# G1OJS/PyFT8

Hardware: AMD Instinct MI355X
Metric: FT8 15-s frames decoded/sec (higher is better)
Workload: dtype f32

## Files before the change

### pyft8_amd/csrc/ft8rx.hip

```cpp
#include <hip/hip_runtime.h>
#include <math.h>
#include <stdarg.h>
#include <stdio.h>
#include <stdlib.h>
#include <string.h>
#include <algorithm>
#include <new>
#include <string>
#include <vector>
#include "../../include/ft8rx.h"
#include "ft8_dev.h"

#define WL_MULT(i) ((i) == WL_BP0 ? 5 : (i) == WL_OSDNAN ? 10 : 1)
#define NF0MAX (FT8RX_MAX_F0 > 1024 ? 2048 : 1024)

#include "kernels/common.hpp"
#include "kernels/spectrogram.hpp"
#include "kernels/sync_search.hpp"
#include "kernels/llr.hpp"
#include "kernels/ap_patterns.hpp"
#include "kernels/bp.hpp"
#include "kernels/cycle_spectrum.hpp"
#include "kernels/fine_sync.hpp"
#include "kernels/osd.hpp"
#include "kernels/ap_calls.hpp"
#include "kernels/recall.hpp"
#include "kernels/report.hpp"
#include "kernels/ddc.hpp"
#include "kernels/synth.hpp"
#include "kernels/subtract.hpp"
#include "kernels/probes.hpp"
#include "host_messages.hpp"
#include "batch_plan.hpp"
#include "ddc_ring.hpp"
#include "optins.hpp"
#include "ilp_launch.hpp"

#define EV_EAGER_BYTES ((size_t)1 << 20)
#define HIPCHK(h, x) do { hipError_t _e = (x); if (_e != hipSuccess) { set_err(h, "%s failed: %s (%s:%d)", #x, hipGetErrorString(_e), __FILE__, __LINE__); return -2; } } while (0)

static std::vector<uint32_t> osd_trial_table(int S, int D, int T) {
    std::vector<uint32_t> t;
    const uint32_t N = OSD_NONE;
    t.push_back(N | (N << 8) | (N << 16));
    for (int i = 0; i < S; i++) t.push_back((uint32_t)i | (N << 8) | (N << 16));
    for (int i = 0; i < S; i++) for (int j = 0; j < D && j < i; j++) t.push_back((uint32_t)i | ((uint32_t)j << 8) | (N << 16));
    for (int i = 0; i < T; i++) for (int j = 0; j < i; j++) for (int k = 0; k < j; k++) t.push_back((uint32_t)i | ((uint32_t)j << 8) | ((uint32_t)k << 16));
    return t;
}
static int osd_nflip(int S, int T) { return S > T ? S : T; }

struct ft8rx_hashes { hostmsg::Hashes H; };

#define SYNC_WIN 352
static size_t sync_lds_bytes(const ft8rx_config& c) {
    const int nh0 = c.h0_hi - c.h0_lo;
    const size_t nrows = (size_t)((nh0 < SYNC_WIN ? nh0 : SYNC_WIN) + 24);
    return nrows * 16 * sizeof(double) + (nrows * 29 + 512) * sizeof(float);
}
static std::string g_create_err;

struct ResultSlot {
    ft8rx_record* rec = nullptr; int32_t* ncand = nullptr; ft8rx_event* ev = nullptr; int32_t* evcount = nullptr;
    ft8rx_record* h_rec = nullptr; int32_t* h_cnt = nullptr; ft8rx_event* h_ev = nullptr; int32_t* h_evc = nullptr;
    hipEvent_t ev_comp = nullptr, ev_done = nullptr;
    int B = 0;
    bool evpending = false;
    int32_t* d_evoffs = nullptr; ft8rx_event* h_evpacked = nullptr; ft8rx_event* d_evpacked = nullptr;
    bool packed = false;
    unsigned char* pk_buf = nullptr; hipEvent_t pk_fence = nullptr;
    ft8rx_packed_header* h_pkhdr = nullptr; ft8rx_packed_header* d_pkhdr = nullptr;
    bool recall = false;
    ft8rx_recall_entry* d_rc_ent = nullptr; int32_t* d_rc_cnt = nullptr; ft8rx_record* d_rc_rec = nullptr;
    ft8rx_record* h_rc_rec = nullptr; int32_t* h_rc_cnt = nullptr;
    bool reports = false;
    ft8rx_report* d_rp = nullptr; ft8rx_report* h_rp = nullptr;
};

static ApCalls ap_calls_off() { ApCalls a; memset(&a, 0, sizeof(a)); a.max_hd = FT8RX_AP_MAX_HD_DEFAULT; return a; }

#ifndef LADDER_GRID_CAP
#define LADDER_GRID_CAP (4 * 256 * 32)
#endif

struct ft8rx_handle {
    ft8rx_config cfg = {};
    int device = 0, max_frames = 0;
    hipStream_t stream = nullptr;
    int n_streams = 2;
    int ladder_mode = 0;
    int ladder_cap = LADDER_GRID_CAP;
    int msg_types = 0;
    bool weak = false; float weak_sync_min = FT8RX_WEAK_SYNC_MIN_DEFAULT; int32_t weak_osd_max_hd = FT8RX_WEAK_OSD_MAX_HD_DEFAULT;
    ApCalls ap = ap_calls_off();
    uint32_t ap_version = 0, ap_chunk_version[batchplan::MAX_CHUNKS] = {};
    ApCalls* d_apc = nullptr;
    int32_t* d_apcount = nullptr;
    bool rc_armed = false; int rc_frames = 0; bool rc_td = false; std::vector<int32_t> rc_off;
    int32_t rc_max_hd = FT8RX_RECALL_MAX_HD_DEFAULT, rc_min_gap = FT8RX_RECALL_MIN_GAP_DEFAULT;
    ft8rx_recall_entry* d_rc_src = nullptr; int32_t* d_rc_srccnt = nullptr; int32_t* d_rc_off = nullptr;
    int32_t* d_rc_trip = nullptr; int32_t* d_rc_tout = nullptr; float* d_rc_tsd = nullptr; float* d_rc_sgrid = nullptr; float* d_rc_llr = nullptr;
    bool reports = false;
    int32_t* d_rp_items = nullptr; int32_t* d_rp_count = nullptr;
    int sub_frames = FT8RX_SUBBATCH_DEFAULT;
    hipStream_t sub[batchplan::MAX_STREAMS] = {};
    hipEvent_t ev_fork = nullptr, ev_join[batchplan::MAX_STREAMS] = {};
    hipStream_t copy_s = nullptr;
    hipEvent_t ev_chunk[batchplan::MAX_CHUNKS] = {};
    Tables T = {};
    std::vector<void*> allocs, pinned;
    unsigned ready = 0;
    struct Chunk { void* p; size_t cap, used; };
    std::vector<Chunk> arena;
    int16_t* d_audio = nullptr;
    int16_t* d_audio2 = nullptr;
    hipStream_t h2d_s = nullptr;
    float* d_grid = nullptr;
    float* d_best_score = nullptr; int32_t* d_best_h0 = nullptr;
    ft8rx_record* d_rec = nullptr; int32_t* d_ncand = nullptr; ft8rx_event* d_ev = nullptr; int32_t* d_evcount = nullptr;
    float* d_llr0 = nullptr; float* d_saved = nullptr;
    Att *d_att0 = nullptr, *d_attG = nullptr, *d_attB = nullptr, *d_attO = nullptr;
    cpx *d_A = nullptr, *d_spec = nullptr;
    const uint32_t* d_trials = nullptr; int n_trials = 0;
    int32_t* d_work[WL_N] = {};
    int32_t* d_wcount = nullptr;
    uint8_t* d_colmask = nullptr; bool use_mask = false;
    ResultSlot slots[2];
    int slot_enq = 0, slot_fetch = 0, inflight = 0, last_slot = -1, fetched_slot = -1;
    hipEvent_t ev_cdone[2][batchplan::MAX_STREAMS] = {};
    bool free_running = false, need_barrier = true; int part_B = 0, part_n = 0;
    uint64_t pk_cap = 0; uint64_t* d_pkneed = nullptr; int32_t* d_pknrec = nullptr;
    hipEvent_t d2h_ev[32] = {}; uint32_t d2h_next = 0;
    float* d_wf = nullptr; double2* d_part = nullptr; double* d_pulse = nullptr; double* d_pc = nullptr;
    ft8rx_subsig* d_sigs = nullptr; int32_t* d_sigcnt = nullptr; int sig_cap = 0;
    float2 *d_zdec = nullptr, *d_model = nullptr, *d_adec = nullptr; SubdCtx* d_subctx = nullptr;
    double* d_ones = nullptr;
    DdcOut* d_ddc_outs = nullptr; DdcOut* h_ddc_outs = nullptr; hipEvent_t ddc_ev = nullptr; void* d_ddc_in = nullptr; size_t ddc_in_cap = 0;
    struct DdcStream {
        bool open = false; int kind = 0, D = 0, n_streams = 0, n_out = 0; int32_t rate = 0; float scale = 0.0f;
        int64_t n_origin = 0, pushed = 0, tiles = 0, cap = 0;
        void* d_in = nullptr; int16_t* d_out = nullptr; float* d_f32 = nullptr; DdcOut* d_outs = nullptr; char* h_stage = nullptr;
        hipEvent_t ev = nullptr;
    } ds;
    std::string err;
    bool profiling = false;
    std::vector<hipEvent_t> pev;
    std::vector<const char*> pnames;
    int n_stage = 0;
    float stage_ms[24] = {};
};
static_assert(sizeof(ft8rx_handle::ev_chunk) / sizeof(hipEvent_t) == batchplan::MAX_CHUNKS &&
              sizeof(ft8rx_handle::ap_chunk_version) / sizeof(uint32_t) == batchplan::MAX_CHUNKS &&
              sizeof(batchplan::BatchPlan::cb) / sizeof(int) == batchplan::MAX_CHUNKS + 1 &&
              batchplan::MAX_CHUNKS == 16 && batchplan::MAX_STREAMS == 8, "per-chunk arrays and the plan's boundaries");

static_assert(ddcring::TILE == DDC_TO && ddcring::OUT_RING == 2 * FT8RX_NSAMP, "ddc_ring.hpp: tile and output ring");
template <int D> constexpr bool ddc_ring_geom_ok() {
    using G = DdcGeom<D>;
    return ddcring::geom(D).R1 == G::R1 && ddcring::geom(D).C1 == G::C1 && ddcring::geom(D).R2 == G::R2 && ddcring::geom(D).C2 == G::C2 &&
           ddcring::last(D) == (int64_t)(G::NV - 1 - G::C2) * G::R1 + G::C1 && ddcring::in_capacity(D) >= 12000 * D + ddcring::span(D);
}
static_assert(ddc_ring_geom_ok<1>() && ddc_ring_geom_ok<2>() && ddc_ring_geom_ok<4>() && ddc_ring_geom_ok<8>() && ddc_ring_geom_ok<16>(),
              "ddc_ring.hpp: the filter geometry is the kernels'");

static void set_err(ft8rx_handle* h, const char* fmt, ...) {
    char buf[512];
    va_list ap; va_start(ap, fmt); vsnprintf(buf, sizeof(buf), fmt, ap); va_end(ap);
    if (h) h->err = buf; else g_create_err = buf;
}

#include <mutex>
struct StreamPool { hipStream_t main = nullptr, copy = nullptr, h2d = nullptr, sub[8] = {}; };
static std::mutex g_pool_mu;
static StreamPool g_pool[64];
static hipStream_t pool_stream(int device, hipStream_t StreamPool::* which, bool blocking) {
    std::lock_guard<std::mutex> lk(g_pool_mu);
    StreamPool& P = g_pool[device & 63];
    if (!(P.*which)) {
        hipStream_t s = nullptr;
        if ((blocking ? hipStreamCreate(&s) : hipStreamCreateWithFlags(&s, hipStreamNonBlocking)) != hipSuccess) return nullptr;
        P.*which = s;
    }
    return P.*which;
}
static hipStream_t pool_sub(int device, int i) {
    std::lock_guard<std::mutex> lk(g_pool_mu);
    StreamPool& P = g_pool[device & 63];
    if (!P.sub[i] && hipStreamCreateWithFlags(&P.sub[i], hipStreamNonBlocking) != hipSuccess) P.sub[i] = nullptr;
    return P.sub[i];
}

template <typename T> static int dalloc(ft8rx_handle* h, T** p, size_t n) {
    void* q = nullptr;
    hipError_t e = hipMalloc(&q, n * sizeof(T));
    if (e != hipSuccess) { set_err(h, "hipMalloc(%zu bytes) failed: %s", n * sizeof(T), hipGetErrorString(e)); return -2; }
    h->allocs.push_back(q); *p = (T*)q; return 0;
}
template <typename T> static int halloc(ft8rx_handle* h, T** p, size_t n, T** dev = nullptr) {
    void *q = nullptr, *d = nullptr;
    hipError_t e = hipHostMalloc(&q, n * sizeof(T), hipHostMallocDefault);
    if (e == hipSuccess && dev && (e = hipHostGetDevicePointer(&d, q, 0)) != hipSuccess) hipHostFree(q);
    if (e != hipSuccess) { set_err(h, "hipHostMalloc(%zu bytes) failed: %s", n * sizeof(T), hipGetErrorString(e)); return -2; }
    h->pinned.push_back(q); *p = (T*)q; if (dev) *dev = (T*)d; return 0;
}

enum WsGroup { WS_STAGING, WS_STAGING2, WS_MASK, WS_RECALL, WS_REPORTS, WS_PACKED, WS_SUB, WS_SUBD, WS_ONES, WS_DDC };
struct FirstUse {
    ft8rx_handle* h; WsGroup g; size_t nd, nh; int rc = 0;
    std::vector<void**> members;
    FirstUse(ft8rx_handle* h_, WsGroup g_) : h(h_), g(g_), nd(h_->allocs.size()), nh(h_->pinned.size()) {}
    template <typename T> void dev(T** p, size_t n) { if (!rc && !(rc = dalloc(h, p, n))) members.push_back((void**)p); }
    template <typename T> void host(T** p, size_t n, T** d = nullptr) {
        if (rc || (rc = halloc(h, p, n, d))) return;
        members.push_back((void**)p); if (d) members.push_back((void**)d);
    }
    int done() {
        if (!rc) { h->ready |= 1u << g; return 0; }
        while (h->allocs.size() > nd) { hipFree(h->allocs.back()); h->allocs.pop_back(); }
        while (h->pinned.size() > nh) { hipHostFree(h->pinned.back()); h->pinned.pop_back(); }
        for (void** m : members) *m = nullptr;
        return -2;
    }
};
static bool ws_ready(const ft8rx_handle* h, WsGroup g) { return (h->ready >> g) & 1u; }
#define FIRST_HIP(F, x) do { if (!(F).rc) { hipError_t _e = (x); if (_e != hipSuccess) { set_err((F).h, "%s failed: %s (%s:%d)", #x, hipGetErrorString(_e), __FILE__, __LINE__); (F).rc = -2; } } } while (0)

static int need_staging(ft8rx_handle* h, bool second = false) {
    const WsGroup g = second ? WS_STAGING2 : WS_STAGING;
    if (ws_ready(h, g)) return 0;
    FirstUse F(h, g);
    F.dev(second ? &h->d_audio2 : &h->d_audio, (size_t)h->max_frames * FT8RX_NSAMP);
    return F.done();
}

static void host_twiddle(int n, int count, std::vector<cpx>& w) {
    w.resize(count);
    for (int t = 0; t < count; t++) {
        double ang = (2.0 * M_PI * (double)t) / (double)n;
        w[t] = make_float2((float)cos(ang), (float)(-sin(ang)));
    }
}
template <typename T> static int upload(ft8rx_handle* h, const T** dst, const std::vector<T>& v) {
    T* p; if (dalloc(h, &p, v.size())) return -2;
    if (hipMemcpy(p, v.data(), v.size() * sizeof(T), hipMemcpyHostToDevice) != hipSuccess) { set_err(h, "table upload failed"); return -2; }
    *dst = p; return 0;
}

struct Scratch {
    ft8rx_handle* h;
    ~Scratch() { for (auto& c : h->arena) c.used = 0; }
    void* raw(size_t bytes) {
        bytes = (bytes + 255) & ~(size_t)255;
        if (!bytes) bytes = 256;
        for (auto& c : h->arena) if (c.cap - c.used >= bytes) { void* q = (char*)c.p + c.used; c.used += bytes; return q; }
        size_t largest = 0;
        for (auto& c : h->arena) if (c.cap > largest) largest = c.cap;
        size_t cap = bytes > 2 * largest ? bytes : 2 * largest;
        if (cap < ((size_t)1 << 20)) cap = (size_t)1 << 20;
        for (size_t i = 0; i < h->arena.size();) {
            if (h->arena[i].used == 0) { hipFree(h->arena[i].p); h->arena.erase(h->arena.begin() + i); } else i++;
        }
        void* q = nullptr;
        if (hipMalloc(&q, cap) != hipSuccess) { if (cap == bytes || hipMalloc(&q, bytes) != hipSuccess) return nullptr; cap = bytes; }
        h->arena.push_back({q, cap, bytes});
        return q;
    }
    template <typename T> T* get(size_t n) { return (T*)raw(n * sizeof(T)); }
    template <typename T> T* put(const T* src, size_t n) { T* q = get<T>(n); if (q && hipMemcpy(q, src, n * sizeof(T), hipMemcpyHostToDevice) != hipSuccess) return nullptr; return q; }
};

static int quiesce(ft8rx_handle* h, bool next_is_batch = false) {
    if (h->free_running || (h->last_slot >= 0 && !next_is_batch)) HIPCHK(h, hipStreamSynchronize(h->copy_s));
    h->free_running = false;
    h->need_barrier = true;
    return 0;
}
#define ENTER(h) do { HIPCHK(h, hipSetDevice((h)->device)); { const int _q = quiesce(h); if (_q) return _q; } } while (0)

template <class K, class KX, class... A>
static void launch_mt(K k, KX kx, unsigned mt, int grid, hipStream_t s, A... a) {
    if (!mt) k<<<grid, 64, 0, s>>>(a...);
    else kx<<<grid, 64, 0, s>>>(a..., mt);
}

static unsigned active_optins(const ft8rx_handle* h) {
    using namespace optins;
    return (h->slots[0].pk_buf ? bit(PACKED) : 0) | (h->msg_types != 0 ? bit(MSG_TYPES) : 0) | (h->ap.np != 0 ? bit(AP_CALLS) : 0) |
           (h->rc_armed ? bit(RECALL) : 0) | (h->weak ? bit(WEAK) : 0) | (h->reports ? bit(REPORTS) : 0);
}
static int refuse_conflict(ft8rx_handle* h, const char* who, optins::Id which, const char* hint = "") {
    const int c = optins::conflict(active_optins(h), which);
    if (c < 0) return 0;
    set_err(h, "%s: not supported together with %s%s", who, optins::TABLE[c].name, hint);
    return -1;
}

extern "C" {

int ft8rx_default_config(ft8rx_config* c) {
    if (!c) return -1;
    c->sync_score_min = 85.0f; c->max_cands = 200; c->f0_lo = 32; c->f0_hi = 960; c->h0_lo = -37; c->h0_hi = 87;
    c->bp_nc0_a = 35; c->bp_iters_a = 5; c->bp_nc0_b = 90; c->bp_iters_b = 20; c->osd_single = 30; c->osd_double = 2;
    c->llr_sd_min = 5.0f;
    c->osd_triple = 0; c->osd_max_hd = 0;
    return 0;
}

int ft8rx_device_count(void) { int n = 0; if (hipGetDeviceCount(&n) != hipSuccess) return 0; return n; }
int ft8rx_device_pci_bus_id(int device, char* buf, int len) {
    if (!buf || len < 16) return -1;
    return hipDeviceGetPCIBusId(buf, len, device) == hipSuccess ? 0 : -2;
}
int ft8rx_build_info(int32_t* grid_cols, int32_t* spec_bins, int32_t* max_f0) {
    static_assert(NF0MAX >= FT8RX_GRID_COLS && NF0MAX >= FT8RX_MAX_F0, "per-f0 scratch stride");
    if (grid_cols) *grid_cols = FT8RX_GRID_COLS;
    if (spec_bins) *spec_bins = FT8RX_SPEC_BINS;
    if (max_f0) *max_f0 = FT8RX_MAX_F0;
    return 0;
}
int ft8rx_build_limits(int32_t* max_cands, int32_t* event_cap) {
    static_assert(FT8RX_MAX_CANDS <= NF0MAX && (1 << cand_shift(FT8RX_MAX_CANDS)) == FT8RX_MAX_CANDS,
                  "max_cands: never more than k_topk has keys, and the largest candidate stride is the limit itself");
    if (max_cands) *max_cands = FT8RX_MAX_CANDS;
    if (event_cap) *event_cap = FT8RX_EVENT_CAP;
    return 0;
}

int ft8rx_get_fft_plans(int32_t* p1920, int32_t* p3200, int32_t* p300, int32_t* p320) {
    const int32_t a[8] = {8, 4, 4, 5, 3, 0, 0, 0}, b[8] = {8, 4, 4, 5, 5, 0, 0, 0}, c[8] = {5, 5, 4, 3, 0, 0, 0, 0}, d[8] = {8, 8, 5, 0, 0, 0, 0, 0};
    if (p1920) memcpy(p1920, a, sizeof(a));
    if (p3200) memcpy(p3200, b, sizeof(b));
    if (p300) memcpy(p300, c, sizeof(c));
    if (p320) memcpy(p320, d, sizeof(d));
    return 0;
}

const char* ft8rx_last_error(ft8rx_handle* h) { return h ? h->err.c_str() : g_create_err.c_str(); }

void ft8rx_destroy(ft8rx_handle* h) {
    if (!h) return;
    hipSetDevice(h->device);
    if (h->stream) hipStreamSynchronize(h->stream);
    if (h->copy_s) hipStreamSynchronize(h->copy_s);
    if (h->h2d_s) hipStreamSynchronize(h->h2d_s);
    for (int i = 0; i < 8; i++) { if (h->sub[i]) hipStreamSynchronize(h->sub[i]); if (h->ev_join[i]) hipEventDestroy(h->ev_join[i]); }
    for (void* p : h->allocs) hipFree(p);
    for (auto& c : h->arena) hipFree(c.p);
    for (auto e : h->pev) hipEventDestroy(e);
    for (int k = 0; k < 2; k++) for (int i = 0; i < 8; i++) if (h->ev_cdone[k][i]) hipEventDestroy(h->ev_cdone[k][i]);
    for (int i = 0; i < 32; i++) if (h->d2h_ev[i]) hipEventDestroy(h->d2h_ev[i]);
    for (hipEvent_t e : h->ev_chunk) if (e) hipEventDestroy(e);
    if (h->ev_fork) hipEventDestroy(h->ev_fork);
    if (h->ddc_ev) hipEventDestroy(h->ddc_ev);
    if (h->ds.ev) hipEventDestroy(h->ds.ev);
    for (ResultSlot& sl : h->slots) {
        if (sl.ev_comp) hipEventDestroy(sl.ev_comp);
        if (sl.ev_done) hipEventDestroy(sl.ev_done);
    }
    for (void* p : h->pinned) hipHostFree(p);
    delete h;
}

int ft8rx_create(const ft8rx_config* cfg, int device, int max_frames, ft8rx_handle** out) {
    if (!cfg || !out || max_frames < 1) { set_err(nullptr, "ft8rx_create: bad arguments"); return -1; }
    if (cfg->max_cands < 1 || cfg->max_cands > FT8RX_MAX_CANDS || cfg->f0_lo < 4 || cfg->f0_hi > FT8RX_MAX_F0 || cfg->f0_lo >= cfg->f0_hi ||
        cfg->h0_hi <= cfg->h0_lo || cfg->h0_lo < FT8RX_MIN_H0 || cfg->h0_hi > FT8RX_MAX_H0 || cfg->bp_nc0_a > cfg->bp_nc0_b || cfg->bp_iters_a > cfg->bp_iters_b ||
        cfg->osd_single < 0 || cfg->osd_single > OSD_MAXFLIP || cfg->osd_double < 0 || cfg->osd_double > OSD_MAXFLIP ||
        cfg->osd_triple < 0 || cfg->osd_triple > 40 || cfg->osd_max_hd < 0 || cfg->osd_max_hd > 174 ||
        osd_trial_table(cfg->osd_single, cfg->osd_double, cfg->osd_triple).size() > OSD_MAXTRIALS) {
        set_err(nullptr, "ft8rx_create: configuration out of the supported range"); return -1; }
    int ndev = 0;
    if (hipGetDeviceCount(&ndev) != hipSuccess || ndev < 1) { set_err(nullptr, "ft8rx_create: no HIP device available (this library has no CPU fallback)"); return -3; }
    if (device < 0 || device >= ndev) { set_err(nullptr, "ft8rx_create: device %d out of range (%d devices)", device, ndev); return -1; }
    ft8rx_handle* h = new ft8rx_handle();
    h->cfg = *cfg; h->device = device; h->max_frames = max_frames;
    if (hipSetDevice(device) != hipSuccess || !(h->stream = pool_stream(device, &StreamPool::main, true))) { set_err(nullptr, "ft8rx_create: cannot open device %d", device); delete h; return -2; }
    const size_t B = (size_t)max_frames, S = (size_t)1 << cand_shift(*cfg);
    int rc = 0;
    rc |= dalloc(h, &h->d_grid, B * FT8RX_GRID_ROWS * FT8RX_GRID_COLS);
    rc |= dalloc(h, &h->d_best_score, B * NF0MAX);
    rc |= dalloc(h, &h->d_best_h0, B * NF0MAX);
    rc |= dalloc(h, &h->d_rec, B * S);
    rc |= dalloc(h, &h->d_ncand, B);
    rc |= dalloc(h, &h->d_llr0, B * S * 174);
    rc |= dalloc(h, &h->d_saved, B * S * 5 * 174);
    rc |= dalloc(h, &h->d_att0, B * S * 5);
    rc |= dalloc(h, &h->d_attG, B * S * 2);
    rc |= dalloc(h, &h->d_attB, B * S * 5);
    rc |= dalloc(h, &h->d_attO, B * S * 10);
    static_assert((size_t)(96000 + FT8RX_SPEC_BINS) * sizeof(cpx) <= (size_t)FT8RX_GRID_ROWS * FT8RX_GRID_COLS * sizeof(float), "scratch A + cycle spectrum fit a frame's grid");
    if (!rc) { h->d_A = reinterpret_cast<cpx*>(h->d_grid); h->d_spec = h->d_A + B * 96000; }
    for (int i = 0; i < WL_N; i++) rc |= dalloc(h, &h->d_work[i], B * S * WL_MULT(i));
    rc |= dalloc(h, &h->d_wcount, (size_t)batchplan::MAX_CHUNKS * WL_N);
    rc |= dalloc(h, &h->d_apc, batchplan::MAX_CHUNKS);
    rc |= dalloc(h, &h->d_apcount, (size_t)batchplan::MAX_CHUNKS * 2);
    rc |= dalloc(h, &h->d_ev, B * FT8RX_EVENT_CAP);
    rc |= dalloc(h, &h->d_evcount, B);
    ResultSlot* const sl = h->slots;
    sl[0].rec = h->d_rec; sl[0].ncand = h->d_ncand; sl[0].ev = h->d_ev; sl[0].evcount = h->d_evcount;
    rc |= dalloc(h, &sl[1].rec, B * S);
    rc |= dalloc(h, &sl[1].ncand, B);
    rc |= dalloc(h, &sl[1].ev, B * FT8RX_EVENT_CAP);
    rc |= dalloc(h, &sl[1].evcount, B);
    const bool ev_compact = B * FT8RX_EVENT_CAP * sizeof(ft8rx_event) > EV_EAGER_BYTES;
    for (int k = 0; k < 2 && ev_compact; k++) rc |= dalloc(h, &sl[k].d_evoffs, B + 1);
    for (int k = 0; k < 2 && !rc; k++) {
        rc = halloc(h, &sl[k].h_rec, B * cfg->max_cands);
        if (!rc) rc = halloc(h, &sl[k].h_cnt, B);
        if (!rc) rc = halloc(h, &sl[k].h_ev, B * FT8RX_EVENT_CAP);
        if (!rc) rc = halloc(h, &sl[k].h_evc, B);
        if (!rc && ev_compact) rc = halloc(h, &sl[k].h_evpacked, B * FT8RX_EVENT_CAP, &sl[k].d_evpacked);
    }
    if (rc) { g_create_err = h->err; ft8rx_destroy(h); return -2; }
    std::vector<float> win(3840);
    for (int i = 0; i < 3840; i++) win[i] = (float)(0.5 + 0.5 * cos(M_PI * (double)(2 * i + 1 - 3840) / 3839.0));
    std::vector<double> taper(100);
    { double step = (0.0 - M_PI) / 99.0; for (int i = 0; i < 100; i++) { double y = (i == 99) ? 0.0 : (double)i * step + M_PI; taper[i] = 0.5 * (1.0 + cos(y)); } }
    std::vector<cpx> w;
    rc |= upload(h, &h->T.win, win);
    rc |= upload(h, &h->T.taper, taper);
    host_twiddle(1920, 1920, w);   rc |= upload(h, &h->T.W1920, w);
    host_twiddle(3840, FT8RX_GRID_COLS, w);    rc |= upload(h, &h->T.WR3840, w);
    host_twiddle(3200, 3200, w);   rc |= upload(h, &h->T.W3200, w);
    host_twiddle(96000, 96000, w); rc |= upload(h, &h->T.W96000, w);
    host_twiddle(300, 300, w);     rc |= upload(h, &h->T.W300, w);
    host_twiddle(320, 320, w);     rc |= upload(h, &h->T.W320, w);
    host_twiddle(192000, FT8RX_SPEC_BINS, w); rc |= upload(h, &h->T.WR192k, w);
    host_twiddle(32, 32, w);       rc |= upload(h, &h->T.W32, w);
    {
        std::vector<float> k32(1800);
        std::vector<cpx> cs(156), g1000(1000);
        for (int m = -900; m < 900; m++) {
            const int r = ((m % 100) + 100) % 100;
            k32[m + 900] = (r == 0) ? (m == 0 ? 32.0f : 0.0f) : (float)(sin(M_PI * (double)r / 100.0) / sin(M_PI * (double)m / 3200.0));
        }
        for (int sidx = 1; sidx < 7; sidx++) for (int q = 0; q <= 25; q++) {
            const double a = 2.0 * M_PI * (double)((q * sidx) % 100) / 100.0;
            cpx v = make_float2((float)cos(a), (float)sin(a));
            if (q == 0) v = make_float2(1.0f, 0.0f);
            cs[(sidx - 1) * 26 + q] = v;
        }
        for (int k = -150; k < 850; k++) {
            const int r = ((k % 100) + 100) % 100, j = (k - r) / 100;
            const double a = M_PI * (31.0 * (double)r - 100.0 * (double)j) / 3200.0;
            g1000[k + 150] = make_float2((float)cos(a), (float)sin(a));
        }
        std::vector<cpx> tw100(100);
        for (int m = 0; m < 100; m++) { const double a = -2.0 * M_PI * (double)m / 100.0; tw100[m] = make_float2((float)cos(a), (float)sin(a)); }
        rc |= upload(h, &h->T.K32, k32); rc |= upload(h, &h->T.CS100, cs); rc |= upload(h, &h->T.G1000, g1000); rc |= upload(h, &h->T.TW100, tw100);
    }
    if (rc) { g_create_err = h->err; ft8rx_destroy(h); return -2; }
    bool ok = true;
    ok &= hipMemcpyToSymbol(HIP_SYMBOL(d_CHK_N), FT8_CHK_N, sizeof(FT8_CHK_N)) == hipSuccess;
    ok &= hipMemcpyToSymbol(HIP_SYMBOL(d_CHK_V), FT8_CHK_V, sizeof(FT8_CHK_V)) == hipSuccess;
    {
        static uint8_t ev[522], ec[522]; static uint16_t ve[174][3];
        auto slot = [](int e) { const int c = FT8_EDGE_C[e], j = e - FT8_CHK_E0[c]; return j < 6 ? 83 * j + c : 498 + (c - 59); };
        for (int e = 0; e < 522; e++) { ev[slot(e)] = FT8_EDGE_V[e]; ec[slot(e)] = FT8_EDGE_C[e]; }
        for (int v = 0; v < 174; v++) for (int k = 0; k < 3; k++) ve[v][k] = (uint16_t)slot(FT8_VAR_E[v][k]);
        ok &= hipMemcpyToSymbol(HIP_SYMBOL(d_EDGE_V), ev, sizeof(ev)) == hipSuccess;
        ok &= hipMemcpyToSymbol(HIP_SYMBOL(d_EDGE_C), ec, sizeof(ec)) == hipSuccess;
        ok &= hipMemcpyToSymbol(HIP_SYMBOL(d_VAR_E), ve, sizeof(ve)) == hipSuccess;
    }
    ok &= hipMemcpyToSymbol(HIP_SYMBOL(d_G0), FT8_G0, sizeof(FT8_G0)) == hipSuccess;
    {
        static uint64_t rcg[83][2];
        memset(rcg, 0, sizeof(rcg));
        for (int r = 0; r < 91; r++) for (int j = 0; j < 83; j++) {
            const int v = 91 + j;
            if ((FT8_G0[r][v >> 6] >> (v & 63)) & 1ull) rcg[j][r >> 6] |= 1ull << (r & 63);
        }
        ok &= hipMemcpyToSymbol(HIP_SYMBOL(d_RCG), rcg, sizeof(rcg)) == hipSuccess;
    }
    {
        static uint64_t cm[128][3];
        memset(cm, 0, sizeof(cm));
        for (int c = 0; c < 83; c++) for (int j = 0; j < FT8_CHK_N[c]; j++) { int v = FT8_CHK_V[c][j]; cm[c][v >> 6] |= 1ull << (v & 63); }
        ok &= hipMemcpyToSymbol(HIP_SYMBOL(d_CHK_MASK), cm, sizeof(cm)) == hipSuccess;
    }
    {
        uint16_t syn[77];
        for (int pos = 0; pos < 77; pos++) syn[pos] = (uint16_t)hostmsg::crc14_serial(pos < 64 ? (1ull << pos) : 0ull, pos >= 64 ? (1ull << (pos - 64)) : 0ull);
        ok &= hipMemcpyToSymbol(HIP_SYMBOL(d_CRC_SYN), syn, sizeof(syn)) == hipSuccess;
    }
    {
        static uint32_t g0t[192][3];
        memset(g0t, 0, sizeof(g0t));
        for (int r = 0; r < 91; r++) for (int v = 0; v < 174; v++) if ((FT8_G0[r][v >> 6] >> (v & 63)) & 1ull) g0t[v][r >> 5] |= 1u << (r & 31);
        ok &= hipMemcpyToSymbol(HIP_SYMBOL(d_G0T), g0t, sizeof(g0t)) == hipSuccess;
        uint16_t syn91[96]; memset(syn91, 0, sizeof(syn91));
        for (int v = 0; v < 91; v++) {
            if (v < 77) { const int pos = 76 - v; syn91[v] = (uint16_t)hostmsg::crc14_serial(pos < 64 ? (1ull << pos) : 0ull, pos >= 64 ? (1ull << (pos - 64)) : 0ull); }
            else syn91[v] = (uint16_t)(1u << (13 - (v - 77)));
        }
        uint32_t synm[14][3]; memset(synm, 0, sizeof(synm));
        for (int v = 0; v < 91; v++) for (int k = 0; k < 14; k++) if ((syn91[v] >> k) & 1) synm[k][v >> 5] |= 1u << (v & 31);
        ok &= hipMemcpyToSymbol(HIP_SYMBOL(d_SYNM), synm, sizeof(synm)) == hipSuccess;
        static uint16_t ct[12][256];
        for (int b = 0; b < 12; b++) for (int x = 0; x < 256; x++) { uint16_t a = 0; for (int t = 0; t < 8; t++) if ((x >> t) & 1) a ^= syn91[8 * b + t]; ct[b][x] = a; }
        ok &= hipMemcpyToSymbol(HIP_SYMBOL(d_CRC_T), ct, sizeof(ct)) == hipSuccess;
        {
            float xn[174]; int perm[176], stk[64]; uint8_t p8[192];
            for (int i = 0; i < 174; i++) xn[i] = NAN;
            osd_std_sort_withnan(xn, perm, stk);
            memset(p8, 0, sizeof(p8));
            for (int i = 0; i < 174; i++) p8[i] = (uint8_t)perm[i];
            ok &= hipMemcpyToSymbol(HIP_SYMBOL(d_NANPERM), p8, sizeof(p8)) == hipSuccess;
        }
        const std::vector<uint32_t> tr = osd_trial_table(cfg->osd_single, cfg->osd_double, cfg->osd_triple);
        h->n_trials = (int)tr.size();
        if (upload(h, &h->d_trials, tr)) ok = false;
    }
    if (!ok) { set_err(nullptr, "ft8rx_create: device table upload failed"); ft8rx_destroy(h); return -2; }
    if (sync_lds_bytes(*cfg) > 65536) {
        ok &= hipFuncSetAttribute((const void*)k_sync, hipFuncAttributeMaxDynamicSharedMemorySize, (int)sync_lds_bytes(*cfg)) == hipSuccess;
        ok &= hipFuncSetAttribute((const void*)k_sync_acc, hipFuncAttributeMaxDynamicSharedMemorySize, (int)sync_lds_bytes(*cfg)) == hipSuccess;
    }
    if (!ok) { set_err(nullptr, "ft8rx_create: cannot reserve LDS for k_sync"); ft8rx_destroy(h); return -2; }
    int nfill = (int)B * FT8RX_GRID_COLS;
    k_fill_row0<<<(nfill + 255) / 256, 256, 0, h->stream>>>(h->d_grid, (int)B);
    if (hipStreamSynchronize(h->stream) != hipSuccess) { set_err(nullptr, "ft8rx_create: init kernel failed"); ft8rx_destroy(h); return -2; }
    bool okc = true;
    for (int i = 0; i < 24; i++) { hipEvent_t e = nullptr; okc = okc && hipEventCreate(&e) == hipSuccess; if (e) h->pev.push_back(e); }
    if (const char* e = getenv("FT8RX_SUBS_FIRST")) for (int i = 0; i < atoi(e) && i < 8; i++) pool_sub(device, i);
    okc = okc && (h->copy_s = pool_stream(device, &StreamPool::copy, false)) != nullptr;
    okc = okc && (h->h2d_s = pool_stream(device, &StreamPool::h2d, false)) != nullptr;
    for (hipEvent_t& e : h->ev_chunk) okc = okc && hipEventCreateWithFlags(&e, hipEventDisableTiming) == hipSuccess;
    okc = okc && hipEventCreateWithFlags(&h->ev_fork, hipEventDisableTiming) == hipSuccess;
    for (ResultSlot& s : h->slots) {
        okc = okc && hipEventCreateWithFlags(&s.ev_comp, hipEventDisableTiming) == hipSuccess;
        okc = okc && hipEventCreateWithFlags(&s.ev_done, hipEventDisableTiming) == hipSuccess;
    }
    if (!okc) { set_err(nullptr, "ft8rx_create: cannot create HIP streams/events"); ft8rx_destroy(h); return -2; }
    *out = h;
    return 0;
}

int ft8rx_set_profiling(ft8rx_handle* h, int on) { if (!h) return -1; h->profiling = on != 0; return 0; }

int ft8rx_get_stage_times(ft8rx_handle* h, int* n, const char** names, float* ms) {
    if (!h || !n) return -1;
    *n = h->n_stage;
    for (int i = 0; i < h->n_stage; i++) { if (names) names[i] = h->pnames[i]; if (ms) ms[i] = h->stage_ms[i]; }
    return 0;
}


static int ladder_grid(const ft8rx_handle* h, int max_items) { return max_items < h->ladder_cap ? max_items : h->ladder_cap; }

static void launch_sync(const float* grid, float* bs, int32_t* bh, const ft8rx_config& c, int B, hipStream_t s, bool weak) {
    const auto first = weak ? k_sync3 : k_sync, acc = weak ? k_sync3_acc : k_sync_acc;
    const int win = weak ? SYNC3_WIN : SYNC_WIN;
    const size_t lds = weak ? 0 : sync_lds_bytes(c);
    const int ntile = (c.f0_hi - c.f0_lo + 15) / 16;
    for (int lo = c.h0_lo; lo < c.h0_hi; lo += win) {
        ft8rx_config w = c;
        w.h0_lo = lo; w.h0_hi = lo + win < c.h0_hi ? lo + win : c.h0_hi;
        (lo == c.h0_lo ? first : acc)<<<dim3(ntile, B), 256, lds, s>>>(grid, bs, bh, w);
    }
}
static ft8rx_config weak_config(const ft8rx_handle* h) {
    ft8rx_config w = h->cfg;
    w.sync_score_min = h->weak_sync_min;
    w.llr_sd_min = -INFINITY;
    if (!w.osd_max_hd) w.osd_max_hd = h->weak_osd_max_hd;
    return w;
}
static void launch_fine(ft8rx_handle* h, const ft8rx_config& cfg, bool weak, int n_blocks, hipStream_t s, const cpx* spec, ft8rx_record* rec,
                        const int32_t* ncand, float* llr, const int32_t* trip, int32_t* t_out, float* t_sd, float* t_sgrid, WorkList work,
                        bool need_td) {
    if (weak) { k_fine_weak<<<n_blocks, FINE_NT, 0, s>>>(spec, rec, ncand, llr, h->T, cfg, trip, t_out, t_sd, t_sgrid, work); return; }
    ft8rx_ilp_fine(n_blocks, s, spec, rec, ncand, llr, h->T, cfg, trip, t_out, t_sd, t_sgrid, work);
    if (need_td) k_fine_td<<<n_blocks, FINE_NT, 0, s>>>(spec, rec, ncand, llr, h->T, cfg, trip, t_out, t_sd, t_sgrid, work);
}

static bool osd_wide(int nflip) { return nflip > OSD_FLIPS_A; }
static void launch_osd(const ft8rx_handle* h, unsigned mt, int grid, hipStream_t s, int mode, const float* llr, const float* saved, const Att* attB, ft8rx_record* rec,
                       const int32_t* ncand, Att* attO, ft8rx_event* ev, int32_t* evc, const uint32_t* trials, int ntr, int nflip, int max_hd,
                       int sh, WorkList work, WorkList nanl) {
    const bool wide = osd_wide(nflip);
    launch_mt(wide ? k_osd_wide : k_osd, wide ? k_osd_wide_ext : k_osd_ext, mt, grid, s,
              mode, llr, saved, attB, rec, ncand, attO, ev, evc, trials, ntr, nflip, max_hd, sh, work, nanl);
    launch_mt(wide ? k_osd_nan_wide : k_osd_nan, wide ? k_osd_nan_wide_ext : k_osd_nan_ext, mt, ladder_grid(h, OSD_NAN_GRID), s,
              mode, llr, saved, attB, rec, ncand, attO, ev, evc, trials, ntr, nflip, max_hd, sh, nanl);
}

static void launch_ap_calls(ft8rx_handle* h, int B, const float* llr0, ft8rx_record* rec, const int32_t* ncand, Att* attO, ft8rx_event* ev,
                            int32_t* evc, int32_t* cand_items, int32_t* osd_items, int32_t* ac, const ApCalls* apc, hipStream_t s) {
    const ft8rx_config& c = h->cfg;
    const int sh = cand_shift(c); const size_t S = (size_t)1 << sh;
    const int nflip = osd_nflip(c.osd_single, c.osd_triple);
    hipMemsetAsync(ac, 0, 2 * sizeof(int32_t), s);
    const WorkList cl = {cand_items, ac}, ol = {osd_items, ac + 1};
    k_ap_worklist<<<(B * S + 255) / 256, 256, 0, s>>>(rec, ncand, B, sh, cl);
    k_bp_ap<<<ladder_grid(h, B * c.max_cands * h->ap.np), 64, 0, s>>>(llr0, rec, ncand, attO, ev, evc, c, apc, cl, ol);
    (osd_wide(nflip) ? k_osd_ap_wide : k_osd_ap)<<<ladder_grid(h, B * c.max_cands * 3), 64, 0, s>>>(
        llr0, rec, ncand, attO, ev, evc, h->d_trials, h->n_trials, nflip, sh, apc, ol);
    k_select_ap<<<(B * S + 255) / 256, 256, 0, s>>>(rec, attO, apc, cl);
}

static void launch_reports(ft8rx_handle* h, int B, const cpx* spec, const ft8rx_record* rec, const int32_t* ncand, int32_t* items,
                           int32_t* count, ft8rx_report* rep, hipStream_t s) {
    const ft8rx_config& c = h->cfg;
    const int sh = cand_shift(c); const size_t S = (size_t)1 << sh;
    hipMemsetAsync(count, 0, sizeof(int32_t), s);
    const WorkList wl = {items, count};
    k_report_worklist<<<(B * S + 255) / 256, 256, 0, s>>>(rec, ncand, B, sh, wl, rep);
    k_report<<<ladder_grid(h, B * c.max_cands), FINE_NT, 0, s>>>(spec, rec, rep, h->T, sh, wl);
}

static void enqueue_chain(ft8rx_handle* h, const int16_t* d_audio, int f0, int B, hipStream_t s, bool prof, int slot, int chunk) {
    const ResultSlot& sl = h->slots[slot];
    const bool weak = h->weak;
    const ft8rx_config cw = weak ? weak_config(h) : h->cfg;
    const ft8rx_config& c = weak ? cw : h->cfg;
    const size_t F = (size_t)f0;
    const int sh = cand_shift(c); const size_t S = (size_t)1 << sh, FS = F * S;
    const int16_t* audio = d_audio + F * FT8RX_NSAMP;
    float* grid = h->d_grid + F * FT8RX_GRID_ROWS * FT8RX_GRID_COLS;
    float* bs = h->d_best_score + F * NF0MAX; int32_t* bh = h->d_best_h0 + F * NF0MAX;
    ft8rx_record* rec = sl.rec + FS; int32_t* ncand = sl.ncand + F;
    float* llr0 = h->d_llr0 + FS * 174; float* saved = h->d_saved + FS * 5 * 174;
    Att* att0 = h->d_att0 + FS * 5; Att* attG = h->d_attG + FS * 2; Att* attB = h->d_attB + FS * 5; Att* attO = h->d_attO + FS * 10;
    cpx* A = reinterpret_cast<cpx*>(grid); cpx* spec = A + (size_t)B * 96000;
    ft8rx_event* ev = sl.ev + F * FT8RX_EVENT_CAP; int32_t* evc = sl.evcount + F;
#define STAGE(name) do { if (prof) { hipEventRecord(h->pev[h->pnames.size()], s); h->pnames.push_back(name); } } while (0)
    int32_t* wc = h->d_wcount + WL_N * chunk;
    WorkList wl[WL_N];
    for (int i = 0; i < WL_N; i++) { wl[i].items = h->d_work[i] + FS * WL_MULT(i); wl[i].count = wc + i; }
    STAGE("spectrogram");
    ft8rx_ilp_spectrogram(B, s, audio, grid, h->T);
    STAGE("sync");
    launch_sync(grid, bs, bh, c, B, s, weak);
    STAGE("topk");
    k_topk<<<B, 1024, 0, s>>>(bs, bh, rec, ncand, c, evc, wc, h->use_mask ? h->d_colmask + F * NF0MAX : nullptr);
    STAGE("grid_llr");
    const unsigned mt = (unsigned)h->msg_types;
    launch_mt(k_grid_llr, k_grid_llr_ext, mt, XCD_GRID(B, c.max_cands), s, grid, rec, ncand, llr0, c, nullptr, nullptr, nullptr, att0, ev, evc, B);
    k_worklist_att<<<(B * S * 5 + 255) / 256, 256, 0, s>>>(rec, ncand, att0, B, sh, wl[WL_BP0]);
    STAGE("bp_grid");
    launch_mt(k_bp, k_bp_ext, mt, ladder_grid(h, B * c.max_cands * 5), s, 0, llr0, rec, ncand, nullptr, att0, nullptr, ev, evc, c, c.bp_nc0_a, c.bp_iters_a, wl[WL_BP0], 0, 5);
    STAGE("select0");
    k_select0<<<(B * S + 255) / 256, 256, 0, s>>>(rec, ncand, att0, B, sh, wl[WL_FINE]);
    STAGE("cycle_fft");
    k_cyc_a<<<dim3(40, B), 256, 0, s>>>(audio, A, h->T);
    k_cyc_bc<<<dim3(CYC_BC_GRID, B), 256, 0, s>>>(A, spec, h->T);
    STAGE("fine");
    launch_fine(h, c, weak, ladder_grid(h, B * c.max_cands), s, spec, rec, ncand, llr0, nullptr, nullptr, nullptr, nullptr, wl[WL_FINE],
                c.h0_lo < FT8RX_MIN_H0_FD || c.h0_hi > FT8RX_MAX_H0_FD + 1);
    k_worklist<<<(B * S + 255) / 256, 256, 0, s>>>(rec, ncand, B, sh, wl[WL_BP1]);
    STAGE("bp_fine");
    const auto bp_fine = [&](int n_variants, const WorkList& work, int v0) {
        launch_mt(k_bp, k_bp_ext, mt, B * c.max_cands * n_variants, s, 1, llr0, rec, ncand, attG, attB, saved, ev, evc, c, c.bp_nc0_b, c.bp_iters_b,
                  work, v0, n_variants);
    };
    if (h->ladder_mode == 0) {
        bp_fine(1, wl[WL_BP1], 0);
        k_select1<<<(B * S + 255) / 256, 256, 0, s>>>(0, rec, ncand, attG, attB, B, c, wl[WL_BP1B]);
        bp_fine(1, wl[WL_BP1B], 1);
        k_select1<<<(B * S + 255) / 256, 256, 0, s>>>(1, rec, ncand, attG, attB, B, c, wl[WL_BP1C]);
        bp_fine(3, wl[WL_BP1C], 2);
        STAGE("select1");
        k_select1<<<(B * S + 255) / 256, 256, 0, s>>>(2, rec, ncand, attG, attB, B, c, wl[WL_OSD]);
    } else {
        bp_fine(5, wl[WL_BP1], 0);
        STAGE("select1");
        k_select1<<<(B * S + 255) / 256, 256, 0, s>>>(3, rec, ncand, attG, attB, B, c, wl[WL_OSD]);
    }
    STAGE("osd");
    launch_osd(h, mt, ladder_grid(h, B * c.max_cands * 10), s, 0, llr0, saved, attB, rec, ncand, attO, ev, evc, h->d_trials, h->n_trials,
               osd_nflip(c.osd_single, c.osd_triple), c.osd_max_hd, sh, wl[WL_OSD], wl[WL_OSDNAN]);
    STAGE("select2");
    k_select2<<<(B * S + 255) / 256, 256, 0, s>>>(rec, ncand, attO, B, sh);
    if (h->ap.np) {
        STAGE("ap_calls");
        ApCalls* apc = h->d_apc + chunk;
        if (h->ap_chunk_version[chunk] != h->ap_version) {
            k_ap_stage<<<1, 64, 0, s>>>(apc, h->ap);
            h->ap_chunk_version[chunk] = h->ap_version;
        }
        launch_ap_calls(h, B, llr0, rec, ncand, attO, ev, evc, wl[WL_BP0].items, wl[WL_OSDNAN].items, h->d_apcount + 2 * chunk, apc, s);
    }
    if (sl.recall) {
        STAGE("recall");
        ft8rx_recall_entry* ent = sl.d_rc_ent + F * FT8RX_RECALL_MAX;
        int32_t* rcnt = sl.d_rc_cnt + F;
        k_recall_stage<<<B, FT8RX_RECALL_MAX, 0, s>>>(h->d_rc_src + F * FT8RX_RECALL_MAX, h->d_rc_srccnt + F, ent, rcnt, sl.d_rc_rec + F * FT8RX_RECALL_MAX);
        const int base = h->rc_off[F], n = h->rc_off[F + B] - base;
        if (n > 0) {
            k_recall_trip<<<B, FT8RX_RECALL_MAX, 0, s>>>(ent, rcnt, h->d_rc_off + F, h->d_rc_trip);
            const size_t b = (size_t)base;
            launch_fine(h, c, false, n, s, spec, nullptr, nullptr, h->d_rc_llr + b * 174, h->d_rc_trip + 3 * b, h->d_rc_tout + 5 * b,
                        h->d_rc_tsd + b, h->d_rc_sgrid + b * 632, WorkList{nullptr, nullptr}, h->rc_td);
            k_recall_score<<<n, 64, 0, s>>>(h->d_rc_sgrid, h->d_rc_tout, h->d_rc_trip, h->d_rc_off + F, base, ent, rec, ncand, sh,
                                            h->rc_max_hd, h->rc_min_gap, sl.d_rc_rec + F * FT8RX_RECALL_MAX);
        }
    }
    if (sl.reports) {
        STAGE("report");
        launch_reports(h, B, spec, rec, ncand, h->d_rp_items + FS, h->d_rp_count + chunk, sl.d_rp + FS, s);
    }
    if (prof) hipEventRecord(h->pev[h->pnames.size()], s);
#undef STAGE
}

static void enqueue_chunk(ft8rx_handle* h, const int16_t* d_audio, int f0, int n, hipStream_t s, int slot, int chunk) {
    const int sub = (h->sub_frames > 0 && h->sub_frames < n) ? h->sub_frames : n;
    for (int o = 0; o < n; o += sub) enqueue_chain(h, d_audio, f0 + o, (o + sub <= n) ? sub : n - o, s, false, slot, chunk);
}

using batchplan::BatchPlan;
using batchplan::Entry;

static int batch_begin(ft8rx_handle* h, Entry e, int B, int slot, bool chunked, int16_t** stage) {
    ResultSlot& sl = h->slots[slot];
    h->pnames.clear();
    if (e != batchplan::DEVICE && need_staging(h)) return -2;
    if (e == batchplan::HOST_PIPELINED && slot == 1 && need_staging(h, true)) return -2;
    if (h->inflight == 2) { h->slot_fetch ^= 1; h->inflight = 1; }
    if (h->rc_armed && B != h->rc_frames) { set_err(h, "recall entries were set for %d frames, the batch has %d", h->rc_frames, B); return -1; }
    sl.recall = h->rc_armed;
    h->rc_armed = false;
    sl.reports = h->reports;
    *stage = h->d_audio;
    if (e == batchplan::HOST_PIPELINED) {
        *stage = slot ? h->d_audio2 : h->d_audio;
        HIPCHK(h, hipStreamWaitEvent(h->h2d_s, sl.ev_comp, 0));
    }
    for (int i = 1; i < h->n_streams && chunked; i++) if (!h->sub[i - 1]) {
        if (!(h->sub[i - 1] = pool_sub(h->device, i - 1))) { set_err(h, "cannot create a chunk stream"); return -2; }
        HIPCHK(h, hipEventCreateWithFlags(&h->ev_join[i - 1], hipEventDisableTiming));
    }
    return 0;
}

static int batch_submit(ft8rx_handle* h, const BatchPlan& plan, Entry e, int slot, const int16_t* audio, int16_t* stage) {
    ResultSlot& sl = h->slots[slot];
    const bool host = e != batchplan::DEVICE;
    const int16_t* d_audio = host ? stage : audio; const int16_t* host_audio = host ? audio : nullptr;
    const int ns = h->n_streams, nc = plan.nc, B = plan.cb[nc];
    const bool free_run = plan.mode == batchplan::FREE_RUN, pipelined = e == batchplan::HOST_PIPELINED, sync_host = e == batchplan::HOST_SYNC;
    hipStream_t cs = pipelined ? h->h2d_s : h->copy_s;
    const size_t frame_bytes = sizeof(int16_t) * (size_t)FT8RX_NSAMP;
    auto chunk_stream = [&](int k) { const int i = k % ns; return i == 0 ? h->stream : h->sub[i - 1]; };
    if (free_run) {
        for (int i = 0; i < ns; i++) for (int k = 0; k < 2; k++)
            if (!h->ev_cdone[k][i]) HIPCHK(h, hipEventCreateWithFlags(&h->ev_cdone[k][i], hipEventDisableTiming));
        if (h->need_barrier || h->part_B != B || h->part_n != nc) {
            if (h->free_running) HIPCHK(h, hipStreamWaitEvent(h->stream, h->slots[h->last_slot].ev_comp, 0));
            HIPCHK(h, hipEventRecord(h->ev_fork, h->stream));
            for (int i = 1; i < ns; i++) HIPCHK(h, hipStreamWaitEvent(h->sub[i - 1], h->ev_fork, 0));
            h->need_barrier = false; h->part_B = B; h->part_n = nc;
        }
    } else {
        { const int q = quiesce(h, true); if (q) return q; }
        HIPCHK(h, hipStreamWaitEvent(h->stream, sl.ev_done, 0));
        if (plan.mode == batchplan::SINGLE) {
            if (host_audio) HIPCHK(h, hipMemcpyAsync(stage, host_audio, frame_bytes * B, hipMemcpyHostToDevice, h->stream));
            if (h->profiling) enqueue_chain(h, d_audio, 0, B, h->stream, true, slot, 0);
            else enqueue_chunk(h, d_audio, 0, B, h->stream, slot, 0);
            return 0;
        }
        HIPCHK(h, hipEventRecord(h->ev_fork, h->stream));
        if (sync_host) HIPCHK(h, hipStreamWaitEvent(cs, h->ev_fork, 0));
        for (int i = 1; i < ns; i++) HIPCHK(h, hipStreamWaitEvent(h->sub[i - 1], h->ev_fork, 0));
    }
    if (pipelined) {
        HIPCHK(h, hipMemcpyAsync(stage, host_audio, frame_bytes * B, hipMemcpyHostToDevice, cs));
        HIPCHK(h, hipEventRecord(h->ev_chunk[0], cs));
        if (!free_run) for (int i = 0; i < ns; i++) HIPCHK(h, hipStreamWaitEvent(chunk_stream(i), h->ev_chunk[0], 0));
    }
    for (int k = 0; k < nc; k++) {
        const int f0 = plan.cb[k], n = plan.cb[k + 1] - f0;
        if (n <= 0 && !free_run) continue;
        hipStream_t s = chunk_stream(k);
        if (free_run) {
            HIPCHK(h, hipStreamWaitEvent(s, sl.ev_done, 0));
            if (pipelined) HIPCHK(h, hipStreamWaitEvent(s, h->ev_chunk[0], 0));
        } else if (sync_host) {
            HIPCHK(h, hipMemcpyAsync(stage + (size_t)f0 * FT8RX_NSAMP, host_audio + (size_t)f0 * FT8RX_NSAMP, frame_bytes * n, hipMemcpyHostToDevice, cs));
            HIPCHK(h, hipEventRecord(h->ev_chunk[k], cs));
            HIPCHK(h, hipStreamWaitEvent(s, h->ev_chunk[k], 0));
        }
        if (n > 0) enqueue_chunk(h, d_audio, f0, n, s, slot, k);
        if (free_run) {
            HIPCHK(h, hipEventRecord(h->ev_cdone[slot][k], s));
            HIPCHK(h, hipStreamWaitEvent(h->copy_s, h->ev_cdone[slot][k], 0));
        }
    }
    if (free_run) h->free_running = true;
    else for (int i = 1; i < ns; i++) {
        HIPCHK(h, hipEventRecord(h->ev_join[i - 1], h->sub[i - 1]));
        HIPCHK(h, hipStreamWaitEvent(h->stream, h->ev_join[i - 1], 0));
    }
    return 0;
}

static int batch_finish(ft8rx_handle* h, int slot, int B, hipStream_t fin) {
    ResultSlot& sl = h->slots[slot];
    const int mc = h->cfg.max_cands, sh = cand_shift(h->cfg);
    const bool pack_events = sl.d_evpacked && (size_t)B * FT8RX_EVENT_CAP * sizeof(ft8rx_event) > EV_EAGER_BYTES;
    if (pack_events) {
        k_ev_scan<<<1, 1024, 0, fin>>>(sl.evcount, B, sl.d_evoffs);
        k_ev_compact<<<B, 64, 0, fin>>>(sl.ev, sl.evcount, sl.d_evoffs, sl.d_evpacked);
    }
    sl.packed = sl.pk_buf != nullptr;
    if (sl.packed) {
        if (sl.pk_fence) { HIPCHK(h, hipStreamWaitEvent(fin, sl.pk_fence, 0)); sl.pk_fence = nullptr; }
        k_pack_count<<<B, 256, 0, fin>>>(sl.rec, sl.ncand, sl.ev, sl.evcount, h->d_pkneed, h->d_pknrec, sh);
        k_pack_scan<<<1, 1024, 0, fin>>>(h->d_pknrec, sl.ncand, sl.evcount, B, mc, (unsigned long long)h->pk_cap, sl.pk_buf, sl.d_pkhdr);
        k_pack_write<<<B, 256, 0, fin>>>(sl.rec, sl.ev, h->d_pkneed, B, sl.pk_buf, sh);
    }
    HIPCHK(h, hipEventRecord(sl.ev_comp, fin));
    if (fin != h->copy_s) HIPCHK(h, hipStreamWaitEvent(h->copy_s, sl.ev_comp, 0));
    HIPCHK(h, hipMemcpyAsync(sl.h_cnt, sl.ncand, sizeof(int32_t) * B, hipMemcpyDeviceToHost, h->copy_s));
    HIPCHK(h, hipMemcpy2DAsync(sl.h_rec, sizeof(ft8rx_record) * mc, sl.rec, sizeof(ft8rx_record) << sh, sizeof(ft8rx_record) * mc, B, hipMemcpyDeviceToHost, h->copy_s));
    HIPCHK(h, hipMemcpyAsync(sl.h_evc, sl.evcount, sizeof(int32_t) * B, hipMemcpyDeviceToHost, h->copy_s));
    sl.evpending = pack_events;
    if (!pack_events) HIPCHK(h, hipMemcpyAsync(sl.h_ev, sl.ev, sizeof(ft8rx_event) * (size_t)B * FT8RX_EVENT_CAP, hipMemcpyDeviceToHost, h->copy_s));
    if (sl.recall) {
        HIPCHK(h, hipMemcpyAsync(sl.h_rc_cnt, sl.d_rc_cnt, sizeof(int32_t) * B, hipMemcpyDeviceToHost, h->copy_s));
        HIPCHK(h, hipMemcpyAsync(sl.h_rc_rec, sl.d_rc_rec, sizeof(ft8rx_record) * FT8RX_RECALL_MAX * (size_t)B, hipMemcpyDeviceToHost, h->copy_s));
    }
    if (sl.reports)
        HIPCHK(h, hipMemcpy2DAsync(sl.h_rp, sizeof(ft8rx_report) * mc, sl.d_rp, sizeof(ft8rx_report) << sh, sizeof(ft8rx_report) * mc, B, hipMemcpyDeviceToHost, h->copy_s));
    HIPCHK(h, hipEventRecord(sl.ev_done, h->copy_s));
    sl.B = B; h->last_slot = slot; h->slot_enq ^= 1; h->inflight++;
    return 0;
}

static int launch_batch(ft8rx_handle* h, Entry e, const int16_t* audio, int B) {
    HIPCHK(h, hipSetDevice(h->device));
    const BatchPlan plan = batchplan::plan_batch(B, h->n_streams, h->profiling, e);
    const int slot = h->slot_enq;
    int16_t* stage = nullptr;
    if (const int rc = batch_begin(h, e, B, slot, plan.mode != batchplan::SINGLE, &stage)) return rc;
    if (const int rc = batch_submit(h, plan, e, slot, audio, stage)) return rc;
    HIPCHK(h, hipGetLastError());
    return batch_finish(h, slot, B, plan.mode == batchplan::FREE_RUN ? h->copy_s : h->stream);
}

static void fetch_events(ResultSlot& sl) {
    if (!sl.evpending) return;
    size_t off = 0;
    for (int f = 0; f < sl.B; f++) {
        int c = sl.h_evc[f]; c = c > FT8RX_EVENT_CAP ? FT8RX_EVENT_CAP : (c < 0 ? 0 : c);
// ... 2 lines not shown
    }
    sl.evpending = false;
}

int ft8rx_enqueue_batch(ft8rx_handle* h, const int16_t* d_audio, int B) {
    if (!h || !d_audio) return -1;
    if (B < 1 || B > h->max_frames) { set_err(h, "ft8rx_enqueue_batch: n_frames %d outside [1, %d]", B, h->max_frames); return -1; }
    return launch_batch(h, batchplan::DEVICE, d_audio, B);
}

int ft8rx_enqueue_batch_host(ft8rx_handle* h, const int16_t* audio, int B) {
    if (!h || !audio) return -1;
    if (B < 1 || B > h->max_frames) { set_err(h, "ft8rx_enqueue_batch_host: n_frames %d outside [1, %d]", B, h->max_frames); return -1; }
    return launch_batch(h, batchplan::HOST_PIPELINED, audio, B);
}

int ft8rx_set_streams(ft8rx_handle* h, int n) { if (!h || n < 1 || n > batchplan::MAX_STREAMS) return -1; h->n_streams = n; return 0; }
int ft8rx_set_subbatch(ft8rx_handle* h, int frames) { if (!h || frames < 0) return -1; h->sub_frames = frames; return 0; }
int ft8rx_set_ladder_mode(ft8rx_handle* h, int mode) { if (!h || mode < 0 || mode > 1) return -1; h->ladder_mode = mode; return 0; }

int ft8rx_set_ladder_grid(ft8rx_handle* h, int cap) {
    if (!h) return -1;
    if (cap < 0 || cap > LADDER_GRID_CAP) { set_err(h, "ft8rx_set_ladder_grid: cap %d outside [0, %d] (0 = the default, %d)", cap, LADDER_GRID_CAP, LADDER_GRID_CAP); return -1; }
    ENTER(h);
    h->ladder_cap = cap ? cap : LADDER_GRID_CAP;
    return 0;
}

int ft8rx_set_weak(ft8rx_handle* h, int32_t on, float sync_min, int32_t osd_max_hd) {
    if (!h) return -1;
    if (on) {
        if (!(sync_min > 0.0f) || !(sync_min < INFINITY)) { set_err(h, "ft8rx_set_weak: sync_min %g must be a positive score", (double)sync_min); return -1; }
        if (osd_max_hd < 1 || osd_max_hd > 174) { set_err(h, "ft8rx_set_weak: osd_max_hd %d outside [1, 174]", osd_max_hd); return -1; }
        if (refuse_conflict(h, "ft8rx_set_weak", optins::WEAK)) return -1;
        h->weak_sync_min = sync_min; h->weak_osd_max_hd = osd_max_hd;
    }
    h->weak = on != 0;
    return 0;
}

int ft8rx_set_msg_types(ft8rx_handle* h, int32_t mask) {
    if (!h) return -1;
    if (mask < 0 || mask > FT8RX_MT_ALL) { set_err(h, "ft8rx_set_msg_types: mask %d outside [0, %d]", mask, FT8RX_MT_ALL); return -1; }
    if (mask && refuse_conflict(h, "ft8rx_set_msg_types", optins::MSG_TYPES)) return -1;
    h->msg_types = mask;
    return 0;
}

static int build_ap_patterns(const char* my, const char* dx, ApCalls* a, std::string* err) {
    const bool hm = my && *my, hd = dx && *dx;
    const long cm = hm ? hostmsg::pack_c28_std(my) : 0, cd = hd ? hostmsg::pack_c28_std(dx) : 0;
    if (cm < 0) { *err = std::string("my_call '") + my + "' is not a standard callsign"; return -1; }
    if (cd < 0) { *err = std::string("dx_call '") + dx + "' is not a standard callsign"; return -1; }
    const int32_t max_hd = a->max_hd;
    memset(a, 0, sizeof(*a)); a->max_hd = max_hd;
    auto word = [](long c1, long c2, unsigned g15) { return ((unsigned __int128)c1 << 49) | ((unsigned __int128)c2 << 20) | ((unsigned __int128)g15 << 3) | 1u; };
    const unsigned G_RRR = 32402, G_73 = 32404, G_RR73 = 32403;
    for (int p = 5; p <= 10; p++) {
        const bool on = p == 5 ? hm : p == 7 ? hd : (hm && hd);
        if (!on) continue;
        const int k = p - FT8RX_AP_FIRST;
        const unsigned __int128 w = word(p == 7 ? 2 : cm, p == 5 ? 0 : cd, p == 8 ? G_RRR : p == 9 ? G_73 : G_RR73);
        const uint64_t lo = (uint64_t)w, hi = (uint64_t)(w >> 64);
        if (p >= 8) {
            hostmsg::encode_cw174(lo, hi, a->val[k]);
            a->msk[k][0] = a->msk[k][1] = ~0ull; a->msk[k][2] = (1ull << 46) - 1;
            a->lo[k] = lo; a->hi[k] = hi;
            hostmsg::Hashes H; std::string f[3];
            if (!hostmsg::unpack_ext(lo, hi, 0, H, f)) { *err = "the words of my_call / dx_call do not unpack as a standard message"; return -1; }
        } else {
            const int nk = p == 5 ? 29 : 58;
            for (int i = 0; i < 77; i++) {
                if (!(i < nk || i >= 74)) continue;
                const unsigned b = (unsigned)((w >> (76 - i)) & 1u);
                a->msk[k][i >> 6] |= 1ull << (i & 63);
                if (b) a->val[k][i >> 6] |= 1ull << (i & 63);
            }
        }
        a->pat[a->np++] = p;
    }
    return 0;
}

int ft8rx_set_ap_calls(ft8rx_handle* h, const char* my_call, const char* dx_call) {
    if (!h) return -1;
    ApCalls a = h->ap;
    std::string err;
    if (build_ap_patterns(my_call, dx_call, &a, &err)) { set_err(h, "ft8rx_set_ap_calls: %s", err.c_str()); return -1; }
    if (a.np && refuse_conflict(h, "ft8rx_set_ap_calls", optins::AP_CALLS)) return -1;
    h->ap = a; h->ap_version++;
    return 0;
}

int ft8rx_set_ap_max_hd(ft8rx_handle* h, int32_t max_hd) {
    if (!h) return -1;
    if (max_hd < 1 || max_hd > 174) { set_err(h, "ft8rx_set_ap_max_hd: %d outside [1, 174]", max_hd); return -1; }
    h->ap.max_hd = max_hd; h->ap_version++;
    return 0;
}

int ft8rx_ap_patterns(const char* my_call, const char* dx_call, uint8_t* bits_out, uint8_t* mask_out) {
    ApCalls a = ap_calls_off();
    std::string err;
    if (build_ap_patterns(my_call, dx_call, &a, &err)) { g_create_err = "ft8rx_ap_patterns: " + err; return -1; }
    for (int k = 0; k < FT8RX_AP_N; k++) for (int i = 0; i < 174; i++) {
        if (bits_out) bits_out[k * 174 + i] = (uint8_t)((a.val[k][i >> 6] >> (i & 63)) & 1ull);
        if (mask_out) mask_out[k * 174 + i] = (uint8_t)((a.msk[k][i >> 6] >> (i & 63)) & 1ull);
    }
    return 0;
}

static int recall_kind(uint64_t lo, uint64_t hi) {
    const unsigned i3 = (unsigned)(lo & 7u);
    if (i3 != 1 && i3 != 2) return RC_SKIP;
    const uint64_t ca = ((lo >> 49) | (hi << 15)) & 0xFFFFFFFull, cb = (lo >> 20) & 0xFFFFFFFull;
    const uint64_t STD = 2063592ull + 4194304ull;
    if (cb < STD || !(ca < 3 || ca >= STD)) return RC_SKIP;
    hostmsg::Hashes H; std::string f[3];
    if (!hostmsg::unpack_ext(lo, hi & 0x1FFFull, 0, H, f)) return RC_SKIP;
    for (int k = 0; k < 3; k++) if (f[k].find('<') != std::string::npos) return RC_SKIP;
    return ca < 3 ? RC_TOKEN : RC_CALL;
}

int ft8rx_recall_hypotheses(const ft8rx_recall_entry* entry, uint64_t* words_lo, uint64_t* words_hi) {
    if (!entry) return -1;
    const uint64_t lo = entry->msg_lo, hi = entry->msg_hi & 0x1FFFull;
    const int kind = recall_kind(lo, hi);
    if (kind == RC_SKIP) return 0;
    int n = 0;
    for (int k = 0; k < 126; k++) {
        uint64_t w; unsigned g15 = 0, r = 0;
        if (k == 0) w = lo;
        else if (kind != RC_CALL) break;
        else {
            if (k <= 3) g15 = 32401u + (unsigned)k;
            else if (k < 65) g15 = (unsigned)(32435 + (k - 4) - 30);
            else { g15 = (unsigned)(32435 + (k - 65) - 30); r = 1; }
            w = (lo & ~(0xFFFFull << 3)) | ((uint64_t)g15 << 3) | ((uint64_t)r << 18);
            if (w == lo) continue;
        }
        if (words_lo) words_lo[n] = w;
        if (words_hi) words_hi[n] = hi;
        n++;
    }
    return n;
}

static int recall_alloc(ft8rx_handle* h) {
    if (ws_ready(h, WS_RECALL)) return 0;
    const size_t B = (size_t)h->max_frames, N = B * FT8RX_RECALL_MAX;
    FirstUse F(h, WS_RECALL);
    F.dev(&h->d_rc_src, N); F.dev(&h->d_rc_srccnt, B); F.dev(&h->d_rc_off, B + 1);
    F.dev(&h->d_rc_trip, N * 3); F.dev(&h->d_rc_tout, N * 5); F.dev(&h->d_rc_tsd, N);
    F.dev(&h->d_rc_sgrid, N * 632); F.dev(&h->d_rc_llr, N * 174);
    for (ResultSlot& sl : h->slots) {
        F.dev(&sl.d_rc_ent, N); F.dev(&sl.d_rc_cnt, B); F.dev(&sl.d_rc_rec, N);
        F.host(&sl.h_rc_rec, N); F.host(&sl.h_rc_cnt, B);
    }
    return F.done();
}

int ft8rx_set_recall(ft8rx_handle* h, const ft8rx_recall_entry* entries, const int32_t* counts, int n_frames) {
    if (!h) return -1;
    ENTER(h);
    if (!entries || n_frames == 0) { h->rc_armed = false; return 0; }
    if (!counts || n_frames < 1 || n_frames > h->max_frames) { set_err(h, "ft8rx_set_recall: n_frames %d outside [1, %d]", n_frames, h->max_frames); return -1; }
    if (refuse_conflict(h, "ft8rx_set_recall", optins::RECALL)) return -1;
    const ft8rx_config& c = h->cfg;
    std::vector<ft8rx_recall_entry> st((size_t)n_frames * FT8RX_RECALL_MAX);
    std::vector<int32_t> cnt(n_frames), off(n_frames + 1, 0);
    bool td = false;
    for (int f = 0; f < n_frames; f++) {
        if (counts[f] < 0 || counts[f] > FT8RX_RECALL_MAX) { set_err(h, "ft8rx_set_recall: counts[%d] = %d outside [0, %d]", f, counts[f], FT8RX_RECALL_MAX); return -1; }
        cnt[f] = counts[f]; off[f + 1] = off[f] + counts[f];
        for (int e = 0; e < counts[f]; e++) {
            ft8rx_recall_entry E = entries[(size_t)f * FT8RX_RECALL_MAX + e];
            if (E.f0_idx < c.f0_lo || E.f0_idx >= c.f0_hi || E.h0_idx < c.h0_lo || E.h0_idx >= c.h0_hi) {
                set_err(h, "ft8rx_set_recall: entry %d of frame %d at (f0_idx %d, h0_idx %d) lies outside the search range", e, f, E.f0_idx, E.h0_idx); return -1; }
            E.pad = (uint16_t)recall_kind(E.msg_lo, E.msg_hi);
            td |= E.h0_idx < FT8RX_MIN_H0_FD || E.h0_idx > FT8RX_MAX_H0_FD;
            st[(size_t)f * FT8RX_RECALL_MAX + e] = E;
        }
    }
    if (recall_alloc(h)) return -2;
    HIPCHK(h, hipMemcpy(h->d_rc_src, st.data(), sizeof(ft8rx_recall_entry) * st.size(), hipMemcpyHostToDevice));
    HIPCHK(h, hipMemcpy(h->d_rc_srccnt, cnt.data(), sizeof(int32_t) * cnt.size(), hipMemcpyHostToDevice));
    HIPCHK(h, hipMemcpy(h->d_rc_off, off.data(), sizeof(int32_t) * off.size(), hipMemcpyHostToDevice));
    h->rc_off = off; h->rc_frames = n_frames; h->rc_td = td; h->rc_armed = true;
    return 0;
}

int ft8rx_fetch_recall(ft8rx_handle* h, int n_frames, ft8rx_record* records, int32_t* counts) {
    if (!h) return -1;
    const int slot = h->fetched_slot;
    if (slot < 0) { set_err(h, "ft8rx_fetch_recall: no batch has been fetched"); return -1; }
    const ResultSlot& sl = h->slots[slot];
    if (n_frames < 1 || n_frames > sl.B) { set_err(h, "ft8rx_fetch_recall: %d frames requested, the batch had %d", n_frames, sl.B); return -1; }
    HIPCHK(h, hipEventSynchronize(sl.ev_done));
    if (!sl.recall) {
        if (counts) memset(counts, 0, sizeof(int32_t) * n_frames);
        if (records) memset(records, 0, sizeof(ft8rx_record) * FT8RX_RECALL_MAX * (size_t)n_frames);
        return 0;
    }
    if (counts) memcpy(counts, sl.h_rc_cnt, sizeof(int32_t) * n_frames);
    if (records) memcpy(records, sl.h_rc_rec, sizeof(ft8rx_record) * FT8RX_RECALL_MAX * (size_t)n_frames);
    return 0;
}

int ft8rx_set_reports(ft8rx_handle* h, int32_t on) {
    if (!h) return -1;
    ENTER(h);
    if (!on) { h->reports = false; return 0; }
    if (refuse_conflict(h, "ft8rx_set_reports", optins::REPORTS)) return -1;
    if (!ws_ready(h, WS_REPORTS)) {
        const size_t B = (size_t)h->max_frames, N = B << cand_shift(h->cfg);
        FirstUse F(h, WS_REPORTS);
        F.dev(&h->d_rp_items, N); F.dev(&h->d_rp_count, (size_t)batchplan::MAX_CHUNKS);
        for (ResultSlot& sl : h->slots) { F.dev(&sl.d_rp, N); F.host(&sl.h_rp, B * h->cfg.max_cands); }
        if (F.done()) return -2;
    }
    h->reports = true;
    return 0;
}

int ft8rx_fetch_reports(ft8rx_handle* h, int n_frames, ft8rx_report* reports) {
    if (!h || !reports) return -1;
    const int slot = h->fetched_slot;
    if (slot < 0) { set_err(h, "ft8rx_fetch_reports: no batch has been fetched"); return -1; }
    const ResultSlot& sl = h->slots[slot];
    if (n_frames < 1 || n_frames > sl.B) { set_err(h, "ft8rx_fetch_reports: %d frames requested, the batch had %d", n_frames, sl.B); return -1; }
    HIPCHK(h, hipEventSynchronize(sl.ev_done));
    const size_t bytes = sizeof(ft8rx_report) * (size_t)n_frames * h->cfg.max_cands;
    if (!sl.reports) memset(reports, 0, bytes);
    else memcpy(reports, sl.h_rp, bytes);
    return 0;
}

int ft8rx_set_recall_gates(ft8rx_handle* h, int32_t max_hd, int32_t min_gap) {
    if (!h) return -1;
    if (max_hd < 1 || max_hd > 174 || min_gap < 0 || min_gap > 174) { set_err(h, "ft8rx_set_recall_gates: max_hd %d / min_gap %d outside [1, 174] / [0, 174]", max_hd, min_gap); return -1; }
    h->rc_max_hd = max_hd; h->rc_min_gap = min_gap;
    return 0;
}

static double ddc_bessel_i0(double x) {
    double sum = 1.0, term = 1.0;
    for (int k = 1; k < 200; k++) { term *= (x / (2.0 * k)) * (x / (2.0 * k)); sum += term; if (term < 1e-20 * sum) break; }
    return sum;
}
static std::vector<float> ddc_design(double f_pass, double f_stop, double A, double fs) {
    int N = (int)ceil((A - 7.95) / (2.285 * 2.0 * M_PI * (f_stop - f_pass) / fs)) + 1;
    if (N % 2 == 0) N++;
    const double beta = 0.1102 * (A - 8.7), fc = (f_pass + f_stop) / (2.0 * fs), c = (N - 1) / 2.0;
    std::vector<double> h(N);
    double sum = 0.0;
    for (int n = 0; n < N; n++) {
        const double x = n - c, r = x / c;
        const double sinc = x == 0.0 ? 2.0 * fc : sin(2.0 * M_PI * fc * x) / (M_PI * x);
        h[n] = sinc * ddc_bessel_i0(beta * sqrt(1.0 - r * r)) / ddc_bessel_i0(beta);
        sum += h[n];
    }
    std::vector<float> out(N);
    for (int n = 0; n < N; n++) out[n] = (float)(h[n] / sum);
    return out;
}
struct DdcTaps { std::vector<float> h1[3], h2[2]; };
static const DdcTaps& ddc_taps() {
    static const DdcTaps T = [] {
        DdcTaps t;
        for (int i = 0; i < 3; i++) t.h1[i] = ddc_design(3200.0, 20800.0, 85.0, 48000.0 * (1 << i));
        t.h2[0] = ddc_design(2800.0, 3200.0, 75.0, 24000.0);
        t.h2[1] = ddc_design(2800.0, 3200.0, 75.0, 12000.0);
        return t;
    }();
    return T;
}
static int ddc_decimation(int32_t rate_hz) {
    for (int D = 1; D <= 16; D *= 2) if (rate_hz == 12000 * D) return D;
    return 0;
}
static const std::vector<float>* ddc_stage_taps(int D, int stage) {
    const DdcTaps& T = ddc_taps();
    if (stage == 2) return &T.h2[D == 1];
    return D >= 4 ? &T.h1[D == 4 ? 0 : D == 8 ? 1 : 2] : nullptr;
}

int ft8rx_ddc_taps(int32_t rate_hz, int stage, float* taps, int cap) {
    const int D = ddc_decimation(rate_hz);
    if (!D || (stage != 1 && stage != 2)) return -1;
    const std::vector<float>* t = ddc_stage_taps(D, stage);
    if (!t) return 0;
    for (int i = 0; taps && i < cap && i < (int)t->size(); i++) taps[i] = (*t)[i];
    return (int)t->size();
}

static int ddc_workspaces(ft8rx_handle* h) {
    if (ws_ready(h, WS_DDC)) return 0;
    const DdcTaps& T = ddc_taps();
    static_assert(sizeof(c_ddc_h1) == sizeof(float) * 3 * 64 && sizeof(c_ddc_h2) == sizeof(float) * 2 * 288, "tap tables");
    std::vector<float> a(3 * 64, 0.0f), b(2 * 288, 0.0f);
    for (int i = 0; i < 3; i++) { if (T.h1[i].size() > 64) return -2; memcpy(&a[i * 64], T.h1[i].data(), sizeof(float) * T.h1[i].size()); }
    for (int i = 0; i < 2; i++) { if (T.h2[i].size() > 288) return -2; memcpy(&b[i * 288], T.h2[i].data(), sizeof(float) * T.h2[i].size()); }
    if (T.h1[0].size() != 17 || T.h1[1].size() != 31 || T.h1[2].size() != 61 || T.h2[0].size() != 283 || T.h2[1].size() != 143) {
        set_err(h, "ft8rx_ddc: the designed filters do not have the lengths the kernels were compiled for"); return -2;
    }
    FirstUse F(h, WS_DDC);
    F.dev(&h->d_ddc_outs, (size_t)h->max_frames);
// ... 394 lines not shown

static int launch_batch_sync(ft8rx_handle* h, const int16_t* audio, int B) {
    h->inflight = 0; h->slot_fetch = h->slot_enq;
    if (need_staging(h)) return -2;
    return launch_batch(h, batchplan::HOST_SYNC, audio, B);
}

int ft8rx_decode_batch(ft8rx_handle* h, const int16_t* audio, int B, ft8rx_record* records, int32_t* counts,
                       ft8rx_event* events, int32_t* event_counts) {
    if (!h || !audio) return -1;
    if (B < 1 || B > h->max_frames) { set_err(h, "ft8rx_decode_batch: n_frames %d outside [1, %d]", B, h->max_frames); return -1; }
    if (const int rc = launch_batch_sync(h, audio, B)) return rc;
    return ft8rx_fetch_results(h, B, records, counts, events, event_counts);
}

int ft8rx_decode_messages(ft8rx_handle* h, const int16_t* audio, int B, ft8rx_message* out, int max_msgs, int32_t* out_counts,
                          int n_threads, ft8rx_hashes* table, int32_t* flags) {
    if (!h || !audio || !out || !out_counts) return -1;
    if (B < 1 || B > h->max_frames || max_msgs < 1) { set_err(h, "ft8rx_decode_messages: bad n_frames / max_msgs"); return -1; }
    if (refuse_conflict(h, "ft8rx_decode_messages", optins::DECODE_MESSAGES,
                        " (ft8rx_message rows cannot carry it); use ft8rx_decode_batch with ft8rx_package_batch_ext / ft8rx_fetch_recall")) return -1;
    int rc = launch_batch_sync(h, audio, B);
    if (rc) return rc;
    const ft8rx_record* rec; const int32_t* cnt; const ft8rx_event* ev; const int32_t* evc;
    rc = ft8rx_fetch_results_view(h, B, &rec, &cnt, &ev, &evc);
    if (rc) return rc;
    return hostmsg::package_batch(rec, cnt, ev, evc, B, h->cfg.max_cands, out, max_msgs, out_counts, n_threads, table ? &table->H : nullptr, flags);
}

#define NEED(p) do { if (!(p)) { set_err(h, "scratch allocation/copy failed (%s:%d)", __FILE__, __LINE__); return -2; } } while (0)

int ft8rx_spectrogram(ft8rx_handle* h, const int16_t* audio, int B, float* grid) {
    if (!h || !audio || !grid || B < 1 || B > h->max_frames) return -1;
    ENTER(h);
    if (need_staging(h)) return -2;
    HIPCHK(h, hipMemcpy(h->d_audio, audio, sizeof(int16_t) * (size_t)B * FT8RX_NSAMP, hipMemcpyHostToDevice));
    ft8rx_ilp_spectrogram(B, h->stream, h->d_audio, h->d_grid, h->T);
    HIPCHK(h, hipStreamSynchronize(h->stream));
    HIPCHK(h, hipMemcpy(grid, h->d_grid, sizeof(float) * (size_t)B * FT8RX_GRID_ROWS * FT8RX_GRID_COLS, hipMemcpyDeviceToHost));
    return 0;
}

int ft8rx_hop_spectrum(ft8rx_handle* h, const int16_t* window3840, float* row) {
    if (!h || !window3840 || !row) return -1;
    ENTER(h);
    if (need_staging(h)) return -2;
    float* d_row = h->d_best_score;
    HIPCHK(h, hipMemcpyAsync(h->d_audio, window3840, sizeof(int16_t) * 3840, hipMemcpyHostToDevice, h->stream));
    ft8rx_ilp_hop_spectrum(h->stream, h->d_audio, d_row, h->T);
    HIPCHK(h, hipMemcpyAsync(row, d_row, sizeof(float) * FT8RX_GRID_COLS, hipMemcpyDeviceToHost, h->stream));
    HIPCHK(h, hipStreamSynchronize(h->stream));
    return 0;
}

int ft8rx_sync_search(ft8rx_handle* h, const float* grid, int B, int32_t* f0_idx, int32_t* h0_idx, float* score, int32_t* counts) {
    if (!h || !grid || B < 1 || B > h->max_frames) return -1;
    ENTER(h);
    const ft8rx_config& c = h->cfg;
    HIPCHK(h, hipMemcpy(h->d_grid, grid, sizeof(float) * (size_t)B * FT8RX_GRID_ROWS * FT8RX_GRID_COLS, hipMemcpyHostToDevice));
    launch_sync(h->d_grid, h->d_best_score, h->d_best_h0, c, B, h->stream, false);
    k_topk<<<B, 1024, 0, h->stream>>>(h->d_best_score, h->d_best_h0, h->d_rec, h->d_ncand, c, nullptr, nullptr, nullptr);
    HIPCHK(h, hipStreamSynchronize(h->stream));
    const size_t S = (size_t)1 << cand_shift(c);
    std::vector<ft8rx_record> rec((size_t)B * S);
    HIPCHK(h, hipMemcpy(rec.data(), h->d_rec, sizeof(ft8rx_record) * rec.size(), hipMemcpyDeviceToHost));
    HIPCHK(h, hipMemcpy(counts, h->d_ncand, sizeof(int32_t) * B, hipMemcpyDeviceToHost));
    for (int f = 0; f < B; f++) for (int i = 0; i < c.max_cands; i++) {
        const ft8rx_record& r = rec[(size_t)f * S + i];
        size_t o = (size_t)f * c.max_cands + i;
        f0_idx[o] = r.f0_idx; h0_idx[o] = r.h0_idx; score[o] = r.score;
    }
    return 0;
}

static int sync_scores(ft8rx_handle* h, const float* grid, int B, int f0_lo, int f0_hi, float* score, int32_t* h0_idx, bool weak) {
    const char* who = weak ? "ft8rx_sync_scores_weak" : "ft8rx_sync_scores";
    if (!h || !grid || !score || !h0_idx || B < 1 || B > h->max_frames) return -1;
    if (f0_lo < 4 || f0_hi <= f0_lo || f0_hi > FT8RX_GRID_COLS - 15 || f0_hi - f0_lo > NF0MAX) {
        set_err(h, "%s: f0 range [%d, %d) outside [4, %d]", who, f0_lo, f0_hi, FT8RX_GRID_COLS - 15); return -1; }
    ENTER(h);
    ft8rx_config c = h->cfg;
    c.f0_lo = f0_lo; c.f0_hi = f0_hi;
    HIPCHK(h, hipMemcpy(h->d_grid, grid, sizeof(float) * (size_t)B * FT8RX_GRID_ROWS * FT8RX_GRID_COLS, hipMemcpyHostToDevice));
    const int nf0 = f0_hi - f0_lo;
    launch_sync(h->d_grid, h->d_best_score, h->d_best_h0, c, B, h->stream, weak);
    HIPCHK(h, hipGetLastError());
    HIPCHK(h, hipMemcpy2DAsync(score, sizeof(float) * nf0, h->d_best_score, sizeof(float) * NF0MAX, sizeof(float) * nf0, B, hipMemcpyDeviceToHost, h->stream));
    HIPCHK(h, hipMemcpy2DAsync(h0_idx, sizeof(int32_t) * nf0, h->d_best_h0, sizeof(int32_t) * NF0MAX, sizeof(int32_t) * nf0, B, hipMemcpyDeviceToHost, h->stream));
    HIPCHK(h, hipStreamSynchronize(h->stream));
    return 0;
}

int ft8rx_sync_scores(ft8rx_handle* h, const float* grid, int B, int f0_lo, int f0_hi, float* score, int32_t* h0_idx) {
    return sync_scores(h, grid, B, f0_lo, f0_hi, score, h0_idx, false);
}
int ft8rx_sync_scores_weak(ft8rx_handle* h, const float* grid, int B, int f0_lo, int f0_hi, float* score, int32_t* h0_idx) {
    return sync_scores(h, grid, B, f0_lo, f0_hi, score, h0_idx, true);
}

static std::vector<int32_t> pack_triples(int n, const int32_t* frame, const int32_t* f0_idx, const int32_t* h0_idx) {
    std::vector<int32_t> trip(3 * (size_t)n);
    for (int i = 0; i < n; i++) { trip[3 * i] = frame[i]; trip[3 * i + 1] = f0_idx[i]; trip[3 * i + 2] = h0_idx[i]; }
    return trip;
}

int ft8rx_llr_grid(ft8rx_handle* h, const float* grid, int B, int n, const int32_t* frame, const int32_t* f0_idx,
                   const int32_t* h0_idx, float* llr, float* sd, int32_t* snr) {
    if (!h || !grid || B < 1 || B > h->max_frames || n < 1) return -1;
    ENTER(h);
    HIPCHK(h, hipMemcpy(h->d_grid, grid, sizeof(float) * (size_t)B * FT8RX_GRID_ROWS * FT8RX_GRID_COLS, hipMemcpyHostToDevice));
    const std::vector<int32_t> trip = pack_triples(n, frame, f0_idx, h0_idx);
    Scratch S{h};
    int32_t* d_trip = S.put(trip.data(), trip.size()); NEED(d_trip);
    float* d_llr = S.get<float>((size_t)n * 174); NEED(d_llr);
    float* d_sd = S.get<float>(n); NEED(d_sd);
    int32_t* d_snr = S.get<int32_t>(n); NEED(d_snr);
    k_grid_llr<<<n, 64, 0, h->stream>>>(h->d_grid, nullptr, nullptr, d_llr, h->cfg, d_trip, d_sd, d_snr, nullptr, nullptr, nullptr, n);
    HIPCHK(h, hipStreamSynchronize(h->stream));
    HIPCHK(h, hipMemcpy(llr, d_llr, sizeof(float) * (size_t)n * 174, hipMemcpyDeviceToHost));
    HIPCHK(h, hipMemcpy(sd, d_sd, sizeof(float) * n, hipMemcpyDeviceToHost));
    HIPCHK(h, hipMemcpy(snr, d_snr, sizeof(int32_t) * n, hipMemcpyDeviceToHost));
    return 0;
}

int ft8rx_cycle_spectrum(ft8rx_handle* h, const int16_t* audio, int B, float* spec) {
    if (!h || !audio || !spec || B < 1 || B > h->max_frames) return -1;
    ENTER(h);
    if (need_staging(h)) return -2;
    HIPCHK(h, hipMemcpy(h->d_audio, audio, sizeof(int16_t) * (size_t)B * FT8RX_NSAMP, hipMemcpyHostToDevice));
    k_cyc_a<<<dim3(40, B), 256, 0, h->stream>>>(h->d_audio, h->d_A, h->T);
    k_cyc_bc<<<dim3(CYC_BC_GRID, B), 256, 0, h->stream>>>(h->d_A, h->d_spec, h->T);
    HIPCHK(h, hipStreamSynchronize(h->stream));
    HIPCHK(h, hipMemcpy(spec, h->d_spec, sizeof(cpx) * (size_t)B * FT8RX_SPEC_BINS, hipMemcpyDeviceToHost));
    return 0;
}

static int fine_probe(ft8rx_handle* h, const float* spec, int B, int n, const int32_t* frame, const int32_t* f0_idx, const int32_t* h0_idx,
                      int32_t* ret, int32_t* ttweak, int32_t* ftweak, int32_t* nsync, float* llr, float* sd, int32_t* snr, float* sgrid, bool weak) {
    if (!h || !spec || B < 1 || B > h->max_frames || n < 1) return -1;
    if (weak) for (int i = 0; i < n; i++)
        if (frame[i] < 0 || frame[i] >= B || f0_idx[i] < 4 || f0_idx[i] >= FT8RX_MAX_F0 || h0_idx[i] < FT8RX_MIN_H0 || h0_idx[i] >= FT8RX_MAX_H0) {
            set_err(h, "ft8rx_fine_weak: triple %d (frame %d, f0 %d, h0 %d) outside [0, %d) x [4, %d) x [%d, %d)", i,
                    frame[i], f0_idx[i], h0_idx[i], B, FT8RX_MAX_F0, FT8RX_MIN_H0, FT8RX_MAX_H0); return -1; }
    ENTER(h);
    HIPCHK(h, hipMemcpy(h->d_spec, spec, sizeof(cpx) * (size_t)B * FT8RX_SPEC_BINS, hipMemcpyHostToDevice));
    const std::vector<int32_t> trip = pack_triples(n, frame, f0_idx, h0_idx);
    Scratch S{h};
    int32_t* d_trip = S.put(trip.data(), trip.size()); NEED(d_trip);
    float* d_llr = S.get<float>((size_t)n * 174); NEED(d_llr);
    HIPCHK(h, hipMemset(d_llr, 0, sizeof(float) * (size_t)n * 174));
    float* d_sd = S.get<float>(n); NEED(d_sd);
    int32_t* d_out = S.get<int32_t>((size_t)n * 5); NEED(d_out);
    float* d_sg = sgrid ? S.get<float>((size_t)n * 632) : nullptr; if (sgrid) NEED(d_sg);
    launch_fine(h, weak ? weak_config(h) : h->cfg, weak, n, h->stream, h->d_spec, nullptr, nullptr, d_llr, d_trip, d_out, d_sd, d_sg,
                WorkList{nullptr, nullptr}, true);
    HIPCHK(h, hipStreamSynchronize(h->stream));
    std::vector<int32_t> o((size_t)n * 5);
    HIPCHK(h, hipMemcpy(o.data(), d_out, sizeof(int32_t) * o.size(), hipMemcpyDeviceToHost));
    for (int i = 0; i < n; i++) { ret[i] = o[5 * i]; ttweak[i] = o[5 * i + 1]; ftweak[i] = o[5 * i + 2]; nsync[i] = o[5 * i + 3]; snr[i] = o[5 * i + 4]; }
    HIPCHK(h, hipMemcpy(llr, d_llr, sizeof(float) * (size_t)n * 174, hipMemcpyDeviceToHost));
    HIPCHK(h, hipMemcpy(sd, d_sd, sizeof(float) * n, hipMemcpyDeviceToHost));
    if (sgrid) HIPCHK(h, hipMemcpy(sgrid, d_sg, sizeof(float) * (size_t)n * 632, hipMemcpyDeviceToHost));
    return 0;
}

int ft8rx_fine(ft8rx_handle* h, const float* spec, int B, int n, const int32_t* frame, const int32_t* f0_idx, const int32_t* h0_idx,
               int32_t* ret, int32_t* ttweak, int32_t* ftweak, int32_t* nsync, float* llr, float* sd, int32_t* snr, float* sgrid) {
    return fine_probe(h, spec, B, n, frame, f0_idx, h0_idx, ret, ttweak, ftweak, nsync, llr, sd, snr, sgrid, false);
}
int ft8rx_fine_weak(ft8rx_handle* h, const float* spec, int B, int n, const int32_t* frame, const int32_t* f0_idx, const int32_t* h0_idx,
                    int32_t* ret, int32_t* ttweak, int32_t* ftweak, int32_t* nsync, float* llr, float* sd, int32_t* snr, float* sgrid) {
    return fine_probe(h, spec, B, n, frame, f0_idx, h0_idx, ret, ttweak, ftweak, nsync, llr, sd, snr, sgrid, true);
}

int ft8rx_ldpc(ft8rx_handle* h, const float* llr, int n, int max_ncheck0, int max_iters, int32_t* ok, uint64_t* msg_lo,
               uint64_t* msg_hi, int32_t* n_its, int32_t* has_out, float* llr_out) {
    if (!h || !llr || n < 1) return -1;
    ENTER(h);
    Scratch S{h};
    float* d_in = S.put(llr, (size_t)n * 174); NEED(d_in);
    float* d_out = S.get<float>((size_t)n * 174); NEED(d_out);
    HIPCHK(h, hipMemset(d_out, 0, sizeof(float) * (size_t)n * 174));
    Att* d_att = S.get<Att>(n); NEED(d_att);
    k_bp<<<n, 64, 0, h->stream>>>(2, d_in, nullptr, nullptr, nullptr, d_att, d_out, nullptr, nullptr, h->cfg, max_ncheck0, max_iters, WorkList{nullptr, nullptr}, 0, 1);
    HIPCHK(h, hipStreamSynchronize(h->stream));
    std::vector<Att> a(n);
    HIPCHK(h, hipMemcpy(a.data(), d_att, sizeof(Att) * n, hipMemcpyDeviceToHost));
    for (int i = 0; i < n; i++) { ok[i] = a[i].ok; msg_lo[i] = a[i].lo; msg_hi[i] = a[i].hi; n_its[i] = a[i].ok ? a[i].n_its : -1; has_out[i] = a[i].has_out; }
    if (llr_out) HIPCHK(h, hipMemcpy(llr_out, d_out, sizeof(float) * (size_t)n * 174, hipMemcpyDeviceToHost));
    return 0;
}

int ft8rx_ap_calls_probe(ft8rx_handle* h, const float* llr, int n, ft8rx_record* records, ft8rx_event* events, int32_t* event_count) {
    if (!h || !llr || !records || n < 1 || n > h->cfg.max_cands) { if (h) set_err(h, "ft8rx_ap_calls_probe: 1 <= n <= max_cands"); return -1; }
    if (!h->ap.np) { set_err(h, "ft8rx_ap_calls_probe: no call set (ft8rx_set_ap_calls)"); return -1; }
    ENTER(h);
    Scratch S{h};
    const size_t st = (size_t)1 << cand_shift(h->cfg);
    std::vector<ft8rx_record> r0(st);
    memset(r0.data(), 0, sizeof(ft8rx_record) * st);
    for (int i = 0; i < n; i++) r0[i].status = FT8RX_ST_EXHAUSTED;
    std::vector<float> l0(st * 174, 0.0f);
    memcpy(l0.data(), llr, sizeof(float) * (size_t)n * 174);
    const int32_t nc = n, zero = 0;
    float* d_llr = S.put(l0.data(), l0.size()); NEED(d_llr);
    ft8rx_record* d_rec = S.put(r0.data(), st); NEED(d_rec);
    int32_t* d_nc = S.put(&nc, 1); NEED(d_nc);
    int32_t* d_evc = S.put(&zero, 1); NEED(d_evc);
    Att* d_att = S.get<Att>(st * 10); NEED(d_att);
    ft8rx_event* d_ev = S.get<ft8rx_event>(FT8RX_EVENT_CAP); NEED(d_ev);
    int32_t* d_cl = S.get<int32_t>(st); NEED(d_cl);
    int32_t* d_ol = S.get<int32_t>(st * 3); NEED(d_ol);
    int32_t* d_ac = S.get<int32_t>(2); NEED(d_ac);
    ApCalls* d_apc = S.get<ApCalls>(1); NEED(d_apc);
    k_ap_stage<<<1, 64, 0, h->stream>>>(d_apc, h->ap);
    launch_ap_calls(h, 1, d_llr, d_rec, d_nc, d_att, d_ev, d_evc, d_cl, d_ol, d_ac, d_apc, h->stream);
    HIPCHK(h, hipStreamSynchronize(h->stream));
    HIPCHK(h, hipMemcpy(records, d_rec, sizeof(ft8rx_record) * (size_t)n, hipMemcpyDeviceToHost));
    int32_t ne = 0;
    HIPCHK(h, hipMemcpy(&ne, d_evc, sizeof(int32_t), hipMemcpyDeviceToHost));
    if (event_count) *event_count = ne;
    if (events) HIPCHK(h, hipMemcpy(events, d_ev, sizeof(ft8rx_event) * (size_t)(ne < FT8RX_EVENT_CAP ? ne : FT8RX_EVENT_CAP), hipMemcpyDeviceToHost));
    return 0;
}

int ft8rx_recall_probe(ft8rx_handle* h, const float* sgrid, const ft8rx_recall_entry* entries, int n, ft8rx_record* records) {
    if (!h || !sgrid || !entries || !records || n < 1) { if (h) set_err(h, "ft8rx_recall_probe: bad arguments"); return -1; }
    ENTER(h);
    Scratch S{h};
    std::vector<ft8rx_recall_entry> st((size_t)n * FT8RX_RECALL_MAX);
    std::vector<int32_t> trip(3 * (size_t)n), off(n + 1), tout(5 * (size_t)n, 0);
    for (int i = 0; i < n; i++) {
        ft8rx_recall_entry E = entries[i];
        E.pad = (uint16_t)recall_kind(E.msg_lo, E.msg_hi);
        st[(size_t)i * FT8RX_RECALL_MAX] = E;
        trip[3 * i] = i; trip[3 * i + 1] = E.f0_idx; trip[3 * i + 2] = E.h0_idx; off[i] = i;
    }
    off[n] = n;
    float* d_sg = S.put(sgrid, (size_t)n * 632); NEED(d_sg);
    ft8rx_recall_entry* d_ent = S.put(st.data(), st.size()); NEED(d_ent);
    int32_t* d_trip = S.put(trip.data(), trip.size()); NEED(d_trip);
    int32_t* d_off = S.put(off.data(), off.size()); NEED(d_off);
    int32_t* d_tout = S.put(tout.data(), tout.size()); NEED(d_tout);
    ft8rx_record* d_rec = S.get<ft8rx_record>((size_t)n * FT8RX_RECALL_MAX); NEED(d_rec);
    HIPCHK(h, hipMemset(d_rec, 0, sizeof(ft8rx_record) * (size_t)n * FT8RX_RECALL_MAX));
    k_recall_score<<<n, 64, 0, h->stream>>>(d_sg, d_tout, d_trip, d_off, 0, d_ent, nullptr, nullptr, 0, h->rc_max_hd, h->rc_min_gap, d_rec);
    HIPCHK(h, hipStreamSynchronize(h->stream));
    HIPCHK(h, hipMemcpy2D(records, sizeof(ft8rx_record), d_rec, sizeof(ft8rx_record) * FT8RX_RECALL_MAX, sizeof(ft8rx_record), n, hipMemcpyDeviceToHost));
    return 0;
}

int ft8rx_report_probe(ft8rx_handle* h, const float* spec, int B, int n, const int32_t* frame, const int32_t* f0_idx, const int32_t* h0_idx,
                       const int32_t* ttweak, const int32_t* ftweak, const uint64_t* msg_lo, const uint64_t* msg_hi, ft8rx_report* reports) {
    if (!h || !spec || !frame || !f0_idx || !h0_idx || !ttweak || !ftweak || !msg_lo || !msg_hi || !reports || B < 1 || B > h->max_frames || n < 1) {
        if (h) set_err(h, "ft8rx_report_probe: bad arguments (1 <= n_frames <= max_frames, n >= 1)"); return -1; }
    const int sh = cand_shift(h->cfg); const size_t S = (size_t)1 << sh;
    std::vector<ft8rx_record> r0((size_t)B * S);
    memset(r0.data(), 0, sizeof(ft8rx_record) * r0.size());
    std::vector<int32_t> nc(B, 0), where(n);
    for (int i = 0; i < n; i++) {
        if (frame[i] < 0 || frame[i] >= B || f0_idx[i] < -32768 || f0_idx[i] > 32767 || h0_idx[i] < -32768 || h0_idx[i] > 32767 ||
            ttweak[i] < -128 || ttweak[i] > 127 || ftweak[i] < -128 || ftweak[i] > 127) {
            set_err(h, "ft8rx_report_probe: candidate %d (frame %d, f0 %d, h0 %d, tweaks %d / %d) is out of range", i, frame[i], f0_idx[i], h0_idx[i], ttweak[i], ftweak[i]); return -1; }
        if (nc[frame[i]] >= (int)S) { set_err(h, "ft8rx_report_probe: more than %zu candidates in frame %d", S, frame[i]); return -1; }
        where[i] = (int32_t)((size_t)frame[i] * S + nc[frame[i]]++);
        ft8rx_record& r = r0[where[i]];
        r.msg_lo = msg_lo[i]; r.msg_hi = msg_hi[i]; r.f0_idx = (int16_t)f0_idx[i]; r.h0_idx = (int16_t)h0_idx[i];
        r.ttweak = (int8_t)ttweak[i]; r.ftweak = (int8_t)ftweak[i]; r.status = FT8RX_ST_DECODED;
    }
    ENTER(h);
    HIPCHK(h, hipMemcpy(h->d_spec, spec, sizeof(cpx) * (size_t)B * FT8RX_SPEC_BINS, hipMemcpyHostToDevice));
    Scratch Sc{h};
    ft8rx_record* d_rec = Sc.put(r0.data(), r0.size()); NEED(d_rec);
    int32_t* d_nc = Sc.put(nc.data(), nc.size()); NEED(d_nc);
    int32_t* d_items = Sc.get<int32_t>((size_t)B * S); NEED(d_items);
    int32_t* d_count = Sc.get<int32_t>(1); NEED(d_count);
    ft8rx_report* d_rep = Sc.get<ft8rx_report>((size_t)B * S); NEED(d_rep);
    launch_reports(h, B, h->d_spec, d_rec, d_nc, d_items, d_count, d_rep, h->stream);
    HIPCHK(h, hipGetLastError());
    HIPCHK(h, hipStreamSynchronize(h->stream));
    std::vector<ft8rx_report> out((size_t)B * S);
    HIPCHK(h, hipMemcpy(out.data(), d_rep, sizeof(ft8rx_report) * out.size(), hipMemcpyDeviceToHost));
    for (int i = 0; i < n; i++) reports[i] = out[where[i]];
    return 0;
}

int ft8rx_osd_ext(ft8rx_handle* h, const float* llr, int n, int singleflips, int doubleflips, int tripleflips, int max_hd,
                  int32_t* ok, uint64_t* msg_lo, uint64_t* msg_hi, int32_t* trial, int32_t* hd) {
    if (!h || !llr || n < 1) return -1;
    if (singleflips < 0 || singleflips > OSD_MAXFLIP || doubleflips < 0 || doubleflips > OSD_MAXFLIP || tripleflips < 0 || tripleflips > 40 ||
        max_hd < 0 || max_hd > 174) { set_err(h, "ft8rx_osd: flip counts out of range"); return -1; }
    const std::vector<uint32_t> tr = osd_trial_table(singleflips, doubleflips, tripleflips);
    if (tr.size() > OSD_MAXTRIALS) { set_err(h, "ft8rx_osd: %zu trials exceed %d", tr.size(), OSD_MAXTRIALS); return -1; }
    ENTER(h);
    Scratch S{h};
    float* d_in = S.put(llr, (size_t)n * 174); NEED(d_in);
    uint32_t* d_tr = S.put(tr.data(), tr.size()); NEED(d_tr);
    Att* d_att = S.get<Att>(n); NEED(d_att);
    int32_t* d_nan = S.get<int32_t>((size_t)n + 1); NEED(d_nan);
    HIPCHK(h, hipMemsetAsync(d_nan, 0, sizeof(int32_t), h->stream));
    const WorkList nanl{d_nan + 1, d_nan};
    launch_osd(h, 0, n, h->stream, 2, d_in, nullptr, nullptr, nullptr, nullptr, d_att, nullptr, nullptr, d_tr, (int)tr.size(),
               osd_nflip(singleflips, tripleflips), max_hd, cand_shift(h->cfg), WorkList{nullptr, nullptr}, nanl);
    HIPCHK(h, hipStreamSynchronize(h->stream));
    std::vector<Att> a(n);
    HIPCHK(h, hipMemcpy(a.data(), d_att, sizeof(Att) * n, hipMemcpyDeviceToHost));
    for (int i = 0; i < n; i++) {
        ok[i] = a[i].ok; msg_lo[i] = a[i].lo; msg_hi[i] = a[i].hi; trial[i] = a[i].ok ? a[i].n_its : -1;
// ... 157 lines not shown
                                             decimated ? SUBD_D * SUBD_CH : SUB_CH);
    }
}
static void sub_apply_fullrate(ft8rx_handle* h, int B, const SubSel& sel, const SubTables& T) {
    k_sub_accum<<<dim3(SUB_GRIDX, B), 256, 0, h->stream>>>(h->d_wf, sel, T, h->d_part);
    k_sub_apply<<<dim3(SUB_GRIDX, B), 256, 0, h->stream>>>(h->d_wf, sel, T, h->d_part);
}

int ft8rx_subtract(ft8rx_handle* h, int16_t* d_audio, int B, ft8rx_subsig* sigs, const int32_t* counts, int max_sigs,
                   int refine, float* audio_f32_out) {
    if (!h || !d_audio || !sigs || !counts) return -1;
    if (B < 1 || B > h->max_frames || max_sigs < 1 || max_sigs > 256 || refine < 0 || refine > 3) { set_err(h, "ft8rx_subtract: bad n_frames / max_sigs / refine"); return -1; }
    ENTER(h);
    HIPCHK(h, hipStreamSynchronize(h->stream));
    if (subtract_workspaces(h, 0)) return -2;
    if (h->sig_cap < max_sigs) {
        ft8rx_subsig* p = nullptr;
        if (dalloc(h, &p, (size_t)h->max_frames * max_sigs)) return -2;
        h->d_sigs = p; h->sig_cap = max_sigs;
    }
    int nmax = 0;
    for (int f = 0; f < B; f++) {
        if (counts[f] < 0 || counts[f] > max_sigs) { set_err(h, "ft8rx_subtract: counts[%d] = %d outside [0, %d]", f, counts[f], max_sigs); return -1; }
        if (counts[f] > nmax) nmax = counts[f];
    }
    HIPCHK(h, hipMemcpyAsync(h->d_sigs, sigs, sizeof(ft8rx_subsig) * (size_t)B * max_sigs, hipMemcpyHostToDevice, h->stream));
    HIPCHK(h, hipMemcpyAsync(h->d_sigcnt, counts, sizeof(int32_t) * B, hipMemcpyHostToDevice, h->stream));
    const size_t n = (size_t)B * FT8RX_NSAMP;
    k_sub_to_f32<<<(unsigned)((n + 255) / 256), 256, 0, h->stream>>>(d_audio, h->d_wf, n);
    if (subtract_workspaces(h, refine)) return -2;
    const SubTables T{h->d_pulse, h->d_pc};
    Tables Tones = h->T;
    if (refine == 3) Tones.taper = h->d_ones;
    for (int s = 0; s < nmax; s++) {
        const SubSel sel{h->d_sigs, h->d_sigcnt, max_sigs, s};
        if (refine == 2) {
            k_subd_mix<<<dim3(SUBD_NZ / 256, B), 256, 0, h->stream>>>(h->d_wf, sel, h->d_zdec, h->d_subctx);
            sub_refine(h, B, sel, T, true);
            k_subd_model<<<dim3((SUBD_N + 255) / 256, B), 256, 0, h->stream>>>(sel, T, h->d_subctx, h->d_model);
            k_subd_accum<<<B, 256, 0, h->stream>>>(h->d_zdec, h->d_model, sel, h->d_subctx, h->d_adec);
            k_subd_apply<<<dim3(SUB_GRIDX, B), 256, 0, h->stream>>>(h->d_wf, sel, T, h->d_adec);
            continue;
        }
        if (refine == 1) sub_refine(h, B, sel, T, false);
        if (refine == 3) {
            k_cyc_a_f32<<<dim3(40, B), 256, 0, h->stream>>>(h->d_wf, h->d_A, h->T);
            k_cyc_bc<<<dim3(CYC_BC_GRID, B), 256, 0, h->stream>>>(h->d_A, h->d_spec, h->T);
            k_refine3<<<B, FINE_NT, 0, h->stream>>>(h->d_spec, sel, Tones);
        }
        sub_apply_fullrate(h, B, sel, T);
    }
    k_sub_to_i16<<<(unsigned)((n + 255) / 256), 256, 0, h->stream>>>(h->d_wf, d_audio, n);
    HIPCHK(h, hipGetLastError());
    if (audio_f32_out) HIPCHK(h, hipMemcpyAsync(audio_f32_out, h->d_wf, sizeof(float) * n, hipMemcpyDeviceToHost, h->stream));
    if (refine) HIPCHK(h, hipMemcpyAsync(sigs, h->d_sigs, sizeof(ft8rx_subsig) * (size_t)B * max_sigs, hipMemcpyDeviceToHost, h->stream));
    HIPCHK(h, hipStreamSynchronize(h->stream));
    return 0;
}

int ft8rx_encode_tones(const uint64_t* msg_lo, const uint64_t* msg_hi, int n, uint8_t* tones) {
    if (!msg_lo || !msg_hi || !tones || n < 0) return -1;
    for (int i = 0; i < n; i++) hostmsg::encode_tones(msg_lo[i], msg_hi[i], tones + (size_t)i * 79);
    return 0;
}

void* ft8rx_alloc_host(ft8rx_handle* h, uint64_t bytes) {
    if (!h || bytes == 0) return nullptr;
    void* p = nullptr;
    if (hipSetDevice(h->device) != hipSuccess || hipHostMalloc(&p, (size_t)bytes, hipHostMallocDefault) != hipSuccess) {
        set_err(h, "ft8rx_alloc_host: hipHostMalloc(%llu) failed", (unsigned long long)bytes);
        return nullptr;
    }
    return p;
}

int ft8rx_free_host(ft8rx_handle* h, void* p) {
    if (!p) return -1;
    const hipError_t e = hipHostFree(p);
    if (e != hipSuccess) { if (h) set_err(h, "hipHostFree failed: %s", hipGetErrorString(e)); return -2; }
    return 0;
}

int ft8rx_synth_frames_ex(ft8rx_handle* h, uint64_t seed, int first_index, int n_frames, int n_signals,
                          const void* signal_table, int signal_bytes, const double* pulse_cumsum, int16_t* d_audio, int no_noise) {
    if (!h || !signal_table || !pulse_cumsum || !d_audio || n_frames < 1 || n_signals < 0 || n_signals > 64) return -1;
    if (signal_bytes != (int)sizeof(SynthSig)) { set_err(h, "ft8rx_synth_frames: signal record is %d bytes, expected %d", signal_bytes, (int)sizeof(SynthSig)); return -1; }
    ENTER(h);
    Scratch S{h};
    SynthSig* d_s = S.put((const SynthSig*)signal_table, (size_t)n_frames * (n_signals ? n_signals : 1)); NEED(d_s);
    double* d_q = S.put(pulse_cumsum, 5761); NEED(d_q);
    k_synth<<<dim3((FT8RX_NSAMP / 4 + 255) / 256, n_frames), 256, 0, h->stream>>>(d_audio, d_s, n_signals, d_q, (uint32_t)seed, (uint32_t)(seed >> 32), first_index, no_noise);
    HIPCHK(h, hipStreamSynchronize(h->stream));
    return 0;
}

int ft8rx_synth_frames(ft8rx_handle* h, uint64_t seed, int first_index, int n_frames, int n_signals,
                       const void* signal_table, int signal_bytes, const double* pulse_cumsum, int16_t* d_audio) {
    return ft8rx_synth_frames_ex(h, seed, first_index, n_frames, n_signals, signal_table, signal_bytes, pulse_cumsum, d_audio, 0);
}

int ft8rx_package_batch(const ft8rx_record* records, const int32_t* counts, const ft8rx_event* events, const int32_t* event_counts,
                        int n_frames, int max_cands, ft8rx_message* out, int max_msgs, int32_t* out_counts, int n_threads,
                        ft8rx_hashes* table, int32_t* flags) {
    return hostmsg::package_batch(records, counts, events, event_counts, n_frames, max_cands, out, max_msgs, out_counts, n_threads,
                                  table ? &table->H : nullptr, flags);
}

int ft8rx_package_batch_ext(const ft8rx_record* records, const int32_t* counts, const ft8rx_event* events, const int32_t* event_counts,
                            int n_frames, int max_cands, ft8rx_message_ext* out, int max_msgs, int32_t* out_counts, int n_threads,
                            ft8rx_hashes* table, int32_t* flags, int32_t mask) {
    if (mask < 0 || mask > FT8RX_MT_ALL) return -1;
    return hostmsg::package_batch(records, counts, events, event_counts, n_frames, max_cands, out, max_msgs, out_counts, n_threads,
                                  table ? &table->H : nullptr, flags, (unsigned)mask);
}

int ft8rx_package_batch_recall(const ft8rx_record* records, const int32_t* counts, const ft8rx_event* events, const int32_t* event_counts,
                               const ft8rx_record* recall, const int32_t* recall_counts, int n_frames, int max_cands, ft8rx_message* out,
                               int max_msgs, int32_t* out_counts, int n_threads, ft8rx_hashes* table, int32_t* flags) {
    if (!recall || !recall_counts) return -1;
    return hostmsg::package_batch(records, counts, events, event_counts, n_frames, max_cands, out, max_msgs, out_counts, n_threads,
                                  table ? &table->H : nullptr, flags, 0u, recall, recall_counts);
}

int ft8rx_package_packed(const void* packed, uint64_t bytes, int frame_lo, int n_frames, ft8rx_message* out, int max_msgs,
                         int32_t* out_counts, int n_threads, ft8rx_hashes* table, int32_t* flags) {
    return hostmsg::package_packed(packed, bytes, frame_lo, n_frames, out, max_msgs, out_counts, n_threads, table ? &table->H : nullptr, flags);
}

int ft8rx_merge_messages(ft8rx_message* out, int32_t* out_counts, int max_out, const ft8rx_message* add, const int32_t* add_counts,
                         int max_add, int n_frames, int pass_tag, int drop_osd, ft8rx_message* fresh, int32_t* fresh_counts) {
    if (!out || !out_counts || !add || !add_counts || n_frames < 0 || max_out < 1 || max_add < 1) return -1;
    hostmsg::merge_messages(out, out_counts, max_out, add, add_counts, max_add, n_frames, pass_tag, drop_osd, fresh, fresh_counts);
    return 0;
}

int ft8rx_subtraction_list(const ft8rx_message* msgs, const int32_t* counts, int max_msgs, const ft8rx_record* records, int max_cands,
                           int n_frames, int min_snr, ft8rx_subsig* sigs, int max_sigs, int32_t* sig_counts) {
    if (!msgs || !counts || !records || !sigs || !sig_counts || n_frames < 0 || max_msgs < 1 || max_cands < 1 || max_sigs < 1) return -1;
    return hostmsg::subtraction_list(msgs, counts, max_msgs, records, max_cands, n_frames, min_snr, sigs, max_sigs, sig_counts);
}

ft8rx_hashes* ft8rx_hashes_create(void) { return new (std::nothrow) ft8rx_hashes(); }
void ft8rx_hashes_destroy(ft8rx_hashes* t) { delete t; }
int ft8rx_hashes_clear(ft8rx_hashes* t) { if (!t) return -1; t->H.clear(); return 0; }
int ft8rx_hashes_add(ft8rx_hashes* t, const char* call) { if (!t || !call) return -1; t->H.add(call); return 0; }
int ft8rx_hashes_size(const ft8rx_hashes* t) { return t ? (int)t->H.size() : -1; }

int ft8rx_set_reject_log(const char* path) { hostmsg::set_reject_log(path); return 0; }

#ifdef FINE_TIMING
int ft8rx_debug_fine_times(ft8rx_handle* h, unsigned long long* out32, int reset) {
    if (!h) return -1;
    ENTER(h);
    return ft8rx_ilp_fine_times(out32, reset);
}
#endif

#ifdef BP_TIMING
int ft8rx_debug_bp_times(ft8rx_handle* h, unsigned long long* out8, int reset) {
    if (!h) return -1;
    ENTER(h);
    if (hipDeviceSynchronize() != hipSuccess) return -2;
    std::vector<unsigned long long> all((size_t)65536 * 8);
    if (out8) {
        if (hipMemcpyFromSymbol(all.data(), HIP_SYMBOL(g_bp_t), sizeof(unsigned long long) * all.size()) != hipSuccess) return -2;
        for (int i = 0; i < 8; i++) out8[i] = 0;
        for (size_t b = 0; b < 65536; b++) for (int i = 0; i < 8; i++) out8[i] += all[b * 8 + i];
    }
    if (reset) { std::fill(all.begin(), all.end(), 0ull); if (hipMemcpyToSymbol(HIP_SYMBOL(g_bp_t), all.data(), sizeof(unsigned long long) * all.size()) != hipSuccess) return -2; }
    return 0;
}
#endif
#ifdef OSD_TIMING
int ft8rx_debug_osd_times(ft8rx_handle* h, unsigned long long* out16, int reset) {
    if (!h) return -1;
    ENTER(h);
    if (hipDeviceSynchronize() != hipSuccess) return -2;
    std::vector<unsigned long long> all((size_t)32768 * 10);
    if (out16) {
        if (hipMemcpyFromSymbol(all.data(), HIP_SYMBOL(g_osd_t), sizeof(unsigned long long) * all.size()) != hipSuccess) return -2;
        for (int i = 0; i < 16; i++) out16[i] = 0;
        for (size_t b = 0; b < 32768; b++) for (int i = 0; i < 10; i++) out16[i == 9 ? 15 : i] += all[b * 10 + i];
    }
    if (reset) { std::fill(all.begin(), all.end(), 0ull); if (hipMemcpyToSymbol(HIP_SYMBOL(g_osd_t), all.data(), sizeof(unsigned long long) * all.size()) != hipSuccess) return -2; }
    return 0;
}
#endif

int ft8rx_math_probe(ft8rx_handle* h, int which, const float* x, int n, float* y) {
    if (!h || !x || !y || n < 1) return -1;
    ENTER(h);
    Scratch S{h};
    if (which == 0 || which == 1) {
        float* d_x = S.put(x, n); NEED(d_x);
        float* d_y = S.get<float>(n); NEED(d_y);
        k_math_probe<<<(n + 255) / 256, 256, 0, h->stream>>>(which, d_x, d_y, n);
        HIPCHK(h, hipStreamSynchronize(h->stream));
        HIPCHK(h, hipMemcpy(y, d_y, sizeof(float) * n, hipMemcpyDeviceToHost));
        return 0;
    }
    if (which == 2) {
        cpx* d_x = S.put((const cpx*)x, n); NEED(d_x);
        cpx* d_y = S.get<cpx>(n); NEED(d_y);
        const size_t lds = 2 * (size_t)n * sizeof(cpx);
        if (n == 1920) k_fft_probe<1920, 8, 4, 4, 5, 3><<<1, 256, lds, h->stream>>>(d_x, d_y, h->T.W1920);
        else if (n == 3200) k_fft_probe<3200, 8, 4, 4, 5, 5><<<1, 256, lds, h->stream>>>(d_x, d_y, h->T.W3200);
        else if (n == 300) k_fft_probe<300, 5, 5, 4, 3><<<1, 256, lds, h->stream>>>(d_x, d_y, h->T.W300);
        else if (n == 320) k_fft_probe<320, 8, 8, 5><<<1, 256, lds, h->stream>>>(d_x, d_y, h->T.W320);
        else { set_err(h, "ft8rx_math_probe: no FFT plan of length %d", n); return -1; }
        HIPCHK(h, hipStreamSynchronize(h->stream));
        HIPCHK(h, hipMemcpy(y, d_y, sizeof(cpx) * n, hipMemcpyDeviceToHost));
        return 0;
    }
    return -1;
}

}
```

### pyft8_amd/csrc/ft8rx_ilp.hip

```cpp
#define FT8RX_ILP_UNIT 1
#include <hip/hip_runtime.h>
#include <math.h>
#include <stdint.h>
#include <string.h>
#include "../../include/ft8rx.h"
#include "ft8_dev.h"

#define NF0MAX (FT8RX_MAX_F0 > 1024 ? 2048 : 1024)

#include "kernels/common.hpp"
#include "kernels/spectrogram.hpp"
#include "kernels/llr.hpp"
#include "kernels/fine_sync.hpp"
#include "ilp_launch.hpp"

void ft8rx_ilp_spectrogram(int n_frames, hipStream_t s, const int16_t* audio, float* grid, const Tables& T) {
    k_spectrogram<<<dim3(376, n_frames), SPEC_NT, 0, s>>>(audio, grid, T);
}
void ft8rx_ilp_hop_spectrum(hipStream_t s, const int16_t* win3840, float* row, const Tables& T) {
    k_hop_spectrum<<<1, SPEC_NT, 0, s>>>(win3840, row, T);
}
void ft8rx_ilp_fine(int n_blocks, hipStream_t s, const cpx* spec, ft8rx_record* rec, const int32_t* ncand, float* llr0, const Tables& T,
                    const ft8rx_config& cfg, const int32_t* trip, int32_t* t_out, float* t_sd, float* t_sgrid, WorkList work) {
    k_fine<<<n_blocks, FINE_NT, 0, s>>>(spec, rec, ncand, llr0, T, cfg, trip, t_out, t_sd, t_sgrid, work);
}
#ifdef FINE_TIMING
int ft8rx_ilp_fine_times(unsigned long long* out32, int reset) {
    if (hipDeviceSynchronize() != hipSuccess) return -2;
    if (out32 && hipMemcpyFromSymbol(out32, HIP_SYMBOL(g_fine_t), sizeof(unsigned long long) * 32) != hipSuccess) return -2;
    if (reset) { unsigned long long z[32] = {0}; if (hipMemcpyToSymbol(HIP_SYMBOL(g_fine_t), z, sizeof(z)) != hipSuccess) return -2; }
    return 0;
}
#endif
```

### pyft8_amd/csrc/ilp_launch.hpp

```cpp
#ifndef FT8RX_ILP_LAUNCH_HPP
#define FT8RX_ILP_LAUNCH_HPP
void ft8rx_ilp_spectrogram(int n_frames, hipStream_t s, const int16_t* audio, float* grid, const Tables& T);
void ft8rx_ilp_hop_spectrum(hipStream_t s, const int16_t* win3840, float* row, const Tables& T);
void ft8rx_ilp_fine(int n_blocks, hipStream_t s, const cpx* spec, ft8rx_record* rec, const int32_t* ncand, float* llr0, const Tables& T,
                    const ft8rx_config& cfg, const int32_t* trip, int32_t* t_out, float* t_sd, float* t_sgrid, WorkList work);
#ifdef FINE_TIMING
int ft8rx_ilp_fine_times(unsigned long long* out32, int reset);
#endif
#endif
```

### pyft8_amd/csrc/kernels/fine_sync.hpp

```cpp
#ifndef FT8RX_FINE_SYNC_HPP
#define FT8RX_FINE_SYNC_HPP

#ifndef FINE_NT
#define FINE_NT 128
#endif
#ifndef FINE_WV
#define FINE_WV 3
#endif
#define FINE_INV 0.0003125f

#ifdef FINE_TIMING
__device__ unsigned long long g_fine_t[32];
#define FT_DECL __shared__ unsigned long long ft_l[32]; if (tid < 32) ft_l[tid] = 0; __syncthreads(); unsigned long long ft_prev = __builtin_readcyclecounter();
#define FT_ARG , unsigned long long& ft_prev, unsigned long long* ft_l
#define FT_PASS , ft_prev, ft_l
#define FT(i) do { if (tid == 0) { unsigned long long ft_now = __builtin_readcyclecounter(); ft_l[i] += ft_now - ft_prev; ft_prev = __builtin_readcyclecounter(); } } while (0)
#define FT_FLUSH do { __syncthreads(); if (tid < 32) atomicAdd(&g_fine_t[tid], ft_l[tid]); } while (0)
#else
#define FT_DECL
#define FT_ARG
#define FT_PASS
#define FT(i) do { } while (0)
#define FT_FLUSH do { } while (0)
#endif

#define FINE_SLICE 1064
FT8_DEV cpx fine_taper(cpx v, double t) { return make_float2((float)((double)v.x * t), (float)((double)v.y * t)); }
FT8_DEV cpx fine_conj(cpx v) { return make_float2(v.x, -v.y); }

FT8_DEV void dft8_in012(cpx* a) {
    const float h = 0.70710678f;
    const cpx a0 = a[0], a1 = a[1], a2 = a[2];
    const cpx e0 = cadd(a0, a2), e2 = csub(a0, a2);
    const cpx e1 = make_float2(a0.x + a2.y, a0.y - a2.x), e3 = make_float2(a0.x - a2.y, a0.y + a2.x);
    const cpx o1 = make_float2(h * (a1.x + a1.y), h * (a1.y - a1.x));
    const cpx o2 = make_float2(a1.y, -a1.x);
    const cpx o3 = make_float2(o1.y, -o1.x);
    a[0] = cadd(e0, a1); a[4] = csub(e0, a1);
    a[1] = cadd(e1, o1); a[5] = csub(e1, o1);
    a[2] = cadd(e2, o2); a[6] = csub(e2, o2);
    a[3] = cadd(e3, o3); a[7] = csub(e3, o3);
}
FT8_DEV void dft8_in017(cpx* a) {
    const float h = 0.70710678f;
    const cpx a0 = a[0], a1 = a[1], a7 = a[7];
    const cpx q0 = cadd(a1, a7), q2 = csub(a1, a7);
    const cpx q1 = make_float2(a1.x - a7.y, a1.y + a7.x), q3 = make_float2(a1.x + a7.y, a1.y - a7.x);
    const cpx o1 = make_float2(h * (q1.x + q1.y), h * (q1.y - q1.x));
    const cpx o2 = make_float2(q2.y, -q2.x);
    const cpx o3 = make_float2(h * (q3.y - q3.x), -(h * (q3.x + q3.y)));
    a[0] = cadd(a0, q0); a[4] = csub(a0, q0);
    a[1] = cadd(a0, o1); a[5] = csub(a0, o1);
    a[2] = cadd(a0, o2); a[6] = csub(a0, o2);
    a[3] = cadd(a0, o3); a[7] = csub(a0, o3);
}
static_assert(FINE_NT == 128, "fine_stage1 is written for 128 threads");
FT8_DEV void fine_stage1(const cpx* S, int fb, cpx* z, const cpx* __restrict__ W,
                         const double* __restrict__ taper, int tid FT_ARG) {
    const cpx zero = make_float2(0.0f, 0.0f);
    const cpx* s0 = S + fb + tid;
    const cpx* s7 = S + fb - 150 - 250 + tid;
    const cpx a00 = s0[0], a01 = s0[400];
    const cpx a10 = s0[128], a11 = s0[528];
    const cpx a20 = s0[256], a21 = s0[656];
    const bool r3 = tid < 16;
    const int t3 = r3 ? tid : 0;
    const cpx a30 = s0[384 + t3 - tid], a31 = s0[784 + t3 - tid];
    const bool has02 = tid < 50;
    const cpx a02r = s0[has02 ? 800 : 0];
    const double t02 = taper[has02 ? tid + 50 : 0];
    const bool has17 = tid >= 122;
    const cpx a17r = s7[has17 ? 128 : 250];
    const double t17 = taper[has17 ? tid - 122 : 0];
    const uint32_t m02 = has02 ? 0xFFFFFFFFu : 0u, m17 = has17 ? 0xFFFFFFFFu : 0u;
    const cpx a27r = s7[256];
    const bool tap21 = tid >= 94;
    const double t2 = taper[tap21 ? tid - 94 : tid + 6];
    const cpx a37r = s7[384 + t3 - tid];
    const double t31 = taper[34 + t3];
    const cpx t02v = fine_taper(a02r, t02), t17v = fine_taper(a17r, t17);
    const cpx a02 = make_float2(__uint_as_float(__float_as_uint(t02v.x) & m02), __uint_as_float(__float_as_uint(t02v.y) & m02));
    const cpx a17 = make_float2(__uint_as_float(__float_as_uint(t17v.x) & m17), __uint_as_float(__float_as_uint(t17v.y) & m17));
    const cpx sel2 = fine_taper(tap21 ? a21 : a27r, t2);
    const cpx b21 = tap21 ? sel2 : a21, a27 = tap21 ? a27r : sel2;
    const cpx b31 = fine_taper(a31, t31);
    cpx a[4][8];
#pragma unroll
    for (int i = 0; i < 4; i++)
#pragma unroll
        for (int j = 2; j < 7; j++) a[i][j] = zero;
    a[0][0] = fine_conj(a00); a[0][1] = fine_conj(a01); a[0][2] = fine_conj(a02); a[0][7] = zero;
    a[1][0] = fine_conj(a10); a[1][1] = fine_conj(a11); a[1][7] = fine_conj(a17);
    a[2][0] = fine_conj(a20); a[2][1] = fine_conj(b21); a[2][7] = fine_conj(a27);
    a[3][0] = fine_conj(a30); a[3][1] = fine_conj(b31); a[3][7] = fine_conj(a37r);
#pragma unroll
    for (int i = 0; i < 4; i++) {
        const int p = tid + 128 * i;
        const int pw = (i < 3) ? p : 384 + t3;
        cpx w[8];
#pragma unroll
        for (int j = 1; j < 8; j++) w[j] = W[j * pw];
        if (i == 0) dft8_in012(a[i]); else dft8_in017(a[i]);
#pragma unroll
        for (int j = 1; j < 8; j++) a[i][j] = cmul(a[i][j], w[j]);
        if (i < 3 || r3) {
#pragma unroll
            for (int j = 0; j < 8; j++) z[8 * p + j] = a[i][j];
        }
    }
    FT(1);
    __syncthreads();
    FT(2);
}
FT8_DEV void fine_stage2(cpx* z, const cpx* w400, int tid FT_ARG) {
    typedef Fused2<3200, 400, 8, 4, 4> F;
    constexpr int R = (F::groups + FINE_NT - 1) / FINE_NT;
    cpx a[R][4][4];
#pragma unroll
    for (int r = 0; r < R; r++) { const int g = tid + FINE_NT * r; if (g < F::groups) F::load_affine<200, 800>(z, g, a[r]); }
    FT(3);
    __syncthreads();
    FT(4);
#pragma unroll
    for (int r = 0; r < R; r++) {
        const int g = tid + FINE_NT * r;
        if (g < F::groups) {
            const int pp = g >> 3;
#pragma unroll
            for (int jp = 0; jp < 4; jp++) {
                dft<4>(a[r][jp]);
                const int pq = pp + 25 * jp;
#pragma unroll
                for (int j = 1; j < 4; j++) a[r][jp][j] = cmul(a[r][jp][j], w400[j * pq]);
            }
#pragma unroll
            for (int j = 0; j < 4; j++) {
                cpx b[4];
#pragma unroll
                for (int jp = 0; jp < 4; jp++) b[jp] = a[r][jp][j];
                dft<4>(b);
#pragma unroll
                for (int jp = 1; jp < 4; jp++) b[jp] = cmul(b[jp], w400[4 * jp * pp]);
#pragma unroll
                for (int jp = 0; jp < 4; jp++) a[r][jp][j] = b[jp];
            }
            F::store_affine<32, 8>(z, (g & 7) + 128 * (g >> 3), a[r]);
        }
    }
    FT(5);
    __syncthreads();
    FT(6);
}
FT8_DEV void fine_stage3(cpx* z, const cpx* __restrict__ W, int tid, int lo, int hi FT_ARG) {
    typedef Fused2<3200, 25, 128, 5, 5> F;
    constexpr int R = F::groups / FINE_NT;
    cpx a[R][5][5];
#pragma unroll
    for (int r = 0; r < R; r++) F::load_affine<128, 640>(z, tid + FINE_NT * r, a[r]);
    FT(7);
    __syncthreads();
    FT(8);
#pragma unroll
    for (int r = 0; r < R; r++) {
        const int q = tid + FINE_NT * r;
        F::compute_passA(0, a[r], W);
#pragma unroll
        for (int j = 0; j < 5; j++) {
            const int rr = q + 128 * j;
            const int first = rr + 640 * (lo / 640 + (rr < lo % 640 ? 1 : 0));
            if (first < hi && first < 3200) {
                cpx b[5];
#pragma unroll
                for (int jp = 0; jp < 5; jp++) b[jp] = a[r][jp][j];
                dft<5>(b);
#pragma unroll
                for (int jp = 0; jp < 5; jp++) z[rr + 640 * jp] = b[jp];
            }
        }
    }
    FT(9);
    __syncthreads();
    FT(10);
}
FT8_DEV void fine_fft(const cpx* S, int fb, cpx* z, const cpx* w400, const Tables& T, int tid, int lo, int hi FT_ARG) {
    FT(0);
    fine_stage1(S, fb, z, T.W3200, T.taper, tid FT_PASS);
    fine_stage2(z, w400, tid FT_PASS);
    fine_stage3(z, T.W3200, tid, lo, hi FT_PASS);
}

template <int NT>
FT8_DEV void fine_sym_quad(const cpx* z, int i0, int n2, const cpx* wq, float* mag) {
    if (i0 < 0) i0 = 0;
    if (i0 > 3168) i0 = 3168;
    cpx x[8];
#pragma unroll
    for (int n1 = 0; n1 < 8; n1++) { cpx v = z[i0 + 4 * n1 + n2]; x[n1] = make_float2(v.x * FINE_INV, -(v.y * FINE_INV)); }
    sym32_quad<NT>(x, n2, wq, mag);
}

#ifdef FT8RX_ILP_UNIT
#define FS_CS 0
#define FS_H 156
#define FS_MAG 1556
struct FsLane {
    float k[17];
    cpx g0[10];
    cpx g[10];
    double tap;
    cpx cs[2];
    int r, jlo;
};
FT8_DEV void fscore_fetch(FsLane& L, const Tables& T, int tid) {
    const int lane = tid & 63;
    const int ln = lane < 50 ? lane : 0;
    L.r = tid < 64 ? 50 + ln : ln;
    L.jlo = tid < 64 ? -2 : -1;
#pragma unroll
    for (int u = 0; u < 17; u++) L.k[u] = T.K32[900 + L.r + 100 * (L.jlo - 7 + u)];
#pragma unroll
    for (int q = 0; q < 10; q++) L.g0[q] = T.G1000[L.r + 100 * (L.jlo + q) + 150];
    L.tap = T.taper[tid < 64 ? ln : 50 + ln];
#pragma unroll
    for (int u = 0; u < 2; u++) { const int i = tid + FINE_NT * u; L.cs[u] = T.CS100[i < 156 ? i : 0]; }
}
FT8_DEV void fscore_phases(FsLane& L, const Tables& T, int nb0) {
    cpx w[10];
    {
        const int step = (((100 * nb0) % 3200) + 3200) % 3200;
        int idx = ((((L.r + 100 * L.jlo) * nb0) % 3200) + 3200) % 3200;
#pragma unroll
        for (int q = 0; q < 10; q++) { w[q] = T.W3200[idx]; idx += step; idx -= (idx >= 3200) ? 3200 : 0; }
    }
#pragma unroll
    for (int q = 0; q < 10; q++) L.g[q] = cmul(make_float2(w[q].x, -w[q].y), L.g0[q]);
}
FT8_DEV void fscore_prepare(FsLane& L, cpx* zi, const Tables& T, int nb0, int tid) {
    fscore_phases(L, T, nb0);
#pragma unroll
    for (int u = 0; u < 2; u++) { const int i = tid + FINE_NT * u; if (i < 156) zi[FS_CS + i] = L.cs[u]; }
    __syncthreads();
}
template <int NTONE>
FT8_DEV void fscore_p1(const cpx* S, int off, const FsLane& L, cpx* H, int tid FT_ARG) {
    cpx b[10];
#pragma unroll
    for (int q = 0; q < 10; q++) {
        cpx x = S[off + L.r + 100 * (L.jlo + q)];
        if (q == 0 || q == 9) x = fine_taper(x, L.tap);
        b[q] = cmul(x, L.g[q]);
    }
    FT(16);
    float hx[NTONE], hy[NTONE];
#pragma unroll
    for (int t = 0; t < NTONE; t++) { hx[t] = 0.0f; hy[t] = 0.0f; }
#pragma unroll
    for (int u = 0; u < 17; u++) {
#pragma unroll
        for (int t = 0; t < NTONE; t++) {
            const int q = u + t - 7;
            if (q >= 0 && q < 10) {
                hx[t] = __builtin_fmaf(b[q].x, L.k[u], hx[t]);
                hy[t] = __builtin_fmaf(b[q].y, L.k[u], hy[t]);
            }
        }
    }
    FT(17);
#pragma unroll
    for (int t = 0; t < NTONE; t++) H[t * 100 + L.r] = make_float2(hx[t], hy[t]);
}
FT8_DEV void dft10_fwd(const cpx* x, cpx* y) {
    cpx a0[5], a1[5];
#pragma unroll
    for (int n = 0; n < 5; n++) { const cpx u = x[(2 * n) % 10], v = x[(5 + 2 * n) % 10]; a0[n] = cadd(u, v); a1[n] = csub(u, v); }
    dft<5>(a0); dft<5>(a1);
#pragma unroll
    for (int k = 0; k < 5; k++) { y[(6 * k) % 10] = a0[k]; y[(5 + 6 * k) % 10] = a1[k]; }
}
FT8_DEV float row16_sum(float v) {
    v += __int_as_float(__builtin_amdgcn_update_dpp(0, __float_as_int(v), 0xB1, 0xf, 0xf, false));
    v += __int_as_float(__builtin_amdgcn_update_dpp(0, __float_as_int(v), 0x4E, 0xf, 0xf, false));
    v += __int_as_float(__builtin_amdgcn_update_dpp(0, __float_as_int(v), 0x141, 0xf, 0xf, false));
    v += __int_as_float(__builtin_amdgcn_update_dpp(0, __float_as_int(v), 0x140, 0xf, 0xf, false));
    return v;
}
FT8_DEV void fine_fscore(const cpx* S, int off, const FsLane& L, cpx* zi, int n, int tid FT_ARG) {
    cpx* H = zi + FS_H + (n & 1) * 700;
    float* mags = reinterpret_cast<float*>(zi + FS_MAG) + n * 56;
    const int lane = tid & 63;
    if (lane < 50) fscore_p1<7>(S, off, L, H, tid FT_PASS);
    FT(11);
    __syncthreads();
    FT(12);
    {
        const int c = tid & 15, t = tid >> 4;
        cpx acc[7];
#pragma unroll
        for (int s = 0; s < 7; s++) acc[s] = make_float2(0.0f, 0.0f);
        const cpx* Ht = H + (t < 7 ? t : 0) * 100;
#pragma unroll
        for (int i = 0; i < 2; i++) {
            const int p = c + 16 * i;
            if (i < 1 || c < 10) {
                const bool first = (i == 0 && c == 0), last = (i == 1 && c == 9);
                const cpx zero = make_float2(0.0f, 0.0f);
                const cpx h1 = Ht[p];
                cpx h2 = Ht[first ? 99 : 100 - p], h3 = Ht[50 - p], h4 = Ht[50 + p];
                if (first) { h2 = zero; h4 = zero; }
                if (last) { h3 = zero; h4 = zero; }
                const cpx P = make_float2(h1.x + h2.x, h1.y + h2.y), M = make_float2(h1.x - h2.x, h1.y - h2.y);
                const cpx P2 = make_float2(h3.x + h4.x, h3.y + h4.y), M2 = make_float2(h3.x - h4.x, h3.y - h4.y);
                const cpx A = make_float2(P.x + P2.x, P.y + P2.y), B = make_float2(P.x - P2.x, P.y - P2.y);
                const cpx C = make_float2(M.x - M2.x, M.y - M2.y), D = make_float2(M.x + M2.x, M.y + M2.y);
                acc[0] = cadd(acc[0], A);
#pragma unroll
                for (int s = 1; s < 7; s++) {
                    const cpx e = zi[FS_CS + (s - 1) * 26 + p];
                    const cpx X = (s & 1) ? B : A, Y = (s & 1) ? D : C;
                    acc[s].x = __builtin_fmaf(X.x, e.x, __builtin_fmaf(-Y.y, e.y, acc[s].x));
                    acc[s].y = __builtin_fmaf(X.y, e.x, __builtin_fmaf(Y.x, e.y, acc[s].y));
                }
            }
        }
        FT(19);
#pragma unroll
        for (int s = 0; s < 7; s++) { acc[s].x = row16_sum(acc[s].x); acc[s].y = row16_sum(acc[s].y); }
        {
            cpx v = acc[0];
#pragma unroll
            for (int s = 1; s < 7; s++) v = (c == s) ? acc[s] : v;
            const float re = v.x * FINE_INV, im = v.y * FINE_INV;
            mags[c < 7 ? c * 8 + t : 7] = sqrtf(re * re + im * im);
        }
    }
    FT(14);
}

FT8_DEV void fine_candidate(int tid, int bid, const cpx* __restrict__ spec, ft8rx_record* __restrict__ rec,
                            const int32_t* __restrict__ ncand, float* __restrict__ llr0, const Tables& T, const ft8rx_config& cfg,
                            const int32_t* __restrict__ trip, int32_t* __restrict__ t_out ,
                            float* __restrict__ t_sd, float* __restrict__ t_sgrid) {
    __shared__ cpx z[3200];
    __shared__ cpx w400[400];
    float* mg = reinterpret_cast<float*>(w400);
    static_assert(sizeof(cpx) * 400 >= sizeof(float) * 640, "mg overlays w400");
    __shared__ cpx w32[32];
    __shared__ float sc[16];
    __shared__ int ish[4];
    const int lane = tid & 63;
    int frame, ci = 0, f0, h0;
    if (trip) { frame = trip[3 * bid]; f0 = trip[3 * bid + 1]; h0 = trip[3 * bid + 2]; }
    else {
        frame = bid >> cand_shift(cfg); ci = bid & ((1 << cand_shift(cfg)) - 1);
        if (ci >= ncand[frame]) return;
        const ft8rx_record& r = rec[bid];
        if (r.status != FT8RX_ST_ACTIVE) return;
        f0 = r.f0_idx; h0 = r.h0_idx;
    }
    if (h0 < FT8RX_MIN_H0_FD || h0 > FT8RX_MAX_H0_FD) return;
    const cpx w32v = T.W32[tid & 31];
    const int fb0 = 50 * f0;
    {
        constexpr int NW = (400 + FINE_NT - 1) / FINE_NT;
        cpx wv[NW];
#pragma unroll
        for (int q = 0; q < NW; q++) { const int i = tid + FINE_NT * q; wv[q] = T.W3200[8 * (i < 400 ? i : 0)]; }
#pragma unroll
        for (int q = 0; q < NW; q++) { const int i = tid + FINE_NT * q; if (i < 400) w400[i] = wv[q]; }
        if (tid < 32) w32[tid] = w32v;
        __syncthreads();
    }
    const cpx* __restrict__ Sg = spec + (size_t)frame * FT8RX_SPEC_BINS + (fb0 - 182);
    FT_DECL
    cpx wq[8];
    sym32_twiddles(w32, tid & 3, wq);
    const int tb0 = 8 * h0 + (h0 < 0 ? 1 : 0);
    double* dsum = reinterpret_cast<double*>(mg);
    fine_fft(Sg, 182, z, w400, T, tid, tb0 - 8 + 32 * 36, tb0 + 6 + 32 * 43 FT_PASS);
    FsLane L;
    fscore_fetch(L, T, tid);
    const bool lowslice = tb0 >= 667;
    cpx* slice = z + (lowslice ? 0 : 2048);
    cpx* zi = z + (lowslice ? 1152 : 0);
    static_assert(9 * 128 <= 1152 && 2048 + 9 * 128 <= 3200 && 1152 + 1780 <= 3200 && 1780 <= 2048, "slice copy and scan tables share the image");
    {
        const int wv = tid >> 6, ln = tid & 63;
#pragma unroll
        for (int c = 0; c < 5; c++) {
            const int ch = wv + 2 * c;
            if (ch < 9)
                __builtin_amdgcn_global_load_lds((const __attribute__((address_space(1))) void*)(Sg + 128 * ch + 2 * ln),
                                                 (__attribute__((address_space(3))) void*)(slice + 128 * ch), 16, 0, 0);
        }
    }
    const cpx* S = slice;
    float* p = reinterpret_cast<float*>(slice);
    float* llr = p + 464;
    float* sq = llr + 176;
#pragma unroll 1
    for (int r = 0; r < (224 + FINE_NT - 1) / FINE_NT; r++) {
        const int task = tid + FINE_NT * r, qd = task >> 2, n2 = task & 3;
        const bool valid = qd < 56;
        const int ti = valid ? qd / 7 : 0, a = valid ? qd - 7 * ti : 0;
        float mag[8];
        fine_sym_quad<7>(z, tb0 - 8 + 2 * ti + 32 * (36 + a), n2, wq, mag);
#pragma unroll
        for (int b = 0; b < 7; b++) asm volatile("" :: "v"(mag[b]));
        if (valid && n2 == 0) {
            const int c = d_COSTAS[a];
            double off = 0.0, on = 0.0;
#pragma unroll
            for (int b = 0; b < 7; b++) { const double m = (double)mag[b]; on = (b == c) ? m : on; off += (b == c) ? 0.0 : m; }
            dsum[(ti * 7 + a) * 2] = on; dsum[(ti * 7 + a) * 2 + 1] = off;
        }
    }
    FT(25);
    __syncthreads();
    int tt = -8; float score_f0 = 0.0f;
    {
        const int ti = tid & 7;
        double s1 = 0.0, s2 = 0.0;
#pragma unroll
        for (int a = 0; a < 7; a++) { s1 += dsum[(ti * 7 + a) * 2]; s2 += dsum[(ti * 7 + a) * 2 + 1]; }
        const float sct = (float)(s1 + W6 * s2);
#pragma unroll
        for (int u = 0; u < 8; u++) {
            const float v = __int_as_float(__builtin_amdgcn_readlane(__float_as_int(sct), u));
            if (u == 0 || v > score_f0) { score_f0 = v; tt = -8 + 2 * u; }
        }
    }
    FT(26);
    float best = 0.0f; int ft = 0;
    __builtin_amdgcn_s_waitcnt(0x0F70);
    fscore_prepare(L, zi, T, tb0 + tt + 32 * 36, tid);
    FT(18);
#pragma unroll 1
    for (int n = 0; n < 8; n++) {
        fine_fscore(S, 182 - 32 + 8 * (n < 4 ? n : n + 1), L, zi, n, tid FT_PASS);
        FT(15);
    }
    __syncthreads();
    if (tid < 56) {
        const int n = tid / 7, a = tid - 7 * n, c = d_COSTAS[a];
        const float* mags = reinterpret_cast<const float*>(zi + FS_MAG) + n * 56 + a * 8;
        double off = 0.0, on = 0.0;
#pragma unroll
        for (int b = 0; b < 7; b++) { const double m = (double)mags[b]; on = (b == c) ? m : on; off += (b == c) ? 0.0 : m; }
        dsum[tid * 2] = on; dsum[tid * 2 + 1] = off;
    }
    __syncthreads();
    {
        const int n = tid & 7;
        double s1 = 0.0, s2 = 0.0;
#pragma unroll
        for (int a = 0; a < 7; a++) { s1 += dsum[(n * 7 + a) * 2]; s2 += dsum[(n * 7 + a) * 2 + 1]; }
        const float sct = (float)(s1 + W6 * s2);
#pragma unroll
        for (int i = 0; i < 9; i++) {
            const float v = (i == 4) ? score_f0 : __int_as_float(__builtin_amdgcn_readlane(__float_as_int(sct), i < 4 ? i : i - 1));
            if (i == 0 || v > best) { best = v; ft = -32 + 8 * i; }
        }
    }
    FT(20);
    const int tb = tb0 + tt;
    cpx* Hc = zi;
    cpx* Ab = zi + 800;
    {
        const int t = (tid < 80) ? tid / 10 : 0, c10 = (tid < 80) ? tid - 10 * t : 0;
        cpx tw[9];
#pragma unroll
        for (int s1 = 1; s1 < 10; s1++) tw[s1 - 1] = T.TW100[c10 * s1];
        fscore_phases(L, T, tb);
        if (lane < 50) fscore_p1<8>(S, 182 + ft, L, Hc, tid FT_PASS);
        __syncthreads();
        FT(21);
        if (tid < 80) {
            cpx x[10], y[10];
#pragma unroll
            for (int r1 = 0; r1 < 10; r1++) { const cpx h = Hc[t * 100 + 10 * r1 + c10]; x[r1] = make_float2(h.x, -h.y); }
            dft10_fwd(x, y);
            Ab[t * 100 + c10] = y[0];
#pragma unroll
            for (int s1 = 1; s1 < 10; s1++) Ab[t * 100 + 10 * s1 + c10] = cmul(y[s1], tw[s1 - 1]);
        }
        __syncthreads();
        FT(22);
        if (tid < 80) {
            cpx x[10], y[10];
#pragma unroll
            for (int r2 = 0; r2 < 10; r2++) x[r2] = Ab[t * 100 + 10 * c10 + r2];
            dft10_fwd(x, y);
#pragma unroll
            for (int s2 = 0; s2 < 8; s2++) {
                const int sy = c10 + 10 * s2;
                const float re = y[s2].x * FINE_INV, im = y[s2].y * FINE_INV;
                if (sy < 79) mg[sy * 8 + t] = sqrtf(re * re + im * im);
            }
        }
    }
    const int n_lo = (tb < 0) ? min(79, (-tb) / 32 + 1) : 0;
    const int s_strict = (tb > 3168) ? 0 : (3168 - tb) / 32 + 1;
    const int s_up = (s_strict < 79) ? max(0, (3168 - tb + 31) / 32) : 79;
    if (n_lo > 0 || s_up < 79) {
        __syncthreads();
        fscore_phases(L, T, n_lo > 0 ? 0 : 3168);
        if (lane < 50) fscore_p1<8>(S, 182 + ft, L, Hc, tid FT_PASS);
        __syncthreads();
        const int c = tid & 15, t = tid >> 4;
        float ax = 0.0f, ay = 0.0f;
#pragma unroll
        for (int i = 0; i < 7; i++) {
            if (i < 6 || c < 4) { const cpx h = Hc[t * 100 + c + 16 * i]; ax = ax + h.x; ay = ay + h.y; }
        }
        ax = row16_sum(ax); ay = row16_sum(ay);
        const float re = ax * FINE_INV, im = ay * FINE_INV;
        const float m = sqrtf(re * re + im * im);
        if (n_lo > 0) { for (int sy = c; sy < n_lo; sy += 16) mg[sy * 8 + t] = m; }
        else { for (int sy = s_up + c; sy < 79; sy += 16) mg[sy * 8 + t] = m; }
    }
    __syncthreads();
    FT(23);
    bool match = false;
    if (tid < 21) {
        int blk = tid / 7, a = tid - blk * 7;
        const float* q = mg + 8 * (36 * blk + a);
        int am = 0; for (int t = 1; t < 8; t++) if (q[t] > q[am]) am = t;
        match = (am == d_COSTAS[a]);
    }
    if (tid < 64) { int nm = __popcll(__ballot(match)); if (tid == 0) ish[1] = nm; }
    __syncthreads();
    const int nsync = ish[1];
    FT(24);
    if (trip && t_sgrid) for (int i = tid; i < 632; i += FINE_NT) t_sgrid[(size_t)bid * 632 + i] = mg[i];
    int ret = 1; float sd = 0.0f; int snr = 0;
    if (nsync <= 6) ret = 0;
    else {
        for (int i = tid; i < 464; i += FINE_NT) p[i] = 20.0f * ft8_log10f(mg[8 * (int)d_PAYSYM[i >> 3] + (i & 7)]);
        __syncthreads();
        llr_from_p(p, llr, sq, tid, tid < 64, &sd, &snr);
        if (tid == 0) { sc[10] = sd; ish[2] = snr; }
        __syncthreads();
        sd = sc[10]; snr = ish[2];
        if (sd <= cfg.llr_sd_min) ret = -1;
        float* out = llr0 + (size_t)bid * 174;
        for (int i = tid; i < 174; i += FINE_NT) out[i] = llr[i];
    }
    FT(13);
    FT_FLUSH;
    if (tid == 0) {
        if (trip) { int32_t* o = t_out + 5 * (size_t)bid; o[0] = ret; o[1] = tt; o[2] = ft; o[3] = nsync; o[4] = snr; t_sd[bid] = sd; }
        else {
            ft8rx_record& r = rec[bid];
            r.ttweak = (int8_t)tt; r.ftweak = (int8_t)ft; r.nsync = (uint8_t)nsync;
            if (ret == 0) r.status = FT8RX_ST_STOP_COSTAS;
            else { r.fine_sd = sd; r.snr_fine = (int8_t)snr; if (ret < 0) r.status = FT8RX_ST_STOP_FINE_SD; }
        }
    }
}


__global__ __launch_bounds__(FINE_NT, FINE_WV) void k_fine(const cpx* __restrict__ spec, ft8rx_record* __restrict__ rec,
                                                  const int32_t* __restrict__ ncand, float* __restrict__ llr0, Tables T, ft8rx_config cfg,
                                                  const int32_t* __restrict__ trip, int32_t* __restrict__ t_out ,
                                                  float* __restrict__ t_sd, float* __restrict__ t_sgrid, WorkList work) {
    if (trip) { fine_candidate(threadIdx.x, blockIdx.x, spec, rec, ncand, llr0, T, cfg, trip, t_out, t_sd, t_sgrid); return; }
    const int n = *work.count;
#ifndef FINE_RUN
#define FINE_RUN 256
#endif
    const int nu = (n + 8 * FINE_RUN - 1) / (8 * FINE_RUN) * (8 * FINE_RUN);
#pragma unroll 1
    for (int u = blockIdx.x; u < nu; u += gridDim.x) {
        const int x = u & 7, j = u >> 3;
        const int item = (j / FINE_RUN) * (8 * FINE_RUN) + x * FINE_RUN + (j % FINE_RUN);
        if (item >= n) continue;
        int tid = threadIdx.x;
        asm volatile("" : "+v"(tid));
        fine_candidate(tid, work.items[item], spec, rec, ncand, llr0, T, cfg, nullptr, nullptr, nullptr, nullptr);
        __syncthreads();
    }
}
#endif

#ifndef FT8RX_ILP_UNIT
FT8_DEV int fine_clamp_pos(int i0) { return i0 < 0 ? 0 : (i0 > 3168 ? 3168 : i0); }
FT8_DEV bool fine_cand(int bid, const ft8rx_record* __restrict__ rec, const int32_t* __restrict__ ncand, const ft8rx_config& cfg,
                       const int32_t* __restrict__ trip, int& frame, int& f0, int& h0) {
    if (trip) { frame = trip[3 * bid]; f0 = trip[3 * bid + 1]; h0 = trip[3 * bid + 2]; return true; }
    frame = bid >> cand_shift(cfg);
    if ((bid & ((1 << cand_shift(cfg)) - 1)) >= ncand[frame]) return false;
    const ft8rx_record& r = rec[bid];
    if (r.status != FT8RX_ST_ACTIVE) return false;
    f0 = r.f0_idx; h0 = r.h0_idx;
    return true;
}
FT8_DEV void fine_tables(const Tables& T, cpx* w400, cpx* w32, cpx* wq, int tid) {
    for (int i = tid; i < 400; i += FINE_NT) w400[i] = T.W3200[8 * i];
    if (tid < 32) w32[tid] = T.W32[tid];
    __syncthreads();
    sym32_twiddles(w32, tid & 3, wq);
}
FT8_DEV void fine_onoff(const float* mag, int a, double& on, double& off) {
    const int c = d_COSTAS[a];
    on = 0.0; off = 0.0;
#pragma unroll
    for (int b = 0; b < 7; b++) { const double m = (double)mag[b]; on = (b == c) ? m : on; off += (b == c) ? 0.0 : m; }
}
FT8_DEV void fine_grid_td(const cpx* z, int tb, const cpx* wq, float* mg, int tid) {
#pragma unroll 1
    for (int r = 0; r < (316 + FINE_NT - 1) / FINE_NT; r++) {
        const int task = tid + FINE_NT * r, sy = task >> 2, n2 = task & 3;
        const bool valid = sy < 79;
        float mag[8];
        fine_sym_quad<8>(z, tb + 32 * (valid ? sy : 0), n2, wq, mag);
        if (valid && n2 == 0) {
#pragma unroll
            for (int b = 0; b < 8; b++) mg[sy * 8 + b] = mag[b];
        }
    }
    __syncthreads();
}
FT8_DEV void fine_tail(const float* mg, int tt, int ft, int tid, int bid, ft8rx_record* __restrict__ rec, float* __restrict__ llr0,
                       const ft8rx_config& cfg, const int32_t* __restrict__ trip, int32_t* __restrict__ t_out, float* __restrict__ t_sd,
                       float* __restrict__ t_sgrid) {
    __shared__ float p[464], llr[176], sq[176], sd_sh;
    __shared__ int nsync_sh, snr_sh;
    bool match = false;
    if (tid < 21) {
        int blk = tid / 7, a = tid - blk * 7;
        const float* q = mg + 8 * (36 * blk + a);
        int am = 0; for (int t = 1; t < 8; t++) if (q[t] > q[am]) am = t;
        match = (am == d_COSTAS[a]);
    }
    if (tid < 64) { int nm = __popcll(__ballot(match)); if (tid == 0) nsync_sh = nm; }
    __syncthreads();
    const int nsync = nsync_sh;
    if (trip && t_sgrid) for (int i = tid; i < 632; i += FINE_NT) t_sgrid[(size_t)bid * 632 + i] = mg[i];
    int ret = 1; float sd = 0.0f; int snr = 0;
    if (nsync <= 6) ret = 0;
    else {
        for (int i = tid; i < 464; i += FINE_NT) p[i] = 20.0f * ft8_log10f(mg[8 * (int)d_PAYSYM[i >> 3] + (i & 7)]);
        __syncthreads();
        llr_from_p(p, llr, sq, tid, tid < 64, &sd, &snr);
        if (tid == 0) { sd_sh = sd; snr_sh = snr; }
        __syncthreads();
        sd = sd_sh; snr = snr_sh;
        if (sd <= cfg.llr_sd_min) ret = -1;
        float* out = llr0 + (size_t)bid * 174;
        for (int i = tid; i < 174; i += FINE_NT) out[i] = llr[i];
    }
    if (tid == 0) {
        if (trip) { int32_t* o = t_out + 5 * (size_t)bid; o[0] = ret; o[1] = tt; o[2] = ft; o[3] = nsync; o[4] = snr; t_sd[bid] = sd; }
        else {
            ft8rx_record& r = rec[bid];
            r.ttweak = (int8_t)tt; r.ftweak = (int8_t)ft; r.nsync = (uint8_t)nsync;
            if (ret == 0) r.status = FT8RX_ST_STOP_COSTAS;
            else { r.fine_sd = sd; r.snr_fine = (int8_t)snr; if (ret < 0) r.status = FT8RX_ST_STOP_FINE_SD; }
        }
    }
}

typedef void FineCandidate(int tid, int bid, const cpx* spec, ft8rx_record* rec, const int32_t* ncand, float* llr0, const Tables& T,
                           const ft8rx_config& cfg, const int32_t* trip, int32_t* t_out, float* t_sd, float* t_sgrid);
template <FineCandidate CAND>
FT8_DEV void fine_blocks(const cpx* __restrict__ spec, ft8rx_record* __restrict__ rec, const int32_t* __restrict__ ncand,
                         float* __restrict__ llr0, const Tables& T, const ft8rx_config& cfg, const int32_t* __restrict__ trip,
                         int32_t* __restrict__ t_out, float* __restrict__ t_sd, float* __restrict__ t_sgrid, const WorkList& work) {
    if (trip) { CAND(threadIdx.x, blockIdx.x, spec, rec, ncand, llr0, T, cfg, trip, t_out, t_sd, t_sgrid); return; }
    const int n = *work.count;
#pragma unroll 1
    for (int item = blockIdx.x; item < n; item += gridDim.x) {
        CAND(threadIdx.x, work.items[item], spec, rec, ncand, llr0, T, cfg, nullptr, nullptr, nullptr, nullptr);
        __syncthreads();
    }
}

FT8_DEV void fine_td_candidate(int tid, int bid, const cpx* __restrict__ spec, ft8rx_record* __restrict__ rec,
                               const int32_t* __restrict__ ncand, float* __restrict__ llr0, const Tables& T, const ft8rx_config& cfg,
                               const int32_t* __restrict__ trip, int32_t* __restrict__ t_out, float* __restrict__ t_sd, float* __restrict__ t_sgrid) {
    __shared__ cpx z[3200];
    __shared__ cpx w400[400];
    __shared__ cpx w32[32];
    __shared__ float mg[640];
    __shared__ double dsum[8 * 7 * 2];
    int frame, f0, h0;
    if (!fine_cand(bid, rec, ncand, cfg, trip, frame, f0, h0)) return;
    if (h0 >= FT8RX_MIN_H0_FD && h0 <= FT8RX_MAX_H0_FD) return;
    cpx wq[8];
    fine_tables(T, w400, w32, wq, tid);
    const cpx* __restrict__ Sg = spec + (size_t)frame * FT8RX_SPEC_BINS + (50 * f0 - 182);
    const int tb0 = 8 * h0 + (h0 < 0 ? 1 : 0);
    fine_fft(Sg, 182, z, w400, T, tid, fine_clamp_pos(tb0 - 8 + 32 * 36), fine_clamp_pos(tb0 + 6 + 32 * 42) + 32);
#pragma unroll 1
    for (int r = 0; r < (224 + FINE_NT - 1) / FINE_NT; r++) {
        const int task = tid + FINE_NT * r, qd = task >> 2, n2 = task & 3;
        const bool valid = qd < 56;
        const int ti = valid ? qd / 7 : 0, a = valid ? qd - 7 * ti : 0;
        float mag[8];
        fine_sym_quad<7>(z, tb0 - 8 + 2 * ti + 32 * (36 + a), n2, wq, mag);
        if (valid && n2 == 0) { double on, off; fine_onoff(mag, a, on, off); dsum[(ti * 7 + a) * 2] = on; dsum[(ti * 7 + a) * 2 + 1] = off; }
    }
    __syncthreads();
    int tt = -8; float score_f0 = 0.0f;
    for (int u = 0; u < 8; u++) {
        double s1 = 0.0, s2 = 0.0;
        for (int a = 0; a < 7; a++) { s1 += dsum[(u * 7 + a) * 2]; s2 += dsum[(u * 7 + a) * 2 + 1]; }
        const float v = (float)(s1 + W6 * s2);
        if (u == 0 || v > score_f0) { score_f0 = v; tt = -8 + 2 * u; }
    }
    float best = 0.0f; int ft = 0;
    const int tb = tb0 + tt;
#pragma unroll 1
    for (int i = 0; i < 9; i++) {
        const int f = -32 + 8 * i;
        float v = score_f0;
        if (f != 0) {
            __syncthreads();
            fine_fft(Sg, 182 + f, z, w400, T, tid, fine_clamp_pos(tb + 32 * 36), fine_clamp_pos(tb + 32 * 42) + 32);
            {
                const int a = tid >> 2, n2 = tid & 3;
                const bool valid = a < 7;
                float mag[8];
                fine_sym_quad<7>(z, tb + 32 * (36 + (valid ? a : 0)), n2, wq, mag);
                if (valid && n2 == 0) { double on, off; fine_onoff(mag, a, on, off); dsum[a * 2] = on; dsum[a * 2 + 1] = off; }
            }
            __syncthreads();
            double s1 = 0.0, s2 = 0.0;
            for (int a = 0; a < 7; a++) { s1 += dsum[a * 2]; s2 += dsum[a * 2 + 1]; }
            v = (float)(s1 + W6 * s2);
        }
        if (i == 0 || v > best) { best = v; ft = f; }
    }
    __syncthreads();
    fine_fft(Sg, 182 + ft, z, w400, T, tid, 0, 3200);
    fine_grid_td(z, tb, wq, mg, tid);
    fine_tail(mg, tt, ft, tid, bid, rec, llr0, cfg, trip, t_out, t_sd, t_sgrid);
}
__global__ __launch_bounds__(FINE_NT) void k_fine_td(const cpx* __restrict__ spec, ft8rx_record* __restrict__ rec,
                                                     const int32_t* __restrict__ ncand, float* __restrict__ llr0, Tables T, ft8rx_config cfg,
                                                     const int32_t* __restrict__ trip, int32_t* __restrict__ t_out,
                                                     float* __restrict__ t_sd, float* __restrict__ t_sgrid, WorkList work) {
    fine_blocks<fine_td_candidate>(spec, rec, ncand, llr0, T, cfg, trip, t_out, t_sd, t_sgrid, work);
}

#define FW_NT 15
#define FW_NTT 17
FT8_DEV void fine_weak_candidate(int tid, int bid, const cpx* __restrict__ spec, ft8rx_record* __restrict__ rec,
                                 const int32_t* __restrict__ ncand, float* __restrict__ llr0, const Tables& T, const ft8rx_config& cfg,
// ... 58 lines not shown
```

Before: 88740.

## Split fine sync kernel into time-sync and frequency-domain kernels with handoff buffer

Splits the monolithic fine-sync kernel into two launches. The first runs the FFT and Costas time-offset search and writes the best time offset and score per candidate into a new FineHand buffer. A second kernel, launched with its own occupancy bound and a smaller shared-memory layout, reads that handoff and performs frequency scoring, demodulation and LLR output. Several per-lane register arrays are moved to local temporaries to cut register pressure. The intent is higher occupancy for each phase, at the cost of an extra launch and a global round trip for the handoff.

```diff
diff --git a/pyft8_amd/csrc/ft8rx.hip b/pyft8_amd/csrc/ft8rx.hip
--- a/pyft8_amd/csrc/ft8rx.hip
+++ b/pyft8_amd/csrc/ft8rx.hip
@@ -100,6 +100,7 @@
     int32_t rc_max_hd = FT8RX_RECALL_MAX_HD_DEFAULT, rc_min_gap = FT8RX_RECALL_MIN_GAP_DEFAULT;
     ft8rx_recall_entry* d_rc_src = nullptr; int32_t* d_rc_srccnt = nullptr; int32_t* d_rc_off = nullptr;
     int32_t* d_rc_trip = nullptr; int32_t* d_rc_tout = nullptr; float* d_rc_tsd = nullptr; float* d_rc_sgrid = nullptr; float* d_rc_llr = nullptr;
+    FineHand* d_rc_hand = nullptr;
     bool reports = false;
     int32_t* d_rp_items = nullptr; int32_t* d_rp_count = nullptr;
     int sub_frames = FT8RX_SUBBATCH_DEFAULT;
@@ -119,6 +120,7 @@
     float* d_best_score = nullptr; int32_t* d_best_h0 = nullptr;
     ft8rx_record* d_rec = nullptr; int32_t* d_ncand = nullptr; ft8rx_event* d_ev = nullptr; int32_t* d_evcount = nullptr;
     float* d_llr0 = nullptr; float* d_saved = nullptr;
+    FineHand* d_fine_hand = nullptr;
     Att *d_att0 = nullptr, *d_attG = nullptr, *d_attB = nullptr, *d_attO = nullptr;
     cpx *d_A = nullptr, *d_spec = nullptr;
     const uint32_t* d_trials = nullptr; int n_trials = 0;
@@ -383,6 +385,7 @@
     rc |= dalloc(h, &h->d_rec, B * S);
     rc |= dalloc(h, &h->d_ncand, B);
     rc |= dalloc(h, &h->d_llr0, B * S * 174);
+    rc |= dalloc(h, &h->d_fine_hand, B * S);
     rc |= dalloc(h, &h->d_saved, B * S * 5 * 174);
     rc |= dalloc(h, &h->d_att0, B * S * 5);
     rc |= dalloc(h, &h->d_attG, B * S * 2);
@@ -568,9 +571,10 @@
 }
 static void launch_fine(ft8rx_handle* h, const ft8rx_config& cfg, bool weak, int n_blocks, hipStream_t s, const cpx* spec, ft8rx_record* rec,
                         const int32_t* ncand, float* llr, const int32_t* trip, int32_t* t_out, float* t_sd, float* t_sgrid, WorkList work,
-                        bool need_td) {
+                        FineHand* hand, bool need_td) {
     if (weak) { k_fine_weak<<<n_blocks, FINE_NT, 0, s>>>(spec, rec, ncand, llr, h->T, cfg, trip, t_out, t_sd, t_sgrid, work); return; }
-    ft8rx_ilp_fine(n_blocks, s, spec, rec, ncand, llr, h->T, cfg, trip, t_out, t_sd, t_sgrid, work);
+    ft8rx_ilp_fine(n_blocks, s, spec, rec, ncand, h->T, cfg, trip, work, hand);
+    k_fine_fd<<<n_blocks, FINE_NT, 0, s>>>(spec, rec, ncand, llr, h->T, cfg, trip, t_out, t_sd, t_sgrid, work, hand);
     if (need_td) k_fine_td<<<n_blocks, FINE_NT, 0, s>>>(spec, rec, ncand, llr, h->T, cfg, trip, t_out, t_sd, t_sgrid, work);
 }
 
@@ -647,7 +651,7 @@
     k_cyc_bc<<<dim3(CYC_BC_GRID, B), 256, 0, s>>>(A, spec, h->T);
     STAGE("fine");
     launch_fine(h, c, weak, ladder_grid(h, B * c.max_cands), s, spec, rec, ncand, llr0, nullptr, nullptr, nullptr, nullptr, wl[WL_FINE],
-                c.h0_lo < FT8RX_MIN_H0_FD || c.h0_hi > FT8RX_MAX_H0_FD + 1);
+                h->d_fine_hand + FS, c.h0_lo < FT8RX_MIN_H0_FD || c.h0_hi > FT8RX_MAX_H0_FD + 1);
     k_worklist<<<(B * S + 255) / 256, 256, 0, s>>>(rec, ncand, B, sh, wl[WL_BP1]);
     STAGE("bp_fine");
     const auto bp_fine = [&](int n_variants, const WorkList& work, int v0) {
@@ -691,7 +695,7 @@
             k_recall_trip<<<B, FT8RX_RECALL_MAX, 0, s>>>(ent, rcnt, h->d_rc_off + F, h->d_rc_trip);
             const size_t b = (size_t)base;
             launch_fine(h, c, false, n, s, spec, nullptr, nullptr, h->d_rc_llr + b * 174, h->d_rc_trip + 3 * b, h->d_rc_tout + 5 * b,
-                        h->d_rc_tsd + b, h->d_rc_sgrid + b * 632, WorkList{nullptr, nullptr}, h->rc_td);
+                        h->d_rc_tsd + b, h->d_rc_sgrid + b * 632, WorkList{nullptr, nullptr}, h->d_rc_hand + b, h->rc_td);
             k_recall_score<<<n, 64, 0, s>>>(h->d_rc_sgrid, h->d_rc_tout, h->d_rc_trip, h->d_rc_off + F, base, ent, rec, ncand, sh,
                                             h->rc_max_hd, h->rc_min_gap, sl.d_rc_rec + F * FT8RX_RECALL_MAX);
         }
@@ -1000,7 +1004,7 @@
     FirstUse F(h, WS_RECALL);
     F.dev(&h->d_rc_src, N); F.dev(&h->d_rc_srccnt, B); F.dev(&h->d_rc_off, B + 1);
     F.dev(&h->d_rc_trip, N * 3); F.dev(&h->d_rc_tout, N * 5); F.dev(&h->d_rc_tsd, N);
-    F.dev(&h->d_rc_sgrid, N * 632); F.dev(&h->d_rc_llr, N * 174);
+    F.dev(&h->d_rc_sgrid, N * 632); F.dev(&h->d_rc_llr, N * 174); F.dev(&h->d_rc_hand, N);
     for (ResultSlot& sl : h->slots) {
         F.dev(&sl.d_rc_ent, N); F.dev(&sl.d_rc_cnt, B); F.dev(&sl.d_rc_rec, N);
         F.host(&sl.h_rc_rec, N); F.host(&sl.h_rc_cnt, B);
@@ -1701,8 +1705,9 @@
     float* d_sd = S.get<float>(n); NEED(d_sd);
     int32_t* d_out = S.get<int32_t>((size_t)n * 5); NEED(d_out);
     float* d_sg = sgrid ? S.get<float>((size_t)n * 632) : nullptr; if (sgrid) NEED(d_sg);
+    FineHand* d_hand = S.get<FineHand>(n); NEED(d_hand);
     launch_fine(h, weak ? weak_config(h) : h->cfg, weak, n, h->stream, h->d_spec, nullptr, nullptr, d_llr, d_trip, d_out, d_sd, d_sg,
-                WorkList{nullptr, nullptr}, true);
+                WorkList{nullptr, nullptr}, d_hand, true);
     HIPCHK(h, hipStreamSynchronize(h->stream));
     std::vector<int32_t> o((size_t)n * 5);
     HIPCHK(h, hipMemcpy(o.data(), d_out, sizeof(int32_t) * o.size(), hipMemcpyDeviceToHost));
@@ -2166,7 +2171,12 @@
 int ft8rx_debug_fine_times(ft8rx_handle* h, unsigned long long* out32, int reset) {
     if (!h) return -1;
     ENTER(h);
-    return ft8rx_ilp_fine_times(out32, reset);
+    unsigned long long ts[32] = {0}, fd[32] = {0};
+    if (ft8rx_ilp_fine_times(ts, reset)) return -2;
+    if (hipMemcpyFromSymbol(fd, HIP_SYMBOL(g_fine_fd_t), sizeof(fd)) != hipSuccess) return -2;
+    if (reset) { unsigned long long z[32] = {0}; if (hipMemcpyToSymbol(HIP_SYMBOL(g_fine_fd_t), z, sizeof(z)) != hipSuccess) return -2; }
+    if (out32) for (int i = 0; i < 32; i++) out32[i] = ts[i] + fd[i];
+    return 0;
 }
 #endif
 
diff --git a/pyft8_amd/csrc/ft8rx_ilp.hip b/pyft8_amd/csrc/ft8rx_ilp.hip
--- a/pyft8_amd/csrc/ft8rx_ilp.hip
+++ b/pyft8_amd/csrc/ft8rx_ilp.hip
@@ -20,9 +20,9 @@
 void ft8rx_ilp_hop_spectrum(hipStream_t s, const int16_t* win3840, float* row, const Tables& T) {
     k_hop_spectrum<<<1, SPEC_NT, 0, s>>>(win3840, row, T);
 }
-void ft8rx_ilp_fine(int n_blocks, hipStream_t s, const cpx* spec, ft8rx_record* rec, const int32_t* ncand, float* llr0, const Tables& T,
-                    const ft8rx_config& cfg, const int32_t* trip, int32_t* t_out, float* t_sd, float* t_sgrid, WorkList work) {
-    k_fine<<<n_blocks, FINE_NT, 0, s>>>(spec, rec, ncand, llr0, T, cfg, trip, t_out, t_sd, t_sgrid, work);
+void ft8rx_ilp_fine(int n_blocks, hipStream_t s, const cpx* spec, const ft8rx_record* rec, const int32_t* ncand, const Tables& T,
+                    const ft8rx_config& cfg, const int32_t* trip, WorkList work, FineHand* hand) {
+    k_fine<<<n_blocks, FINE_NT, 0, s>>>(spec, rec, ncand, T, cfg, trip, work, hand);
 }
 #ifdef FINE_TIMING
 int ft8rx_ilp_fine_times(unsigned long long* out32, int reset) {
diff --git a/pyft8_amd/csrc/ilp_launch.hpp b/pyft8_amd/csrc/ilp_launch.hpp
--- a/pyft8_amd/csrc/ilp_launch.hpp
+++ b/pyft8_amd/csrc/ilp_launch.hpp
@@ -2,8 +2,8 @@
 #define FT8RX_ILP_LAUNCH_HPP
 void ft8rx_ilp_spectrogram(int n_frames, hipStream_t s, const int16_t* audio, float* grid, const Tables& T);
 void ft8rx_ilp_hop_spectrum(hipStream_t s, const int16_t* win3840, float* row, const Tables& T);
-void ft8rx_ilp_fine(int n_blocks, hipStream_t s, const cpx* spec, ft8rx_record* rec, const int32_t* ncand, float* llr0, const Tables& T,
-                    const ft8rx_config& cfg, const int32_t* trip, int32_t* t_out, float* t_sd, float* t_sgrid, WorkList work);
+void ft8rx_ilp_fine(int n_blocks, hipStream_t s, const cpx* spec, const ft8rx_record* rec, const int32_t* ncand, const Tables& T,
+                    const ft8rx_config& cfg, const int32_t* trip, WorkList work, FineHand* hand);
 #ifdef FINE_TIMING
 int ft8rx_ilp_fine_times(unsigned long long* out32, int reset);
 #endif
diff --git a/pyft8_amd/csrc/kernels/fine_sync.hpp b/pyft8_amd/csrc/kernels/fine_sync.hpp
--- a/pyft8_amd/csrc/kernels/fine_sync.hpp
+++ b/pyft8_amd/csrc/kernels/fine_sync.hpp
@@ -7,21 +7,41 @@
 #ifndef FINE_WV
 #define FINE_WV 3
 #endif
+#ifndef FINE_FD_WV
+#define FINE_FD_WV 4
+#endif
 #define FINE_INV 0.0003125f
 
-#ifdef FINE_TIMING
+#define FT_ON_DECL __shared__ unsigned long long ft_l[32]; if (tid < 32) ft_l[tid] = 0; __syncthreads(); unsigned long long ft_prev = __builtin_readcyclecounter();
+#define FT_ON_MARK(i) do { if (tid == 0) { unsigned long long ft_now = __builtin_readcyclecounter(); ft_l[i] += ft_now - ft_prev; ft_prev = __builtin_readcyclecounter(); } } while (0)
+#define FT_ON_FLUSH(arr) do { __syncthreads(); if (tid < 32) atomicAdd(&arr[tid], ft_l[tid]); } while (0)
+#if defined(FINE_TIMING) && defined(FT8RX_ILP_UNIT)
 __device__ unsigned long long g_fine_t[32];
-#define FT_DECL __shared__ unsigned long long ft_l[32]; if (tid < 32) ft_l[tid] = 0; __syncthreads(); unsigned long long ft_prev = __builtin_readcyclecounter();
+#define FT_DECL FT_ON_DECL
 #define FT_ARG , unsigned long long& ft_prev, unsigned long long* ft_l
 #define FT_PASS , ft_prev, ft_l
-#define FT(i) do { if (tid == 0) { unsigned long long ft_now = __builtin_readcyclecounter(); ft_l[i] += ft_now - ft_prev; ft_prev = __builtin_readcyclecounter(); } } while (0)
-#define FT_FLUSH do { __syncthreads(); if (tid < 32) atomicAdd(&g_fine_t[tid], ft_l[tid]); } while (0)
+#define FT(i) FT_ON_MARK(i)
+#define FT_FLUSH FT_ON_FLUSH(g_fine_t)
 #else
 #define FT_DECL
 #define FT_ARG
 #define FT_PASS
 #define FT(i) do { } while (0)
 #define FT_FLUSH do { } while (0)
+#endif
+#if defined(FINE_TIMING) && !defined(FT8RX_ILP_UNIT)
+__device__ unsigned long long g_fine_fd_t[32];
+#define FD_DECL FT_ON_DECL
+#define FD_ARG , unsigned long long& ft_prev, unsigned long long* ft_l
+#define FD_PASS , ft_prev, ft_l
+#define FDT(i) FT_ON_MARK(i)
+#define FD_FLUSH FT_ON_FLUSH(g_fine_fd_t)
+#else
+#define FD_DECL
+#define FD_ARG
+#define FD_PASS
+#define FDT(i) do { } while (0)
+#define FD_FLUSH do { } while (0)
 #endif
 
 #define FINE_SLICE 1064
@@ -199,16 +219,124 @@
     sym32_quad<NT>(x, n2, wq, mag);
 }
 
+typedef int2 FineHand;
+FT8_DEV bool fine_cand(int bid, const ft8rx_record* __restrict__ rec, const int32_t* __restrict__ ncand, const ft8rx_config& cfg,
+                       const int32_t* __restrict__ trip, int& frame, int& f0, int& h0) {
+    if (trip) { frame = trip[3 * bid]; f0 = trip[3 * bid + 1]; h0 = trip[3 * bid + 2]; return true; }
+    frame = bid >> cand_shift(cfg);
+    if ((bid & ((1 << cand_shift(cfg)) - 1)) >= ncand[frame]) return false;
+    const ft8rx_record& r = rec[bid];
+    if (r.status != FT8RX_ST_ACTIVE) return false;
+    f0 = r.f0_idx; h0 = r.h0_idx;
+    return true;
+}
+FT8_DEV bool fine_fd_cand(int bid, const ft8rx_record* __restrict__ rec, const int32_t* __restrict__ ncand, const ft8rx_config& cfg,
+                          const int32_t* __restrict__ trip, int& frame, int& f0, int& h0) {
+    return fine_cand(bid, rec, ncand, cfg, trip, frame, f0, h0) && h0 >= FT8RX_MIN_H0_FD && h0 <= FT8RX_MAX_H0_FD;
+}
+#ifndef FINE_RUN
+#define FINE_RUN 256
+#endif
+FT8_DEV int fine_units(int n) { return (n + 8 * FINE_RUN - 1) / (8 * FINE_RUN) * (8 * FINE_RUN); }
+FT8_DEV int fine_item(int u) {
+    const int x = u & 7, j = u >> 3;
+    return (j / FINE_RUN) * (8 * FINE_RUN) + x * FINE_RUN + (j % FINE_RUN);
+}
+
 #ifdef FT8RX_ILP_UNIT
+FT8_DEV void fine_ts_candidate(int tid, int bid, const cpx* __restrict__ spec, const ft8rx_record* __restrict__ rec,
+                               const int32_t* __restrict__ ncand, const Tables& T, const ft8rx_config& cfg,
+                               const int32_t* __restrict__ trip, FineHand* __restrict__ hand) {
+    __shared__ cpx z[3200];
+    __shared__ cpx w400[400];
+    double* dsum = reinterpret_cast<double*>(w400);
+    static_assert(sizeof(cpx) * 400 >= sizeof(double) * 112, "dsum overlays w400");
+    __shared__ cpx w32[32];
+    int frame, f0, h0;
+    if (!fine_fd_cand(bid, rec, ncand, cfg, trip, frame, f0, h0)) return;
+    const cpx w32v = T.W32[tid & 31];
+    const int fb0 = 50 * f0;
+    {
+        constexpr int NW = (400 + FINE_NT - 1) / FINE_NT;
+        cpx wv[NW];
+#pragma unroll
+        for (int q = 0; q < NW; q++) { const int i = tid + FINE_NT * q; wv[q] = T.W3200[8 * (i < 400 ? i : 0)]; }
+#pragma unroll
+        for (int q = 0; q < NW; q++) { const int i = tid + FINE_NT * q; if (i < 400) w400[i] = wv[q]; }
+        if (tid < 32) w32[tid] = w32v;
+        __syncthreads();
+    }
+    const cpx* __restrict__ Sg = spec + (size_t)frame * FT8RX_SPEC_BINS + (fb0 - 182);
+    FT_DECL
+    cpx wq[8];
+    sym32_twiddles(w32, tid & 3, wq);
+    const int tb0 = 8 * h0 + (h0 < 0 ? 1 : 0);
+    fine_fft(Sg, 182, z, w400, T, tid, tb0 - 8 + 32 * 36, tb0 + 6 + 32 * 43 FT_PASS);
+#pragma unroll 1
+    for (int r = 0; r < (224 + FINE_NT - 1) / FINE_NT; r++) {
+        const int task = tid + FINE_NT * r, qd = task >> 2, n2 = task & 3;
+        const bool valid = qd < 56;
+        const int ti = valid ? qd / 7 : 0, a = valid ? qd - 7 * ti : 0;
+        float mag[8];
+        fine_sym_quad<7>(z, tb0 - 8 + 2 * ti + 32 * (36 + a), n2, wq, mag);
+#pragma unroll
+        for (int b = 0; b < 7; b++) asm volatile("" :: "v"(mag[b]));
+        if (valid && n2 == 0) {
+            const int c = d_COSTAS[a];
+            double off = 0.0, on = 0.0;
+#pragma unroll
+            for (int b = 0; b < 7; b++) { const double m = (double)mag[b]; on = (b == c) ? m : on; off += (b == c) ? 0.0 : m; }
+            dsum[(ti * 7 + a) * 2] = on; dsum[(ti * 7 + a) * 2 + 1] = off;
+        }
+    }
+    FT(25);
+    __syncthreads();
+    int tt = -8; float score_f0 = 0.0f;
+    {
+        const int ti = tid & 7;
+        double s1 = 0.0, s2 = 0.0;
+#pragma unroll
+        for (int a = 0; a < 7; a++) { s1 += dsum[(ti * 7 + a) * 2]; s2 += dsum[(ti * 7 + a) * 2 + 1]; }
+        const float sct = (float)(s1 + W6 * s2);
+#pragma unroll
+        for (int u = 0; u < 8; u++) {
+            const float v = __int_as_float(__builtin_amdgcn_readlane(__float_as_int(sct), u));
+            if (u == 0 || v > score_f0) { score_f0 = v; tt = -8 + 2 * u; }
+        }
+    }
+    FT(26);
+    FT_FLUSH;
+    if (tid == 0) hand[bid] = make_int2(tt, __float_as_int(score_f0));
+}
+
+__global__ __launch_bounds__(FINE_NT, FINE_WV) void k_fine(const cpx* __restrict__ spec, const ft8rx_record* __restrict__ rec,
+                                                  const int32_t* __restrict__ ncand, Tables T, ft8rx_config cfg,
+                                                  const int32_t* __restrict__ trip, WorkList work, FineHand* __restrict__ hand) {
+    if (trip) { fine_ts_candidate(threadIdx.x, blockIdx.x, spec, rec, ncand, T, cfg, trip, hand); return; }
+    const int n = *work.count;
+    const int nu = fine_units(n);
+#pragma unroll 1
+    for (int u = blockIdx.x; u < nu; u += gridDim.x) {
+        const int item = fine_item(u);
+        if (item >= n) continue;
+        int tid = threadIdx.x;
+        asm volatile("" : "+v"(tid));
+        fine_ts_candidate(tid, work.items[item], spec, rec, ncand, T, cfg, nullptr, hand);
+        __syncthreads();
+    }
+}
+#endif
+
+#ifndef FT8RX_ILP_UNIT
+#define FD_NH (FINE_FD_WV >= 4 ? 1 : 2)
 #define FS_CS 0
 #define FS_H 156
-#define FS_MAG 1556
+#define FS_MAG (FS_H + 700 * FD_NH)
+#define FD_ZI (FS_MAG + 224 > 800 ? FS_MAG + 224 : 800)
 struct FsLane {
     float k[17];
-    cpx g0[10];
     cpx g[10];
     double tap;
-    cpx cs[2];
     int r, jlo;
 };
 FT8_DEV void fscore_fetch(FsLane& L, const Tables& T, int tid) {
@@ -218,14 +346,12 @@
     L.jlo = tid < 64 ? -2 : -1;
 #pragma unroll
     for (int u = 0; u < 17; u++) L.k[u] = T.K32[900 + L.r + 100 * (L.jlo - 7 + u)];
-#pragma unroll
-    for (int q = 0; q < 10; q++) L.g0[q] = T.G1000[L.r + 100 * (L.jlo + q) + 150];
     L.tap = T.taper[tid < 64 ? ln : 50 + ln];
-#pragma unroll
-    for (int u = 0; u < 2; u++) { const int i = tid + FINE_NT * u; L.cs[u] = T.CS100[i < 156 ? i : 0]; }
 }
 FT8_DEV void fscore_phases(FsLane& L, const Tables& T, int nb0) {
-    cpx w[10];
+    cpx w[10], g0[10];
+#pragma unroll
+    for (int q = 0; q < 10; q++) g0[q] = T.G1000[L.r + 100 * (L.jlo + q) + 150];
     {
         const int step = (((100 * nb0) % 3200) + 3200) % 3200;
         int idx = ((((L.r + 100 * L.jlo) * nb0) % 3200) + 3200) % 3200;
@@ -233,16 +359,19 @@
         for (int q = 0; q < 10; q++) { w[q] = T.W3200[idx]; idx += step; idx -= (idx >= 3200) ? 3200 : 0; }
     }
 #pragma unroll
-    for (int q = 0; q < 10; q++) L.g[q] = cmul(make_float2(w[q].x, -w[q].y), L.g0[q]);
+    for (int q = 0; q < 10; q++) L.g[q] = cmul(make_float2(w[q].x, -w[q].y), g0[q]);
 }
 FT8_DEV void fscore_prepare(FsLane& L, cpx* zi, const Tables& T, int nb0, int tid) {
+    cpx cs[2];
+#pragma unroll
+    for (int u = 0; u < 2; u++) { const int i = tid + FINE_NT * u; cs[u] = T.CS100[i < 156 ? i : 0]; }
     fscore_phases(L, T, nb0);
 #pragma unroll
-    for (int u = 0; u < 2; u++) { const int i = tid + FINE_NT * u; if (i < 156) zi[FS_CS + i] = L.cs[u]; }
+    for (int u = 0; u < 2; u++) { const int i = tid + FINE_NT * u; if (i < 156) zi[FS_CS + i] = cs[u]; }
     __syncthreads();
 }
 template <int NTONE>
-FT8_DEV void fscore_p1(const cpx* S, int off, const FsLane& L, cpx* H, int tid FT_ARG) {
+FT8_DEV void fscore_p1(const cpx* S, int off, const FsLane& L, cpx* H, int tid FD_ARG) {
     cpx b[10];
 #pragma unroll
     for (int q = 0; q < 10; q++) {
@@ -250,7 +379,7 @@
         if (q == 0 || q == 9) x = fine_taper(x, L.tap);
         b[q] = cmul(x, L.g[q]);
     }
-    FT(16);
+    FDT(16);
     float hx[NTONE], hy[NTONE];
 #pragma unroll
     for (int t = 0; t < NTONE; t++) { hx[t] = 0.0f; hy[t] = 0.0f; }
@@ -265,7 +394,7 @@
             }
         }
     }
-    FT(17);
+    FDT(17);
 #pragma unroll
     for (int t = 0; t < NTONE; t++) H[t * 100 + L.r] = make_float2(hx[t], hy[t]);
 }
@@ -284,14 +413,15 @@
     v += __int_as_float(__builtin_amdgcn_update_dpp(0, __float_as_int(v), 0x140, 0xf, 0xf, false));
     return v;
 }
-FT8_DEV void fine_fscore(const cpx* S, int off, const FsLane& L, cpx* zi, int n, int tid FT_ARG) {
-    cpx* H = zi + FS_H + (n & 1) * 700;
+FT8_DEV void fine_fscore(const cpx* S, int off, const FsLane& L, cpx* zi, int n, int tid FD_ARG) {
+    cpx* H = zi + FS_H + (FD_NH == 2 ? (n & 1) * 700 : 0);
+    if (FD_NH == 1 && n > 0) __syncthreads();
     float* mags = reinterpret_cast<float*>(zi + FS_MAG) + n * 56;
     const int lane = tid & 63;
-    if (lane < 50) fscore_p1<7>(S, off, L, H, tid FT_PASS);
-    FT(11);
-    __syncthreads();
-    FT(12);
+    if (lane < 50) fscore_p1<7>(S, off, L, H, tid FD_PASS);
+    FDT(11);
+    __syncthreads();
+    FDT(12);
     {
         const int c = tid & 15, t = tid >> 4;
         cpx acc[7];
@@ -322,7 +452,7 @@
                 }
             }
         }
-        FT(19);
+        FDT(19);
 #pragma unroll
         for (int s = 0; s < 7; s++) { acc[s].x = row16_sum(acc[s].x); acc[s].y = row16_sum(acc[s].y); }
         {
@@ -333,111 +463,57 @@
             mags[c < 7 ? c * 8 + t : 7] = sqrtf(re * re + im * im);
         }
     }
-    FT(14);
-}
-
-FT8_DEV void fine_candidate(int tid, int bid, const cpx* __restrict__ spec, ft8rx_record* __restrict__ rec,
-                            const int32_t* __restrict__ ncand, float* __restrict__ llr0, const Tables& T, const ft8rx_config& cfg,
-                            const int32_t* __restrict__ trip, int32_t* __restrict__ t_out ,
-                            float* __restrict__ t_sd, float* __restrict__ t_sgrid) {
-    __shared__ cpx z[3200];
-    __shared__ cpx w400[400];
-    float* mg = reinterpret_cast<float*>(w400);
-    static_assert(sizeof(cpx) * 400 >= sizeof(float) * 640, "mg overlays w400");
-    __shared__ cpx w32[32];
+    FDT(14);
+}
+
+
+FT8_DEV void fine_fd_candidate(int tid, int bid, const cpx* __restrict__ spec, ft8rx_record* __restrict__ rec,
+                               const int32_t* __restrict__ ncand, float* __restrict__ llr0, const Tables& T, const ft8rx_config& cfg,
+                               const int32_t* __restrict__ trip, int32_t* __restrict__ t_out ,
+                               float* __restrict__ t_sd, float* __restrict__ t_sgrid, const FineHand* __restrict__ hand) {
+    __shared__ __attribute__((aligned(16))) cpx slice[FINE_SLICE];
+    __shared__ cpx zi[FD_ZI];
+    __shared__ __attribute__((aligned(8))) float mg[640];
     __shared__ float sc[16];
     __shared__ int ish[4];
+    static_assert((sizeof(cpx) * (FINE_SLICE + FD_ZI) + sizeof(float) * (640 + 16) + sizeof(int) * 4) * (FINE_FD_WV >= 4 ? 8 : 6) <= 160 * 1024,
+                  "k_fine_fd: eight (six) blocks per CU");
     const int lane = tid & 63;
-    int frame, ci = 0, f0, h0;
-    if (trip) { frame = trip[3 * bid]; f0 = trip[3 * bid + 1]; h0 = trip[3 * bid + 2]; }
-    else {
-        frame = bid >> cand_shift(cfg); ci = bid & ((1 << cand_shift(cfg)) - 1);
-        if (ci >= ncand[frame]) return;
-        const ft8rx_record& r = rec[bid];
-        if (r.status != FT8RX_ST_ACTIVE) return;
-        f0 = r.f0_idx; h0 = r.h0_idx;
-    }
-    if (h0 < FT8RX_MIN_H0_FD || h0 > FT8RX_MAX_H0_FD) return;
-    const cpx w32v = T.W32[tid & 31];
+    int frame, f0, h0;
+    if (!fine_fd_cand(bid, rec, ncand, cfg, trip, frame, f0, h0)) return;
+    const FineHand hv = hand[bid];
     const int fb0 = 50 * f0;
-    {
-        constexpr int NW = (400 + FINE_NT - 1) / FINE_NT;
-        cpx wv[NW];
-#pragma unroll
-        for (int q = 0; q < NW; q++) { const int i = tid + FINE_NT * q; wv[q] = T.W3200[8 * (i < 400 ? i : 0)]; }
-#pragma unroll
-        for (int q = 0; q < NW; q++) { const int i = tid + FINE_NT * q; if (i < 400) w400[i] = wv[q]; }
-        if (tid < 32) w32[tid] = w32v;
-        __syncthreads();
-    }
     const cpx* __restrict__ Sg = spec + (size_t)frame * FT8RX_SPEC_BINS + (fb0 - 182);
-    FT_DECL
-    cpx wq[8];
-    sym32_twiddles(w32, tid & 3, wq);
+    FD_DECL
     const int tb0 = 8 * h0 + (h0 < 0 ? 1 : 0);
     double* dsum = reinterpret_cast<double*>(mg);
-    fine_fft(Sg, 182, z, w400, T, tid, tb0 - 8 + 32 * 36, tb0 + 6 + 32 * 43 FT_PASS);
+    {
+        const int wv = tid >> 6;
+#pragma unroll
+        for (int c = 0; c < 5; c++) {
+            const int ch = wv + 2 * c;
+            if (ch < 8 || (ch == 8 && lane < (FINE_SLICE - 1024) / 2))
+                __builtin_amdgcn_global_load_lds((const __attribute__((address_space(1))) void*)(Sg + 128 * ch + 2 * lane),
+                                                 (__attribute__((address_space(3))) void*)(slice + 128 * ch), 16, 0, 0);
+        }
+    }
+    static_assert(FINE_SLICE > 1024 && FINE_SLICE <= 1152 && FINE_SLICE % 2 == 0, "slice copy: eight whole chunks and a part");
     FsLane L;
     fscore_fetch(L, T, tid);
-    const bool lowslice = tb0 >= 667;
-    cpx* slice = z + (lowslice ? 0 : 2048);
-    cpx* zi = z + (lowslice ? 1152 : 0);
-    static_assert(9 * 128 <= 1152 && 2048 + 9 * 128 <= 3200 && 1152 + 1780 <= 3200 && 1780 <= 2048, "slice copy and scan tables share the image");
-    {
-        const int wv = tid >> 6, ln = tid & 63;
-#pragma unroll
-        for (int c = 0; c < 5; c++) {
-            const int ch = wv + 2 * c;
-            if (ch < 9)
-                __builtin_amdgcn_global_load_lds((const __attribute__((address_space(1))) void*)(Sg + 128 * ch + 2 * ln),
-                                                 (__attribute__((address_space(3))) void*)(slice + 128 * ch), 16, 0, 0);
-        }
-    }
     const cpx* S = slice;
     float* p = reinterpret_cast<float*>(slice);
     float* llr = p + 464;
     float* sq = llr + 176;
-#pragma unroll 1
-    for (int r = 0; r < (224 + FINE_NT - 1) / FINE_NT; r++) {
-        const int task = tid + FINE_NT * r, qd = task >> 2, n2 = task & 3;
-        const bool valid = qd < 56;
-        const int ti = valid ? qd / 7 : 0, a = valid ? qd - 7 * ti : 0;
-        float mag[8];
-        fine_sym_quad<7>(z, tb0 - 8 + 2 * ti + 32 * (36 + a), n2, wq, mag);
-#pragma unroll
-        for (int b = 0; b < 7; b++) asm volatile("" :: "v"(mag[b]));
-        if (valid && n2 == 0) {
-            const int c = d_COSTAS[a];
-            double off = 0.0, on = 0.0;
-#pragma unroll
-            for (int b = 0; b < 7; b++) { const double m = (double)mag[b]; on = (b == c) ? m : on; off += (b == c) ? 0.0 : m; }
-            dsum[(ti * 7 + a) * 2] = on; dsum[(ti * 7 + a) * 2 + 1] = off;
-        }
-    }
-    FT(25);
-    __syncthreads();
-    int tt = -8; float score_f0 = 0.0f;
-    {
-        const int ti = tid & 7;
-        double s1 = 0.0, s2 = 0.0;
-#pragma unroll
-        for (int a = 0; a < 7; a++) { s1 += dsum[(ti * 7 + a) * 2]; s2 += dsum[(ti * 7 + a) * 2 + 1]; }
-        const float sct = (float)(s1 + W6 * s2);
-#pragma unroll
-        for (int u = 0; u < 8; u++) {
-            const float v = __int_as_float(__builtin_amdgcn_readlane(__float_as_int(sct), u));
-            if (u == 0 || v > score_f0) { score_f0 = v; tt = -8 + 2 * u; }
-        }
-    }
-    FT(26);
+    static_assert(464 + 176 + 176 <= 2 * FINE_SLICE, "p, llr, sq overlay the slice");
+    const int tt = hv.x; const float score_f0 = __int_as_float(hv.y);
     float best = 0.0f; int ft = 0;
     __builtin_amdgcn_s_waitcnt(0x0F70);
     fscore_prepare(L, zi, T, tb0 + tt + 32 * 36, tid);
-    FT(18);
+    FDT(18);
 #pragma unroll 1
     for (int n = 0; n < 8; n++) {
-        fine_fscore(S, 182 - 32 + 8 * (n < 4 ? n : n + 1), L, zi, n, tid FT_PASS);
-        FT(15);
+        fine_fscore(S, 182 - 32 + 8 * (n < 4 ? n : n + 1), L, zi, n, tid FD_PASS);
+        FDT(15);
     }
     __syncthreads();
     if (tid < 56) {
@@ -461,19 +537,19 @@
             if (i == 0 || v > best) { best = v; ft = -32 + 8 * i; }
         }
     }
-    FT(20);
+    FDT(20);
     const int tb = tb0 + tt;
     cpx* Hc = zi;
-    cpx* Ab = zi + 800;
+    cpx* Ab = Hc;
     {
         const int t = (tid < 80) ? tid / 10 : 0, c10 = (tid < 80) ? tid - 10 * t : 0;
+        fscore_phases(L, T, tb);
+        if (lane < 50) fscore_p1<8>(S, 182 + ft, L, Hc, tid FD_PASS);
         cpx tw[9];
 #pragma unroll
         for (int s1 = 1; s1 < 10; s1++) tw[s1 - 1] = T.TW100[c10 * s1];
-        fscore_phases(L, T, tb);
-        if (lane < 50) fscore_p1<8>(S, 182 + ft, L, Hc, tid FT_PASS);
-        __syncthreads();
-        FT(21);
+        __syncthreads();
+        FDT(21);
         if (tid < 80) {
             cpx x[10], y[10];
 #pragma unroll
@@ -484,7 +560,7 @@
             for (int s1 = 1; s1 < 10; s1++) Ab[t * 100 + 10 * s1 + c10] = cmul(y[s1], tw[s1 - 1]);
         }
         __syncthreads();
-        FT(22);
+        FDT(22);
         if (tid < 80) {
             cpx x[10], y[10];
 #pragma unroll
@@ -504,7 +580,7 @@
     if (n_lo > 0 || s_up < 79) {
         __syncthreads();
         fscore_phases(L, T, n_lo > 0 ? 0 : 3168);
-        if (lane < 50) fscore_p1<8>(S, 182 + ft, L, Hc, tid FT_PASS);
+        if (lane < 50) fscore_p1<8>(S, 182 + ft, L, Hc, tid FD_PASS);
         __syncthreads();
         const int c = tid & 15, t = tid >> 4;
         float ax = 0.0f, ay = 0.0f;
@@ -519,7 +595,7 @@
         else { for (int sy = s_up + c; sy < 79; sy += 16) mg[sy * 8 + t] = m; }
     }
     __syncthreads();
-    FT(23);
+    FDT(23);
     bool match = false;
     if (tid < 21) {
         int blk = tid / 7, a = tid - blk * 7;
@@ -530,7 +606,7 @@
     if (tid < 64) { int nm = __popcll(__ballot(match)); if (tid == 0) ish[1] = nm; }
     __syncthreads();
     const int nsync = ish[1];
-    FT(24);
+    FDT(24);
     if (trip && t_sgrid) for (int i = tid; i < 632; i += FINE_NT) t_sgrid[(size_t)bid * 632 + i] = mg[i];
     int ret = 1; float sd = 0.0f; int snr = 0;
     if (nsync <= 6) ret = 0;
@@ -545,8 +621,8 @@
         float* out = llr0 + (size_t)bid * 174;
         for (int i = tid; i < 174; i += FINE_NT) out[i] = llr[i];
     }
-    FT(13);
-    FT_FLUSH;
+    FDT(13);
+    FD_FLUSH;
     if (tid == 0) {
         if (trip) { int32_t* o = t_out + 5 * (size_t)bid; o[0] = ret; o[1] = tt; o[2] = ft; o[3] = nsync; o[4] = snr; t_sd[bid] = sd; }
         else {
@@ -558,42 +634,26 @@
     }
 }
 
-
-__global__ __launch_bounds__(FINE_NT, FINE_WV) void k_fine(const cpx* __restrict__ spec, ft8rx_record* __restrict__ rec,
-                                                  const int32_t* __restrict__ ncand, float* __restrict__ llr0, Tables T, ft8rx_config cfg,
-                                                  const int32_t* __restrict__ trip, int32_t* __restrict__ t_out ,
-                                                  float* __restrict__ t_sd, float* __restrict__ t_sgrid, WorkList work) {
-    if (trip) { fine_candidate(threadIdx.x, blockIdx.x, spec, rec, ncand, llr0, T, cfg, trip, t_out, t_sd, t_sgrid); return; }
+__global__ __launch_bounds__(FINE_NT, FINE_FD_WV) void k_fine_fd(const cpx* __restrict__ spec, ft8rx_record* __restrict__ rec,
+                                                        const int32_t* __restrict__ ncand, float* __restrict__ llr0, Tables T, ft8rx_config cfg,
+                                                        const int32_t* __restrict__ trip, int32_t* __restrict__ t_out ,
+                                                        float* __restrict__ t_sd, float* __restrict__ t_sgrid, WorkList work,
+                                                        const FineHand* __restrict__ hand) {
+    if (trip) { fine_fd_candidate(threadIdx.x, blockIdx.x, spec, rec, ncand, llr0, T, cfg, trip, t_out, t_sd, t_sgrid, hand); return; }
     const int n = *work.count;
-#ifndef FINE_RUN
-#define FINE_RUN 256
-#endif
-    const int nu = (n + 8 * FINE_RUN - 1) / (8 * FINE_RUN) * (8 * FINE_RUN);
+    const int nu = fine_units(n);
 #pragma unroll 1
     for (int u = blockIdx.x; u < nu; u += gridDim.x) {
-        const int x = u & 7, j = u >> 3;
-        const int item = (j / FINE_RUN) * (8 * FINE_RUN) + x * FINE_RUN + (j % FINE_RUN);
+        const int item = fine_item(u);
         if (item >= n) continue;
         int tid = threadIdx.x;
         asm volatile("" : "+v"(tid));
-        fine_candidate(tid, work.items[item], spec, rec, ncand, llr0, T, cfg, nullptr, nullptr, nullptr, nullptr);
-        __syncthreads();
-    }
-}
-#endif
-
-#ifndef FT8RX_ILP_UNIT
+        fine_fd_candidate(tid, work.items[item], spec, rec, ncand, llr0, T, cfg, nullptr, nullptr, nullptr, nullptr, hand);
+        __syncthreads();
+    }
+}
+
 FT8_DEV int fine_clamp_pos(int i0) { return i0 < 0 ? 0 : (i0 > 3168 ? 3168 : i0); }
-FT8_DEV bool fine_cand(int bid, const ft8rx_record* __restrict__ rec, const int32_t* __restrict__ ncand, const ft8rx_config& cfg,
-                       const int32_t* __restrict__ trip, int& frame, int& f0, int& h0) {
-    if (trip) { frame = trip[3 * bid]; f0 = trip[3 * bid + 1]; h0 = trip[3 * bid + 2]; return true; }
-    frame = bid >> cand_shift(cfg);
-    if ((bid & ((1 << cand_shift(cfg)) - 1)) >= ncand[frame]) return false;
-    const ft8rx_record& r = rec[bid];
-    if (r.status != FT8RX_ST_ACTIVE) return false;
-    f0 = r.f0_idx; h0 = r.h0_idx;
-    return true;
-}
 FT8_DEV void fine_tables(const Tables& T, cpx* w400, cpx* w32, cpx* wq, int tid) {
     for (int i = tid; i < 400; i += FINE_NT) w400[i] = T.W3200[8 * i];
     if (tid < 32) w32[tid] = T.W32[tid];
```

New measurement: 91850, median of 6. +3.5%, better.
